# fraunhoferhhi/gaussian_gan_decoder

Hardware: AMD Instinct MI355X
Metric: forward raster frames/s, 1M Gaussians @ 1024x1024 (higher is better)
Workload: dtype f32; 1 GPU; 1000000 synthetic Gaussians ('cube' scene, seed 0, SH degree 0), 1024x1024, forward raster fp32, inputs resident in HBM; num_rendered=4152095, tiles=4096, parallelism=scene-parallel x1 (no collective)

## Files before the change

gaussian_gan_decoder_amd/_capi.py:

```python
from __future__ import annotations

import ctypes as C
import os
import threading

_PKG = os.path.dirname(os.path.abspath(__file__))
LIB_PATH = os.environ.get("GGD_LIB_PATH") or os.path.join(_PKG, "libggd_raster.so")

EXPORTS = [
    "ggd_geom_bytes", "ggd_binning_bytes", "ggd_img_bytes", "ggd_geom_layout", "ggd_binning_layout",
    "ggd_img_layout", "ggd_sort_bits", "ggd_create", "ggd_destroy", "ggd_last_error", "ggd_version",
    "ggd_forward_geometry", "ggd_forward_render", "ggd_forward", "ggd_forward_enqueue", "ggd_forward_collect", "ggd_forward_can_speculate", "ggd_backward",
    "ggd_forward_aux", "ggd_forward_render_aux", "ggd_backward_aux", "ggd_backward_abs", "ggd_mark_visible", "ggd_debug_unsorted",
    "ggd_triplane_forward", "ggd_triplane_backward", "ggd_trigrid_forward", "ggd_trigrid_backward", "ggd_planes_gather", "ggd_planes_scatter", "ggd_surface_tmp_bytes", "ggd_surface_sample", "ggd_attrs_split", "ggd_attrs_merge", "ggd_decoder_packed_bytes", "ggd_decoder_pack", "ggd_decoder_forward", "ggd_decoder_zbuf_bytes", "ggd_decoder_packed_t_bytes",
    "ggd_decoder_forward_train", "ggd_decoder_backward", "ggd_decoder_wgrad_floats", "ggd_decoder_wgrad", "ggd_decoder_backward_wgrad", "ggd_decoder_packed_hl_bytes", "ggd_decoder_packed_t_hl_bytes", "ggd_decoder_dzbuf_hl_bytes", "ggd_decoder_pack_hl", "ggd_decoder_forward_hl", "ggd_decoder_backward_wgrad_hl",
    "ggd_decoder_pack_chain", "ggd_decoder_forward_chain", "ggd_decoder_forward_train_chain", "ggd_decoder_backward_chain", "ggd_decoder_wgrad_chain",
    "ggd_decoder_backward_wgrad_chain", "ggd_decoder_pack_hl_chain", "ggd_decoder_forward_hl_chain", "ggd_decoder_backward_wgrad_hl_chain",
    "ggd_image_loss_tmp_bytes", "ggd_image_loss", "ggd_image_loss_masked", "ggd_mask_composite", "ggd_geometry_loss_tmp_bytes", "ggd_geometry_loss", "ggd_set_option", "ggd_get_option", "ggd_blend_stats", "ggd_blend_backward_stats", "ggd_blend_timeline", "ggd_set_profiling", "ggd_stage_count", "ggd_stage_name", "ggd_stage_times",
    "ggd_knn_tmp_bytes", "ggd_knn_leaf_size", "ggd_knn_max_points", "ggd_knn3", "ggd_knn3_stage",
    "ggd_densify_tmp_bytes", "ggd_densify_stats", "ggd_densify_plan", "ggd_prune_plan", "ggd_densify_emit", "ggd_densify_gather",
    "ggd_density_points", "ggd_density_grid", "ggd_density_lattice", "ggd_teacher_render",
]


class Params(C.Structure):
    _fields_ = [("P", C.c_int32), ("M", C.c_int32), ("sh_degree", C.c_int32), ("width", C.c_int32),
                ("height", C.c_int32), ("tanfovx", C.c_float), ("tanfovy", C.c_float),
                ("scale_modifier", C.c_float), ("prefiltered", C.c_int32), ("debug", C.c_int32),
                ("viewmatrix", C.c_void_p), ("projmatrix", C.c_void_p), ("campos", C.c_void_p),
                ("bg", C.c_void_p), ("raw_attributes", C.c_int32), ("antialiasing", C.c_int32)]


class GeomView(C.Structure):
    _fields_ = [(n, C.c_size_t) for n in ("splat", "tiles_touched", "point_offsets", "clamped", "depth_keys", "rect", "header", "total")]


class BinningView(C.Structure):
    _fields_ = [(n, C.c_size_t) for n in ("keys", "list", "keys_alt", "list_alt", "total")]


class ImgView(C.Structure):
    _fields_ = [(n, C.c_size_t) for n in ("ranges", "final_T", "n_contrib", "total")]


OPT_EXP_MODE, OPT_BLEND_CULL, OPT_BINNING, OPT_BLEND_SPLIT, OPT_FOLD, OPT_MSD_SORT, OPT_PREPROCESS_WGS = 0, 1, 2, 3, 4, 5, 6
STAT_FLAT_STREAK, STAT_SORT_RERUNS, STAT_MSD_FRAMES, STAT_SCAN_IN_SCATTER_FRAMES = 100, 101, 102, 103
SPLAT_BYTES = 48
SPLAT_FIELDS = ("x", "y", "hA", "nB", "hC", "thr", "opacity", "r", "g", "b", "ex", "ey")

_lib = None
_lock = threading.Lock()


def load():
    global _lib
    with _lock:
        if _lib is not None:
            return _lib
        if not os.path.exists(LIB_PATH):
            raise ImportError(
                f"{LIB_PATH} is missing: build it with `python -m gaussian_gan_decoder_amd.build` "
                "(hipcc --offload-arch=gfx950). There is no CPU fallback for the rasterizer.")
        import torch
        lib = C.CDLL(LIB_PATH, mode=C.RTLD_GLOBAL)
        vp, i32, i64, sz = C.c_void_p, C.c_int32, C.c_int64, C.c_size_t
        lib.ggd_geom_bytes.restype = sz; lib.ggd_geom_bytes.argtypes = [i32]
        lib.ggd_binning_bytes.restype = sz; lib.ggd_binning_bytes.argtypes = [i64]
        lib.ggd_img_bytes.restype = sz; lib.ggd_img_bytes.argtypes = [i32, i32]
        lib.ggd_geom_layout.argtypes = [i32, C.POINTER(GeomView)]
        lib.ggd_binning_layout.argtypes = [i64, C.POINTER(BinningView)]
        lib.ggd_img_layout.argtypes = [i32, i32, C.POINTER(ImgView)]
        lib.ggd_sort_bits.argtypes = [i32, i32]
        lib.ggd_create.restype = vp; lib.ggd_create.argtypes = [C.c_int]
        lib.ggd_destroy.restype = None; lib.ggd_destroy.argtypes = [vp]
        lib.ggd_last_error.restype = C.c_char_p; lib.ggd_last_error.argtypes = [vp]
        lib.ggd_version.restype = C.c_char_p
        lib.ggd_forward_geometry.argtypes = [vp, vp, C.POINTER(Params)] + [vp] * 7 + [vp, vp, C.POINTER(i64)]
        lib.ggd_forward_render.argtypes = [vp, vp, C.POINTER(Params), vp, i64, vp, vp, vp]
        lib.ggd_forward.argtypes = [vp, vp, C.POINTER(Params)] + [vp] * 7 + [vp, vp, vp, i64, vp, vp, C.POINTER(i64)]
        lib.ggd_forward_enqueue.argtypes = [vp, vp, C.POINTER(Params)] + [vp] * 7 + [vp, vp, vp, i64, vp, vp]
        lib.ggd_forward_collect.argtypes = [vp, vp, C.POINTER(i64)]
        lib.ggd_forward_can_speculate.argtypes = [vp, C.POINTER(Params), i64]
        lib.ggd_backward.argtypes = [vp, vp, C.POINTER(Params)] + [vp] * 7 + [vp, vp, vp, vp, i64, vp] + [vp] * 8
        lib.ggd_forward_aux.argtypes = [vp, vp, C.POINTER(Params)] + [vp] * 7 + [vp, vp, vp, i64, vp, vp, vp, vp, C.POINTER(i64)]
        lib.ggd_forward_render_aux.argtypes = [vp, vp, C.POINTER(Params), vp, i64, vp, vp, vp, vp, vp]
        lib.ggd_backward_aux.argtypes = [vp, vp, C.POINTER(Params)] + [vp] * 7 + [vp, vp, vp, vp, i64, vp, vp, vp] + [vp] * 8
        lib.ggd_backward_abs.argtypes = [vp, vp, C.POINTER(Params)] + [vp] * 7 + [vp, vp, vp, vp, i64, vp, vp, vp] + [vp] * 9
        lib.ggd_mark_visible.argtypes = [vp, vp, i32, vp, vp, vp, vp]
        lib.ggd_debug_unsorted.argtypes = [vp, vp, vp, vp, i64]
        lib.ggd_triplane_forward.argtypes = [vp, vp, vp, i32, i32, i32, vp, i32, C.c_float, vp]
        lib.ggd_triplane_backward.argtypes = [vp, vp, i32, i32, i32, vp, i32, C.c_float, vp, vp]
        lib.ggd_trigrid_forward.argtypes = [vp, vp, vp, i32, i32, i32, i32, i32, vp, i32, C.c_float, vp]
        lib.ggd_trigrid_backward.argtypes = [vp, vp, i32, i32, i32, i32, i32, vp, i32, C.c_float, vp, vp]
        lib.ggd_planes_gather.argtypes = [vp, vp, vp, i32, i32, i32, i32, i32, vp, vp, i32, C.c_float, vp]
        lib.ggd_planes_scatter.argtypes = [vp, vp, i32, i32, i32, i32, i32, vp, vp, i32, C.c_float, vp, vp, i32]
        lib.ggd_surface_tmp_bytes.restype = sz; lib.ggd_surface_tmp_bytes.argtypes = [i32]
        lib.ggd_surface_sample.argtypes = [vp, vp, vp, i32, C.c_float, i32, C.c_float, C.c_uint64, vp, vp, vp, sz]
        lib.ggd_attrs_split.argtypes = [vp, vp, vp, i64, vp, vp, vp, vp, vp]
        lib.ggd_attrs_merge.argtypes = [vp, vp, i64, vp, vp, vp, vp, vp, vp]
        lib.ggd_decoder_packed_bytes.restype = sz
        lib.ggd_decoder_pack.argtypes = [vp, vp, C.POINTER(C.c_void_p), vp, vp]
        lib.ggd_decoder_forward.argtypes = [vp, vp, vp, vp, i32, vp, vp]
        lib.ggd_decoder_zbuf_bytes.restype = sz; lib.ggd_decoder_zbuf_bytes.argtypes = [i32]
        lib.ggd_decoder_packed_t_bytes.restype = sz
        lib.ggd_decoder_forward_train.argtypes = [vp, vp, vp, vp, i32, vp, vp, vp]
        lib.ggd_decoder_backward.argtypes = [vp, vp, i32, vp, vp, vp, vp, vp, vp, vp, vp]
        lib.ggd_decoder_wgrad_floats.restype = sz
        lib.ggd_decoder_wgrad.argtypes = [vp, vp, i32, vp, vp, vp, vp, vp, vp, vp]
        lib.ggd_decoder_backward_wgrad.argtypes = [vp, vp, i32, i32, vp, vp, vp, vp, vp, vp, vp, vp, vp, vp, vp]
        lib.ggd_decoder_packed_hl_bytes.restype = sz
        lib.ggd_decoder_packed_t_hl_bytes.restype = sz
        lib.ggd_decoder_dzbuf_hl_bytes.restype = sz; lib.ggd_decoder_dzbuf_hl_bytes.argtypes = [i32]
        lib.ggd_decoder_pack_hl.argtypes = [vp, vp, C.POINTER(C.c_void_p), vp, vp]
        lib.ggd_decoder_forward_hl.argtypes = [vp, vp, vp, vp, i32, vp, vp, vp]
        lib.ggd_decoder_backward_wgrad_hl.argtypes = [vp, vp, i32, i32, vp, vp, vp, vp, vp, vp, vp, vp, vp, vp, vp]
        for name in ("pack", "forward", "forward_train", "backward", "wgrad", "backward_wgrad", "pack_hl", "forward_hl",
                     "backward_wgrad_hl"):
            base = getattr(lib, "ggd_decoder_" + name).argtypes
            getattr(lib, "ggd_decoder_" + name + "_chain").argtypes = list(base[:2]) + [i32] + list(base[2:])
        lib.ggd_image_loss_tmp_bytes.restype = sz; lib.ggd_image_loss_tmp_bytes.argtypes = [i32, i32]
        lib.ggd_image_loss.argtypes = [vp, vp, i32, i32, vp, vp, vp, vp, vp, vp, sz]
        lib.ggd_image_loss_masked.argtypes = [vp, vp, i32, i32, vp, vp, vp, i32, i32, vp, vp, vp, vp, sz]
        lib.ggd_mask_composite.argtypes = [vp, vp, i32, i32, i32, vp, vp, i32, i32, i32, vp]
        lib.ggd_geometry_loss_tmp_bytes.restype = sz; lib.ggd_geometry_loss_tmp_bytes.argtypes = [i32, i32]
        lib.ggd_geometry_loss.argtypes = [vp, vp, i32, i32, vp, vp, vp, vp, i32, i32, C.c_float, C.c_float, i32, vp, vp, vp, vp, vp, sz]
        lib.ggd_set_option.argtypes = [vp, C.c_int, C.c_int]
        lib.ggd_get_option.argtypes = [vp, C.c_int]
        lib.ggd_blend_stats.argtypes = [vp, C.c_int, C.POINTER(C.c_ulonglong)]
        lib.ggd_blend_backward_stats.argtypes = [vp, C.POINTER(C.c_ulonglong)]
        lib.ggd_blend_timeline.argtypes = [vp, C.POINTER(C.c_ulonglong), C.c_int]
        lib.ggd_set_profiling.argtypes = [vp, C.c_int]
        lib.ggd_stage_name.restype = C.c_char_p; lib.ggd_stage_name.argtypes = [C.c_int]
        lib.ggd_stage_times.argtypes = [vp, C.POINTER(C.c_float)]
        lib.ggd_knn_tmp_bytes.restype = sz; lib.ggd_knn_tmp_bytes.argtypes = [i32]
        lib.ggd_knn_leaf_size.restype = i32; lib.ggd_knn_leaf_size.argtypes = []
        lib.ggd_knn_max_points.restype = i32; lib.ggd_knn_max_points.argtypes = []
        lib.ggd_knn3.argtypes = [vp, vp, vp, i32, vp, vp, vp, vp, vp, sz]
        lib.ggd_knn3_stage.argtypes = [vp, vp, vp, i32, vp, vp, vp, vp, vp, sz, i32]
        f32 = C.c_float
        lib.ggd_densify_tmp_bytes.restype = sz; lib.ggd_densify_tmp_bytes.argtypes = [i32]
        lib.ggd_densify_stats.argtypes = [vp, vp, i32, vp, vp, vp, vp, vp, vp]
        lib.ggd_densify_plan.argtypes = [vp, vp, i32, vp, vp, vp, vp, f32, f32, f32, i32, f32, vp, sz, C.POINTER(i64)]
        lib.ggd_prune_plan.argtypes = [vp, vp, i32, vp, vp, sz, C.POINTER(i64)]
        lib.ggd_densify_emit.argtypes = [vp, vp, i32, i32, i32, C.POINTER(C.c_void_p), C.POINTER(C.c_void_p), vp, vp, sz]
        lib.ggd_densify_gather.argtypes = [vp, vp, i32, i32, i32, vp, vp, vp, sz]
        lib.ggd_density_points.argtypes = [vp, vp, vp, i32, i32, i32, i32, i32, f32, vp, vp, vp, vp, i32, vp, i32, vp, vp]
        lib.ggd_density_grid.argtypes = [vp, vp, vp, i32, i32, i32, i32, i32, f32, vp, vp, vp, vp, i32, i32, C.c_double, i32, vp, vp]
        lib.ggd_density_lattice.argtypes = [vp, vp, i32, C.c_double, i32, vp]
        lib.ggd_teacher_render.argtypes = [vp, vp, vp, i32, i32, i32, i32, i32, f32, vp, vp, vp, vp, i32, vp, vp, i32, C.c_double, C.c_double,
                                           vp, i32, i32, vp, vp, i32, C.c_double, i32, vp, vp, vp, vp]
        _lib = lib
        return lib


class RasterError(RuntimeError):
    pass


class Context:
    capacity_hint: dict
    capacity_retries: int

    def __init__(self, device_index: int):
        self.capacity_hint = {}
        self.capacity_retries = 0
        self.poison_outputs = False
        self.lib = load()
        self.device_index = int(device_index)
        self.handle = self.lib.ggd_create(self.device_index)
        if not self.handle:
            raise RasterError("ggd_create failed: " + self.lib.ggd_last_error(None).decode())

    def check(self, rc: int):
        if rc != 0:
            raise RasterError(f"ggd error {rc}: " + self.lib.ggd_last_error(self.handle).decode())

    def set_option(self, option: int, value: int):
        self.check(self.lib.ggd_set_option(self.handle, int(option), int(value)))

    def get_option(self, option: int) -> int:
        return int(self.lib.ggd_get_option(self.handle, int(option)))

    def blend_stats(self, enable):
        out = (C.c_ulonglong * 6)()
        self.check(self.lib.ggd_blend_stats(self.handle, int(enable), out))
        return dict(zip(("visited", "culled", "lanes", "pixels", "listed", "culled_in_loop"), [int(v) for v in out]))

    def blend_backward_stats(self):
        out = (C.c_ulonglong * 8)()
        self.check(self.lib.ggd_blend_backward_stats(self.handle, out))
        return dict(zip(("walked", "staged", "needed", "blended", "live_lanes", "atomic_spans", "rounds", "waves"), [int(v) for v in out]))

    def blend_timeline(self, waves: int):
        import numpy as np
        out = (C.c_ulonglong * (3 * waves))()
        self.check(self.lib.ggd_blend_timeline(self.handle, out, int(waves)))
        a = np.frombuffer(out, dtype=np.uint64).reshape(waves, 3)
        return np.stack([a[:, 0], a[:, 1], a[:, 2] >> np.uint64(32), a[:, 2] & np.uint64(0xFFFFFFFF)], 1).astype(np.int64)

    def set_profiling(self, on: bool):
        self.check(self.lib.ggd_set_profiling(self.handle, int(bool(on))))

    def stage_times(self) -> dict:
        n = self.lib.ggd_stage_count()
        arr = (C.c_float * n)()
        self.check(self.lib.ggd_stage_times(self.handle, arr))
        return {self.lib.ggd_stage_name(i).decode(): float(arr[i]) for i in range(n) if arr[i] >= 0}

    def close(self):
        if getattr(self, "handle", None):
            self.lib.ggd_destroy(self.handle)
            self.handle = None

    def __del__(self):
        try:
            self.close()
        except Exception:
            pass


_contexts: dict = {}


def context_for(device) -> Context:
    import torch
    idx = device.index if device.index is not None else torch.cuda.current_device()
    key = (idx, int(torch.cuda.current_stream(idx).cuda_stream))
    ctx = _contexts.get(key)
    if ctx is None:
        ctx = _contexts[key] = Context(idx)
    return ctx


def context_and_stream(device):
    import torch
    idx = device.index if device.index is not None else torch.cuda.current_device()
    handle = int(torch.cuda.current_stream(idx).cuda_stream)
    key = (idx, handle)
    ctx = _contexts.get(key)
    if ctx is None:
        ctx = _contexts[key] = Context(idx)
    return ctx, handle


def geom_view(P: int) -> GeomView:
    v = GeomView(); load().ggd_geom_layout(P, C.byref(v)); return v


def binning_view(R: int) -> BinningView:
    v = BinningView(); load().ggd_binning_layout(R, C.byref(v)); return v


def img_view(W: int, H: int) -> ImgView:
    v = ImgView(); load().ggd_img_layout(W, H, C.byref(v)); return v
```

gaussian_gan_decoder_amd/csrc/ggd_binning.hip:

```cpp
#include "ggd_common.h"

namespace {

#include "ggd_scan.inc"
#include "ggd_lookback.inc"

__global__ __launch_bounds__(SCAN_THREADS) void scan_reduce_kernel(const uint32_t* __restrict__ in, int64_t n,
                                                                   uint32_t* __restrict__ block_sums) {
  __shared__ uint32_t lds4[4];
  scan_reduce_block(in, n, block_sums, (int)blockIdx.x, lds4);
}

__global__ __launch_bounds__(SCAN_THREADS) void scan_blocksums_kernel(uint32_t* __restrict__ block_sums, int nb,
                                                                      uint32_t* __restrict__ d_total,
                                                                      uint32_t* h_total = nullptr) {
  __shared__ uint32_t lds4[4];
  scan_blocksums_block(block_sums, nb, d_total, h_total, lds4);
}

__global__ __launch_bounds__(SCAN_THREADS) void scan_apply_kernel(const uint32_t* __restrict__ in,
                                                                  uint32_t* __restrict__ out, int64_t n,
                                                                  const uint32_t* __restrict__ block_prefix) {
  __shared__ uint32_t lds4[4];
  scan_apply_block(in, out, n, block_prefix, (int)blockIdx.x, lds4);
}

__global__ __launch_bounds__(256) void duplicate_kernel(int P, int W, int H, const uint2* __restrict__ rect,
                                                        const uint32_t* __restrict__ depth_keys,
                                                        const uint32_t* __restrict__ tiles_touched,
                                                        const uint32_t* __restrict__ offsets,
                                                        uint64_t* __restrict__ keys, uint32_t* __restrict__ vals) {
  __shared__ uint32_t s_excl[257];
  __shared__ uint32_t s_origin[256];
  __shared__ uint32_t s_width[256];
  __shared__ uint32_t s_depth[256];
  __shared__ uint32_t s_base;
  const int tid = threadIdx.x;
  const int first = blockIdx.x * 256;
  const int i = first + tid;
  uint32_t nt = 0, inc = 0;
  if (i < P) { nt = tiles_touched[i]; inc = offsets[i]; }
  const uint32_t excl = inc - nt;
  if (tid == 0) s_base = excl;
  const int gx = (W + 15) / 16;
  uint32_t origin = 0, width = 1, dbits = 0;
  if (nt > 0) {
    const uint2 rc = rect[i];
    origin = (rc.x & 0xffffu) | ((rc.y & 0xffffu) << 16);
    width = (rc.x >> 16) - (rc.x & 0xffffu);
    dbits = depth_keys[i];
  }
  __syncthreads();
  const uint32_t base = s_base;
  s_excl[tid] = excl - base;
  s_origin[tid] = origin; s_width[tid] = width; s_depth[tid] = dbits;
  const int last = min(P, first + 256) - 1 - first;
  if (tid == last) s_excl[256] = inc - base;
  __syncthreads();
  const uint32_t total = s_excl[256];
  if (tid > last) s_excl[tid] = total;
  __syncthreads();
  for (uint32_t j = tid; j < total; j += 256) {
    int lo = 0;
#pragma unroll
    for (int step = 128; step >= 1; step >>= 1) {
      const int probe = lo + step;
      if (probe < 256 && s_excl[probe] <= j) lo = probe;
    }
    const uint32_t k = j - s_excl[lo];
    const uint32_t w = s_width[lo];
    const uint32_t ry = k / w, rx = k - ry * w;
    const uint32_t org = s_origin[lo];
    const uint32_t tile = ((org >> 16) + ry) * (uint32_t)gx + (org & 0xffffu) + rx;
    const size_t dst = (size_t)base + j;
    keys[dst] = ((uint64_t)tile << 32) | (uint64_t)s_depth[lo];
    vals[dst] = (uint32_t)(first + lo);
  }
}

template <typename KeyT, int ITEMS, bool SKIP = false>
__global__ __launch_bounds__(RS_THREADS) void sort_global_hist_kernel(const KeyT* __restrict__ keys, int64_t n,
                                                                      int passes, uint32_t* __restrict__ ghist,
                                                                      uint32_t* __restrict__ n_valid = nullptr,
                                                                      uint32_t* __restrict__ zero_ptr = nullptr,
                                                                      size_t zero_words = 0, int main_blocks = 0x7fffffff,
                                                                      ggd_scan_piggy pg = ggd_scan_piggy{}) {
  __shared__ uint32_t s_hist[RS_MAX_PASSES * RS_BINS];
  if ((int)blockIdx.x >= main_blocks) {
    scan_reduce_block(pg.in, pg.n, pg.block_sums, (int)blockIdx.x - main_blocks, s_hist);
    return;
  }
  const size_t nmain = (size_t)min((int)gridDim.x, main_blocks);
  for (size_t i = (size_t)blockIdx.x * RS_THREADS + threadIdx.x; i < zero_words; i += nmain * RS_THREADS)
    zero_ptr[i] = 0u;
  uint32_t my_valid = 0;
  for (int b = threadIdx.x; b < passes * RS_BINS; b += RS_THREADS) s_hist[b] = 0;
  __syncthreads();
  const int64_t base = (int64_t)blockIdx.x * (RS_THREADS * ITEMS);
  const int lane = threadIdx.x & 63;
  KeyT kreg[ITEMS];
#pragma unroll
  for (int k = 0; k < ITEMS; ++k) {
    const int64_t idx = base + (int64_t)k * RS_THREADS + threadIdx.x;
    kreg[k] = idx < n ? keys[idx] : (KeyT)0;
  }
#pragma unroll
  for (int k = 0; k < ITEMS; ++k) {
    const int64_t idx = base + (int64_t)k * RS_THREADS + threadIdx.x;
    const KeyT key = kreg[k];
    const bool ok = idx < n && !(SKIP && key == (KeyT)~(KeyT)0);
    const uint64_t act = __ballot(ok);
    if (act == 0ull) continue;
    if (SKIP && (threadIdx.x & 63) == 0) my_valid += (uint32_t)__popcll(act);
    const int leader = __builtin_ctzll(act);
    for (int p = 0; p < passes; ++p) {
      const uint32_t d = (uint32_t)(key >> (8 * p)) & 0xffu;
      if (p < 2) {
        if (ok) atomicAdd(&s_hist[p * RS_BINS + d], 1u);
        continue;
      }
      const uint32_t d0 = (uint32_t)__builtin_amdgcn_readlane((int)d, leader);
      if (__ballot(ok && d != d0) == 0ull) {
        if (lane == leader) atomicAdd(&s_hist[p * RS_BINS + d0], (uint32_t)__popcll(act));
      } else if (ok) {
        atomicAdd(&s_hist[p * RS_BINS + d], 1u);
      }
    }
  }
  __syncthreads();
  for (int b = threadIdx.x; b < passes * RS_BINS; b += RS_THREADS) {
    const uint32_t c = s_hist[b];
    if (c) atomicAdd(&ghist[b], c);
  }
  if (SKIP && n_valid && my_valid) atomicAdd(n_valid, my_valid);
}

__device__ __forceinline__ void fold_publish_range(const ggd_scan_piggy& pg, uint32_t flags, uint32_t nmin, uint32_t kmax) {
  if (threadIdx.x != 0) return;
  if (pg.d_total) { pg.d_total[3] = ~nmin; pg.d_total[4] = kmax; pg.d_total[5] = flags; }
  if (pg.h_total) { pg.h_total[4] = ~nmin; pg.h_total[5] = kmax; pg.h_total[6] = flags; }
}

enum ggd_passenger_role : int {
  GGD_PASSENGER_SCAN_SUMS = 2,
  GGD_PASSENGER_SCAN_APPLY = 3,
};

template <typename KeyT, bool IOTA, int ITEMS, bool COMPACT = false, bool STAGE = false>
__global__ __launch_bounds__(RS_THREADS) void sort_onesweep_kernel(
    const KeyT* __restrict__ keys_in, const uint32_t* __restrict__ vals_in, KeyT* __restrict__ keys_out,
    uint32_t* __restrict__ vals_out, int64_t n_host, int shift, const uint32_t* __restrict__ ghist ,
    uint32_t* status , int ntiles, int gshift, uint32_t* ticket,
    const uint32_t* __restrict__ n_dev = nullptr, int piggy_role = 0, ggd_scan_piggy pg = ggd_scan_piggy{},
    uint32_t* __restrict__ flat_flag = nullptr, int hist_reps = 1) {
  __shared__ uint32_t s_cnt[4][RS_BINS];
  if ((int)blockIdx.x >= ntiles) {
    if (piggy_role == GGD_PASSENGER_SCAN_SUMS && pg.wg_info) {
      const uint4 tv = scan_info_block(pg.wg_info, pg.n_info, pg.block_sums, pg.n_valid, pg.d_total, pg.h_total, &s_cnt[0][0]);
      int flat = 0;
      if (pg.fold_hist) {
        uint32_t acc[3] = {0u, 0u, 0u};
#pragma unroll 8
        for (int r = 1; r < GGD_FOLD_REPS; ++r) {
#pragma unroll
          for (int p = 1; p < 4; ++p) acc[p - 1] += pg.fold_hist[r * GGD_FOLD_REP_STRIDE + p * RS_BINS + threadIdx.x];
        }
#pragma unroll
        for (int p = 1; p < 4; ++p) {
          acc[p - 1] += pg.fold_hist[p * RS_BINS + threadIdx.x];
          pg.fold_hist[p * RS_BINS + threadIdx.x] = acc[p - 1];
        }
        flat = __syncthreads_or(acc[2] == tv.y);
        fold_publish_range(pg, flat ? 1u : 0u, tv.z, tv.w);
      }
      if (threadIdx.x == 0) {
        if (pg.spec_flat && pg.flat_flag) *pg.flat_flag = 1u;
        if (pg.d_total) pg.d_total[2] = (uint32_t)flat;
        if (pg.h_tagged)
          __hip_atomic_store(pg.h_tagged, ((unsigned long long)flat << 63) | ((unsigned long long)(pg.tag & 0x3fffffffu) << 32) | tv.x,
                             __ATOMIC_RELEASE, __HIP_MEMORY_SCOPE_SYSTEM);
      }
    }
    else if (piggy_role == GGD_PASSENGER_SCAN_SUMS)
      scan_blocksums_block(pg.block_sums, pg.nb, pg.d_total, pg.h_total, &s_cnt[0][0], pg.h_tagged, pg.tag);
    else
      scan_apply_block(pg.in, pg.out, pg.n, pg.block_sums, (int)blockIdx.x - ntiles, &s_cnt[0][0], pg.sum_stride);
    return;
  }
  __shared__ uint32_t s_scan[4];
  __shared__ uint32_t s_tile;
  __shared__ uint32_t s_flat;
  __shared__ KeyT s_keys[STAGE ? RS_THREADS * ITEMS : 1];
  __shared__ uint32_t s_vals[STAGE ? RS_THREADS * ITEMS : 1];
  __shared__ uint32_t s_gdst[STAGE ? RS_BINS : 1];
  __shared__ uint32_t s_ntile;
  const int lane = threadIdx.x & 63, wv = threadIdx.x >> 6;
  const bool use_ticket = ntiles > RS_RESIDENT;
  if (use_ticket && threadIdx.x == 0) s_tile = atomicAdd(ticket, 1u);
  const uint32_t n_dev_v = (COMPACT && !IOTA) ? *n_dev : 0u;
  uint32_t my_bin = ghist[threadIdx.x];
  if (hist_reps > 1) {
    uint32_t rep[GGD_FOLD_REPS - 1];
#pragma unroll
    for (int r = 1; r < GGD_FOLD_REPS; ++r) rep[r - 1] = ghist[r * GGD_FOLD_REP_STRIDE + threadIdx.x];
#pragma unroll
    for (int r = 1; r < GGD_FOLD_REPS; ++r) my_bin += rep[r - 1];
  }
  for (int b = threadIdx.x; b < 4 * RS_BINS; b += RS_THREADS) (&s_cnt[0][0])[b] = 0;
  if (threadIdx.x == 0) s_flat = 0u;
  uint32_t tile = blockIdx.x;
  if (use_ticket) { __syncthreads(); tile = s_tile; }

  const int64_t wbase = (int64_t)tile * (RS_THREADS * ITEMS) + (int64_t)wv * (64 * ITEMS);
  KeyT key[ITEMS];
  uint32_t val[ITEMS];
  uint32_t rank[ITEMS];
#pragma unroll
  for (int r = 0; r < ITEMS; ++r) {
    const int64_t idx = wbase + r * 64 + lane;
    const bool ok = idx < n_host;
    key[r] = ok ? keys_in[idx] : (KeyT)~(KeyT)0;
    val[r] = IOTA ? (uint32_t)idx : (ok ? vals_in[idx] : 0u);
  }
  const int64_t n = (COMPACT && !IOTA) ? (int64_t)n_dev_v : n_host;
  if (COMPACT && (int64_t)tile * (RS_THREADS * ITEMS) >= n) return;
  if (!use_ticket) __syncthreads();
  if (COMPACT && !IOTA) {
    if ((int64_t)my_bin == n) s_flat = 1u;
    __syncthreads();
    if (s_flat != 0u) {
      if (flat_flag) {
        if (tile == 0u && threadIdx.x == 0) *flat_flag = 1u;
        return;
      }
#pragma unroll
      for (int r = 0; r < ITEMS; ++r) {
        const int64_t idx = wbase + r * 64 + lane;
        if (idx < n) { keys_out[idx] = key[r]; vals_out[idx] = val[r]; }
      }
      return;
    }
  }
  const uint64_t lt_mask = (1ull << lane) - 1ull;
#pragma unroll
  for (int r = 0; r < ITEMS; ++r) {
    const int64_t idx = wbase + r * 64 + lane;
    const bool ok = idx < n && !(COMPACT && IOTA && key[r] == (KeyT)~(KeyT)0);
    const uint32_t d = (uint32_t)(key[r] >> shift) & 0xffu;
    uint64_t peers = __ballot(ok);
#pragma unroll
    for (int b = 0; b < 8; ++b) {
      const uint64_t m = __ballot((d >> b) & 1u);
      peers &= ((d >> b) & 1u) ? m : ~m;
    }
    const uint32_t before = s_cnt[wv][d];
    const uint32_t below = (uint32_t)__popcll(peers & lt_mask);
    rank[r] = before + below;
    __builtin_amdgcn_wave_barrier();
    if (ok && below == 0) s_cnt[wv][d] = before + (uint32_t)__popcll(peers);
    __builtin_amdgcn_wave_barrier();
  }
  __syncthreads();
  {
    const int d = threadIdx.x;
    const uint32_t c0 = s_cnt[0][d], c1 = s_cnt[1][d], c2 = s_cnt[2][d], c3 = s_cnt[3][d];
    const uint32_t local = c0 + c1 + c2 + c3;
    const int64_t live_tiles = (n + RS_THREADS * ITEMS - 1) / (RS_THREADS * ITEMS);
    gshift = min(gshift, ggd_group_shift(live_tiles));
    const uint32_t excl = lookback_two_level<RS_BINS>(status, d, ntiles, tile, gshift, local, 0u);
    uint32_t tot;
    const uint32_t gbase = block_exclusive_scan_256(my_bin, &tot, s_scan);
    const uint32_t base = gbase + excl;
    if constexpr (STAGE) {
      uint32_t ltot;
      const uint32_t lexcl = block_exclusive_scan_256(local, &ltot, s_scan);
      s_cnt[0][d] = lexcl; s_cnt[1][d] = lexcl + c0; s_cnt[2][d] = lexcl + c0 + c1; s_cnt[3][d] = lexcl + c0 + c1 + c2;
      s_gdst[d] = base - lexcl;
      if (d == 0) s_ntile = ltot;
    } else {
      s_cnt[0][d] = base; s_cnt[1][d] = base + c0; s_cnt[2][d] = base + c0 + c1; s_cnt[3][d] = base + c0 + c1 + c2;
    }
  }
  __syncthreads();
  if constexpr (STAGE) {
#pragma unroll
    for (int r = 0; r < ITEMS; ++r) {
      const int64_t idx = wbase + r * 64 + lane;
      if (idx < n && !(COMPACT && IOTA && key[r] == (KeyT)~(KeyT)0)) {
        const uint32_t d = (uint32_t)(key[r] >> shift) & 0xffu;
        const uint32_t p = s_cnt[wv][d] + rank[r];
        s_keys[p] = key[r];
        s_vals[p] = val[r];
      }
    }
    __syncthreads();
    const uint32_t nt = s_ntile;
    for (uint32_t p = threadIdx.x; p < nt; p += RS_THREADS) {
      const KeyT k = s_keys[p];
      const uint32_t d = (uint32_t)(k >> shift) & 0xffu;
      const size_t dst = (size_t)(uint32_t)(s_gdst[d] + p);
      keys_out[dst] = k;
      vals_out[dst] = s_vals[p];
    }
    return;
  }
#pragma unroll
  for (int r = 0; r < ITEMS; ++r) {
    const int64_t idx = wbase + r * 64 + lane;
    if (idx < n && !(COMPACT && IOTA && key[r] == (KeyT)~(KeyT)0)) {
      const uint32_t d = (uint32_t)(key[r] >> shift) & 0xffu;
      const size_t dst = (size_t)s_cnt[wv][d] + rank[r];
      keys_out[dst] = key[r];
      vals_out[dst] = val[r];
    }
  }
}


#include "ggd_msd_finish.inc"
constexpr int MSD_DIGIT_BITS = 10;
static_assert((1 << MSD_DIGIT_BITS) == GGD_MSD_BINS && GGD_MSD_BINS % (4 * RS_THREADS) == 0, "1024 buckets");

__device__ __forceinline__ void msd_piggy_block(const ggd_scan_piggy& pg, uint32_t* lds) {
  constexpr int NS = GGD_FOLD_REP_STRIDE / 256;
  uint32_t rep[GGD_FOLD_REPS][NS];
#pragma unroll
  for (int r = 0; r < GGD_FOLD_REPS; ++r)
#pragma unroll
    for (int q = 0; q < NS; ++q) rep[r][q] = pg.fold_hist[r * GGD_FOLD_REP_STRIDE + q * 256 + threadIdx.x];
  const uint32_t outside = pg.fold_hist[GGD_FOLD_OUTSIDE];
  const uint4 tv = scan_info_block(pg.wg_info, pg.n_info, pg.block_sums, pg.n_valid, pg.d_total, pg.h_total, lds);
  uint32_t acc[NS];
#pragma unroll
  for (int q = 0; q < NS; ++q) acc[q] = 0u;
#pragma unroll
  for (int r = 0; r < GGD_FOLD_REPS; ++r) {
#pragma unroll
    for (int q = 0; q < NS; ++q) acc[q] += rep[r][q];
  }
  bool over = false;
#pragma unroll
  for (int q = 0; q < NS; ++q) {
    pg.fold_hist[q * 256 + threadIdx.x] = acc[q];
    if (q < NS - 1) over = over || acc[q] > (uint32_t)GGD_MSD_CAP;
  }
  const int flat = __syncthreads_or(acc[NS - 1] == tv.y);
  const int big = __syncthreads_or(over);
  const bool inside = outside == 0u;
  const unsigned long long ok = (inside && !big) ? 1ull : 0ull;
  fold_publish_range(pg, (flat ? 1u : 0u) | (inside ? 2u : 0u) | (big ? 0u : 4u), tv.z, tv.w);
  if (threadIdx.x == 0) {
    if (pg.d_total) pg.d_total[2] = (uint32_t)(flat ? 1u : 0u) | ((uint32_t)ok << 1);
    if (pg.h_tagged)
      __hip_atomic_store(pg.h_tagged, ((unsigned long long)(flat ? 1 : 0) << 63) | (ok << 62) |
                                      ((unsigned long long)(pg.tag & 0x3fffffffu) << 32) | tv.x,
                         __ATOMIC_RELEASE, __HIP_MEMORY_SCOPE_SYSTEM);
  }
}

__global__ __launch_bounds__(RS_THREADS) void sort_msd_partition_kernel(const uint32_t* __restrict__ keys_in,
                                                                        uint32_t* __restrict__ keys_out,
                                                                        uint32_t* __restrict__ vals_out, int64_t n,
                                                                        uint32_t* __restrict__ table, int ntiles,
                                                                        uint32_t lo, int shift, ggd_scan_piggy pg) {
  __shared__ uint32_t s_cnt[4][GGD_MSD_BINS];
  __shared__ uint32_t s_keys[MSD_TILE];
  __shared__ uint32_t s_vals[MSD_TILE];
  __shared__ uint32_t s_scan[4];
  if ((int)blockIdx.x >= ntiles) { msd_piggy_block(pg, &s_cnt[0][0]); return; }
  const int lane = threadIdx.x & 63, wv = threadIdx.x >> 6;
  const uint32_t tile = blockIdx.x;
  const int64_t wbase = (int64_t)tile * MSD_TILE + (int64_t)wv * (64 * MSD_ITEMS);
  uint32_t key[MSD_ITEMS], rank[MSD_ITEMS];
#pragma unroll
  for (int r = 0; r < MSD_ITEMS; ++r) {
    const int64_t idx = wbase + r * 64 + lane;
    key[r] = idx < n ? keys_in[idx] : 0xffffffffu;
  }
  uint32_t dig[MSD_ITEMS];
#pragma unroll
  for (int r = 0; r < MSD_ITEMS; ++r) {
    const bool ok = key[r] != 0xffffffffu;
    const uint32_t rel = key[r] - lo;
    dig[r] = min(rel >> shift, (uint32_t)(GGD_MSD_BINS - 1));
    key[r] = ok ? rel : 0xffffffffu;
    if (!ok) dig[r] = 0xffffffffu;
  }
  for (int b = threadIdx.x; b < 4 * GGD_MSD_BINS; b += RS_THREADS) (&s_cnt[0][0])[b] = 0;
  __syncthreads();
  const uint64_t lt_mask = (1ull << lane) - 1ull;
#pragma unroll
  for (int r = 0; r < MSD_ITEMS; ++r) {
    const bool ok = dig[r] != 0xffffffffu;
    const uint32_t d = dig[r] & (GGD_MSD_BINS - 1);
    uint64_t peers = __ballot(ok);
#pragma unroll
    for (int b = 0; b < MSD_DIGIT_BITS; ++b) {
      const uint64_t m = __ballot((d >> b) & 1u);
      peers &= ((d >> b) & 1u) ? m : ~m;
    }
    const uint32_t before = s_cnt[wv][d];
    const uint32_t below = (uint32_t)__popcll(peers & lt_mask);
    rank[r] = before + below;
    __builtin_amdgcn_wave_barrier();
    if (ok && below == 0) s_cnt[wv][d] = before + (uint32_t)__popcll(peers);
    __builtin_amdgcn_wave_barrier();
  }
  __syncthreads();
  uint32_t ltot;
  {
    constexpr int DPT = GGD_MSD_BINS / RS_THREADS, G = DPT / 4;
    uint4 c[G][4];
    uint32_t mine = 0;
#pragma unroll
    for (int g = 0; g < G; ++g)
#pragma unroll
      for (int w = 0; w < 4; ++w) {
        c[g][w] = *reinterpret_cast<const uint4*>(&s_cnt[w][DPT * threadIdx.x + 4 * g]);
        mine += c[g][w].x + c[g][w].y + c[g][w].z + c[g][w].w;
      }
    uint32_t e = block_exclusive_scan_256(mine, &ltot, s_scan);
#pragma unroll
    for (int g = 0; g < G; ++g) {
      const uint32_t l0 = c[g][0].x + c[g][1].x + c[g][2].x + c[g][3].x, l1 = c[g][0].y + c[g][1].y + c[g][2].y + c[g][3].y;
      const uint32_t l2 = c[g][0].z + c[g][1].z + c[g][2].z + c[g][3].z, l3 = c[g][0].w + c[g][1].w + c[g][2].w + c[g][3].w;
      const uint32_t e0 = e, e1 = e0 + l0, e2 = e1 + l1, e3 = e2 + l2;
      e = e3 + l3;
      uint4 run = make_uint4(e0, e1, e2, e3);
#pragma unroll
      for (int w = 0; w < 4; ++w) {
        *reinterpret_cast<uint4*>(&s_cnt[w][DPT * threadIdx.x + 4 * g]) = run;
        run.x += c[g][w].x; run.y += c[g][w].y; run.z += c[g][w].z; run.w += c[g][w].w;
      }
      *reinterpret_cast<uint4*>(table + (size_t)tile * GGD_MSD_BINS + DPT * threadIdx.x + 4 * g) =
          make_uint4((e0 << 16) | l0, (e1 << 16) | l1, (e2 << 16) | l2, (e3 << 16) | l3);
    }
  }
  __syncthreads();
#pragma unroll
  for (int r = 0; r < MSD_ITEMS; ++r) {
    if (dig[r] != 0xffffffffu) {
      const uint32_t d = dig[r];
      const uint32_t p = s_cnt[wv][d] + rank[r];
      s_keys[p] = key[r];
      s_vals[p] = (uint32_t)(wbase + r * 64 + lane);
    }
  }
  __syncthreads();
  for (uint32_t p = threadIdx.x; p < ltot; p += RS_THREADS) {
    keys_out[(size_t)tile * MSD_TILE + p] = s_keys[p];
    vals_out[(size_t)tile * MSD_TILE + p] = s_vals[p];
  }
}

__global__ __launch_bounds__(MSDF_THREADS, 8) void sort_msd_finish_kernel(const uint32_t* __restrict__ keys_in,
                                                                       const uint32_t* __restrict__ vals_in,
                                                                       uint32_t* __restrict__ keys_out,
                                                                       uint32_t* __restrict__ vals_out,
                                                                       const uint32_t* __restrict__ hist ,
                                                                       const uint32_t* __restrict__ table, int ntiles, int kshift) {
  __shared__ msd_lds L;
  const int tid = threadIdx.x;
  const uint32_t b = blockIdx.x;
  const uint32_t nb = hist[b];
  constexpr int HPT = GGD_MSD_BINS / MSDF_THREADS;
  uint32_t below = 0;
#pragma unroll
  for (int q = 0; q < HPT; ++q) { const uint32_t i = (uint32_t)(HPT * tid + q); const uint32_t h = hist[i]; if (i < b) below += h; }
  const uint32_t e0 = tid < ntiles ? table[(size_t)tid * GGD_MSD_BINS + b] : 0u;
  if (nb == 0u) return;
  uint32_t base;
  block_exclusive_scan_1024(below, &base, L.part);
  const bool oversized = nb > (uint32_t)GGD_MSD_CAP;
  msd_bucket_pieces(L, table, ntiles, b, e0, oversized);
  if (oversized) {
    for (uint32_t p = tid; p < nb; p += MSDF_THREADS) {
      const size_t src = msd_piece_src_big(L, table, b, ntiles, p);
      vals_out[(size_t)base + p] = vals_in[src];
    }
    return;
  }
  if (nb > (uint32_t)MSD_XCAP) {
    msd_bucket_sort<true, MSDF_ITEMS>(L, keys_in, vals_in, ntiles, nb, kshift, keys_out + base, vals_out + base);
    return;
  }
  msd_bucket_sort<false, MSDX_ITEMS>(L, keys_in, vals_in, ntiles, nb, kshift, nullptr, nullptr);
  for (uint32_t p = tid; p < nb; p += MSDF_THREADS) vals_out[(size_t)base + p] = L.kv[MSD_XCAP + p];
}

__global__ __launch_bounds__(256) void ranges_kernel(const uint64_t* __restrict__ keys, int64_t n,
                                                     uint32_t* __restrict__ ranges) {
  const int64_t i = (int64_t)blockIdx.x * 256 + threadIdx.x;
  if (i >= n) return;
  const uint32_t tile = (uint32_t)(keys[i] >> 32);
  if (i == 0) {
    ranges[2 * tile] = 0;
  } else {
    const uint32_t prev = (uint32_t)(keys[i - 1] >> 32);
    if (prev != tile) {
      ranges[2 * prev + 1] = (uint32_t)i;
      ranges[2 * tile] = (uint32_t)i;
    }
  }
  if (i == n - 1) ranges[2 * tile + 1] = (uint32_t)n;
}

}

size_t ggd_scan_tmp_bytes(int64_t n) {
  const int64_t nb = (n + SCAN_TILE - 1) / SCAN_TILE;
  return ggd_align((size_t)(nb > 0 ? nb : 1) * sizeof(uint32_t));
}

int ggd_launch_inclusive_scan(ggd_ctx* ctx, hipStream_t s, const uint32_t* in, uint32_t* out, int64_t n,
                              uint32_t* d_total, void* tmp, size_t tmp_bytes, uint32_t* h_total) {
  if (n <= 0) {
    if (d_total) GGD_HIP(hipMemsetAsync(d_total, 0, sizeof(uint32_t), s));
    if (h_total) *h_total = 0u;
    return GGD_OK;
  }
  const int nb = (int)((n + SCAN_TILE - 1) / SCAN_TILE);
  if (tmp_bytes < (size_t)nb * sizeof(uint32_t)) return ggd_fail(ctx, GGD_E_INVALID, "scan tmp too small");
  uint32_t* block_sums = static_cast<uint32_t*>(tmp);
  hipLaunchKernelGGL(scan_reduce_kernel, dim3(nb), dim3(SCAN_THREADS), 0, s, in, n, block_sums);
  hipLaunchKernelGGL(scan_blocksums_kernel, dim3(1), dim3(SCAN_THREADS), 0, s, block_sums, nb, d_total, h_total);
  hipLaunchKernelGGL(scan_apply_kernel, dim3(nb), dim3(SCAN_THREADS), 0, s, in, out, n, block_sums);
  GGD_HIP(hipGetLastError());
  return GGD_OK;
}
int ggd_scan_blocks(int64_t n) { return n > 0 ? (int)((n + SCAN_TILE - 1) / SCAN_TILE) : 0; }

int ggd_launch_duplicate(ggd_ctx* ctx, hipStream_t s, const ggd_params& prm, const uint2* rect, const uint32_t* depth_keys,
                         const uint32_t* tiles_touched, const uint32_t* offsets, uint64_t* keys, uint32_t* vals) {
  if (prm.P == 0) return GGD_OK;
  hipLaunchKernelGGL(duplicate_kernel, dim3((prm.P + 255) / 256), dim3(256), 0, s, prm.P, prm.width, prm.height,
                     rect, depth_keys, tiles_touched, offsets, keys, vals);
  GGD_HIP(hipGetLastError());
  return GGD_OK;
}

static inline int sort_passes(int nbits) { return (nbits + 7) / 8; }
int ggd_sort_input_is_alt(int nbits) { return sort_passes(nbits) & 1; }

template <typename KeyT>
static int launch_sort_t(ggd_ctx* ctx, hipStream_t s, KeyT* keys_a, uint32_t* vals_a, KeyT* keys_b, uint32_t* vals_b,
                         int64_t n, int nbits, void* tmp, size_t tmp_bytes) {
  if (n <= 0) return GGD_OK;
  const int passes = sort_passes(nbits);
  if (passes > RS_MAX_PASSES) return ggd_fail(ctx, GGD_E_INVALID, "sort: too many key bits");
  if (tmp_bytes < ggd_sort_tmp_bytes(n)) return ggd_fail(ctx, GGD_E_INVALID, "sort tmp too small");
  const int ntiles = (int)((n + RS_TILE - 1) / RS_TILE);
  const ggd_sort_ctl ctl = ggd_sort_ctl::in_tmp(tmp);
  const int gshift = ggd_group_shift((int64_t)ntiles);
  GGD_HIP(hipMemsetAsync(tmp, 0, ggd_sort_clear_bytes(passes, ntiles), s));
  KeyT* kin = (passes & 1) ? keys_b : keys_a;
  uint32_t* vin = (passes & 1) ? vals_b : vals_a;
  KeyT* kout = (passes & 1) ? keys_a : keys_b;
  uint32_t* vout = (passes & 1) ? vals_a : vals_b;
  hipLaunchKernelGGL((sort_global_hist_kernel<KeyT, RS_ITEMS>), dim3(ntiles), dim3(RS_THREADS), 0, s, kin, n, passes,
                     ctl.ghist);
  for (int p = 0; p < passes; ++p) {
    hipLaunchKernelGGL((sort_onesweep_kernel<KeyT, false, RS_ITEMS>), dim3(ntiles), dim3(RS_THREADS), 0, s, kin, vin, kout, vout, n,
                       8 * p, ctl.pass_hist(p), ctl.pass_status(p, ntiles), ntiles, gshift, ctl.pass_ticket(p));
    KeyT* tk = kin; kin = kout; kout = tk;
    uint32_t* tv = vin; vin = vout; vout = tv;
  }
  GGD_HIP(hipGetLastError());
  return GGD_OK;
}

int ggd_launch_sort32_iota(ggd_ctx* ctx, hipStream_t s, const uint32_t* keys_src, uint32_t* keys_a, uint32_t* vals_a,
                           uint32_t* keys_b, uint32_t* vals_b, int64_t n, int nbits, void* tmp, size_t tmp_bytes,
                           const ggd_sort32_opts& o) {
  if (n <= 0) return GGD_OK;
  const ggd_fold* fold = o.fold;
  const int passes = sort_passes(nbits);
  if (passes > RS_MAX_PASSES || (passes & 1)) return ggd_fail(ctx, GGD_E_INVALID, "sort32: need an even pass count");
  if (fold && (passes != 4 || !o.piggy || !o.piggy->wg_info)) return ggd_fail(ctx, GGD_E_INVALID, "sort32: folded front end needs 4 passes and the workgroup sums");
  if (!fold && tmp_bytes < ggd_sort32_tmp_bytes(n)) return ggd_fail(ctx, GGD_E_INVALID, "sort tmp too small");
  if (o.skip_last && !(fold && o.flag_flat_last)) return ggd_fail(ctx, GGD_E_INVALID, "sort32: skip_last needs the folded front end");
  const int ntiles = (int)((n + RS32_TILE - 1) / RS32_TILE);
  const ggd_sort_ctl ctl = ggd_sort_ctl::select(tmp, o.clean_ctl, fold ? fold->ctl : nullptr);
  const bool own_ctl = !o.clean_ctl && !fold;
  const int gshift = ggd_group_shift((int64_t)ntiles);
  if (own_ctl) GGD_HIP(hipMemsetAsync(tmp, 0, ggd_sort_clear_bytes(passes, ntiles), s));
  ggd_scan_piggy pg = o.piggy ? *o.piggy : ggd_scan_piggy{};
  const int pnb = o.piggy ? pg.nb : 0;
  if (fold) { pg.n_valid = ctl.n_valid; pg.fold_hist = ctl.ghist; pg.flat_flag = ctl.flat; pg.spec_flat = o.skip_last ? 1 : 0; }
  if (!fold) {
    const int htiles = ntiles;
    hipLaunchKernelGGL((sort_global_hist_kernel<uint32_t, RS32_ITEMS, true>), dim3(htiles + pnb), dim3(RS_THREADS), 0, s,
                       keys_src, n, passes, ctl.ghist, ctl.n_valid, o.clean_ctl ? ctl.status : nullptr,
                       o.clean_ctl ? ggd_sort_status_words(passes, ntiles) : (size_t)0, htiles, pg);
  }
  const uint32_t* kin = keys_src;
  const uint32_t* vin = nullptr;
  for (int p = 0; p < passes - (o.skip_last ? 1 : 0); ++p) {
    uint32_t* kout = (p & 1) ? keys_a : keys_b;
    uint32_t* vout = (p & 1) ? vals_a : vals_b;
    if (p == 0)
      hipLaunchKernelGGL((sort_onesweep_kernel<uint32_t, true, RS32_ITEMS, true, true>), dim3(ntiles + (pnb ? 1 : 0)),
                         dim3(RS_THREADS), 0, s, kin, vin, kout, vout, n, 0, ctl.pass_hist(0), ctl.pass_status(0, ntiles), ntiles,
                         gshift, ctl.pass_ticket(0), ctl.n_valid, GGD_PASSENGER_SCAN_SUMS, pg, (uint32_t*)nullptr, ctl.reps);
    if (p != 0)
      hipLaunchKernelGGL((sort_onesweep_kernel<uint32_t, false, RS32_ITEMS, true, true>), dim3(ntiles + ((p == 1 && o.apply_here) ? pnb : 0)),
                         dim3(RS_THREADS), 0, s, kin, vin, kout, vout, n, 8 * p, ctl.pass_hist(p), ctl.pass_status(p, ntiles),
                         ntiles, gshift, ctl.pass_ticket(p), ctl.n_valid, GGD_PASSENGER_SCAN_APPLY, pg,
                         (o.flag_flat_last && p == passes - 1) ? ctl.flat : nullptr, 1);
    kin = kout; vin = vout;
  }
  GGD_HIP(hipGetLastError());
  return GGD_OK;
}

bool ggd_sort32_msd_supported(int64_t n) { return n > 0 && (n + MSD_TILE - 1) / MSD_TILE <= GGD_MSD_MAX_TILES; }

int ggd_launch_sort32_msd(ggd_ctx* ctx, hipStream_t s, const uint32_t* keys_src, uint32_t* keys_a, uint32_t* vals_a,
                          uint32_t* keys_b, uint32_t* vals_b, int64_t n, uint32_t* table, const ggd_scan_piggy* piggy,
                          const ggd_fold* fold) {
  if (n <= 0) return GGD_OK;
  if (!fold || !fold->msd || !piggy || !piggy->wg_info || !ggd_sort32_msd_supported(n))
    return ggd_fail(ctx, GGD_E_INVALID, "sort32 (two launches): needs the folded front end in its msd form");
  if (fold->msd_shift < 0 || fold->msd_shift > GGD_MSD_MAX_SHIFT) return ggd_fail(ctx, GGD_E_INVALID, "sort32 (two launches): bucket shift out of range");
  const int ntiles = (int)((n + MSD_TILE - 1) / MSD_TILE);
  const ggd_sort_ctl ctl = ggd_sort_ctl::in_fold(fold->ctl);
  ggd_scan_piggy pg = *piggy;
  pg.n_valid = ctl.n_valid; pg.fold_hist = ctl.ghist;
  hipLaunchKernelGGL(sort_msd_partition_kernel, dim3(ntiles + 1), dim3(RS_THREADS), 0, s, keys_src, keys_b, vals_b, n, table,
                     ntiles, fold->msd_lo, fold->msd_shift, pg);
  hipLaunchKernelGGL(sort_msd_finish_kernel, dim3(GGD_MSD_BINS), dim3(MSDF_THREADS), 0, s, keys_b, vals_b, keys_a, vals_a,
                     ctl.ghist, table, ntiles, fold->msd_shift);
  GGD_HIP(hipGetLastError());
  return GGD_OK;
}

int ggd_launch_sort(ggd_ctx* ctx, hipStream_t s, uint64_t* keys_a, uint32_t* vals_a, uint64_t* keys_b,
                    uint32_t* vals_b, int64_t n, int nbits, void* tmp, size_t tmp_bytes) {
  return launch_sort_t<uint64_t>(ctx, s, keys_a, vals_a, keys_b, vals_b, n, nbits, tmp, tmp_bytes);
}

int ggd_launch_ranges(ggd_ctx* ctx, hipStream_t s, const uint64_t* keys, int64_t n, uint32_t* ranges, int T) {
  GGD_HIP(hipMemsetAsync(ranges, 0, (size_t)T * 2 * sizeof(uint32_t), s));
  if (n <= 0) return GGD_OK;
  hipLaunchKernelGGL(ranges_kernel, dim3((unsigned)((n + 255) / 256)), dim3(256), 0, s, keys, n, ranges);
  GGD_HIP(hipGetLastError());
  return GGD_OK;
}
```

gaussian_gan_decoder_amd/csrc/ggd_binning_layout.h:

```cpp
#pragma once

#include <stdint.h>
#include <stddef.h>

#if defined(__HIPCC__)
#define GGD_HOST_DEVICE __host__ __device__
#else
#define GGD_HOST_DEVICE
#endif

static inline size_t ggd_align(size_t v, size_t a = 256) { return (v + a - 1) / a * a; }

constexpr int RS_THREADS = 256;
constexpr int RS_ITEMS = 16;
constexpr int RS_TILE = RS_THREADS * RS_ITEMS;
constexpr int RS_BINS = 256;
constexpr int RS_MAX_PASSES = 8;
constexpr int RS32_ITEMS = 16;
constexpr int RS32_TILE = RS_THREADS * RS32_ITEMS;
constexpr int RS_HWORDS = RS_MAX_PASSES * RS_BINS;
constexpr int RS_RESIDENT = 1024;

template <typename T>
GGD_HOST_DEVICE inline int ggd_group_shift(T n) { int g = 2; while (((T)1 << (2 * g)) < n) ++g; return g; }

static inline int64_t rs_status_words(int64_t ntiles) {
  return (ntiles + ((int64_t)1 << ggd_group_shift(ntiles)) + 1) * RS_BINS;
}
static inline int64_t ggd_tiles(int64_t n, int tile) { const int64_t t = (n + tile - 1) / tile; return t > 0 ? t : 1; }

static inline size_t ggd_sort_ctrl_bytes() { return ggd_align((size_t)(RS_HWORDS + 64) * sizeof(uint32_t)); }
static inline size_t ggd_sort_ctrl_words() { return ggd_sort_ctrl_bytes() / sizeof(uint32_t); }
static inline size_t ggd_sort_tmp_bytes(int64_t n) {
  return ggd_sort_ctrl_bytes() + ggd_align((size_t)RS_MAX_PASSES * (size_t)rs_status_words(ggd_tiles(n, RS_TILE)) * sizeof(uint32_t));
}
static inline size_t ggd_sort32_tmp_bytes(int64_t n) {
  return ggd_sort_ctrl_bytes() + ggd_align((size_t)4 * (size_t)rs_status_words(ggd_tiles(n, RS32_TILE)) * sizeof(uint32_t));
}
static inline size_t ggd_sort_status_words(int passes, int64_t ntiles) { return (size_t)passes * (size_t)rs_status_words(ntiles); }
static inline size_t ggd_sort_clear_bytes(int passes, int64_t ntiles) {
  return ggd_sort_ctrl_bytes() + ggd_sort_status_words(passes, ntiles) * sizeof(uint32_t);
}

constexpr int GGD_MSD_BINS = 1024, GGD_MSD_CAP = 12288, GGD_MSD_MAX_TILES = 2048;
constexpr int MSD_ITEMS = 16;
constexpr int MSD_TILE = 256 * MSD_ITEMS;
static inline size_t ggd_sort32_msd_table_bytes(int64_t n) {
  return ggd_align((size_t)ggd_tiles(n, MSD_TILE) * GGD_MSD_BINS * sizeof(uint32_t));
}

constexpr int GGD_FOLD_REPS = 16;
constexpr int GGD_FOLD_REP_STRIDE = GGD_MSD_BINS + 256;
constexpr int GGD_FOLD_OUTSIDE = GGD_FOLD_REPS * GGD_FOLD_REP_STRIDE + 16;
constexpr int GGD_FOLD_ROWTOT = GGD_FOLD_REPS * GGD_FOLD_REP_STRIDE + 64;
constexpr int GGD_FOLD_HEAD = GGD_FOLD_ROWTOT + GGD_FOLD_REPS * 64;
static inline size_t ggd_fold_l1_offset(int64_t P) {
  return (size_t)GGD_FOLD_HEAD + (size_t)4 * (size_t)rs_status_words(ggd_tiles(P, RS32_TILE));
}
static inline size_t ggd_fold_ctl_words(int64_t P) {
  const int64_t chunks = (P + 1023) / 1024;
  return ggd_fold_l1_offset(P) + (size_t)(chunks + ((int64_t)1 << ggd_group_shift(chunks > 0 ? chunks : 1)) + 2) * 64;
}
static inline size_t ggd_fold_rowinst_offset(int64_t P) { return ggd_fold_ctl_words(P); }
static inline size_t ggd_fold_block_words(int64_t P) { return ggd_fold_rowinst_offset(P) + (size_t)GGD_FOLD_REPS * 64; }
static inline uint32_t* ggd_fold_rowtot(uint32_t* fold_ctl) { return fold_ctl + GGD_FOLD_ROWTOT; }
static inline uint32_t* ggd_fold_rowinst(uint32_t* fold_ctl, int64_t P) { return fold_ctl + ggd_fold_rowinst_offset(P); }
static inline uint32_t* ggd_fold_l1_status(uint32_t* fold_ctl, int64_t P) { return fold_ctl + ggd_fold_l1_offset(P); }

struct ggd_sort_ctl {
  uint32_t* ghist = nullptr;
  uint32_t* tickets = nullptr;
  uint32_t* n_valid = nullptr;
  uint32_t* flat = nullptr;
  uint32_t* status = nullptr;
  int reps = 1;

  static ggd_sort_ctl in_tmp(void* tmp) {
    return make(static_cast<uint32_t*>(tmp), RS_HWORDS, tmp_status(tmp), 1);
  }
  static ggd_sort_ctl in_clean(uint32_t* clean_ctl, void* tmp) { return make(clean_ctl, RS_HWORDS, tmp_status(tmp), 1); }
  static ggd_sort_ctl in_fold(uint32_t* fold_ctl) {
    return make(fold_ctl, GGD_FOLD_REPS * GGD_FOLD_REP_STRIDE, fold_ctl + GGD_FOLD_HEAD, GGD_FOLD_REPS);
  }
  static ggd_sort_ctl select(void* tmp, uint32_t* clean_ctl, uint32_t* fold_ctl) {
    return fold_ctl ? in_fold(fold_ctl) : (clean_ctl ? in_clean(clean_ctl, tmp) : in_tmp(tmp));
  }

  uint32_t* pass_hist(int p) const { return ghist + p * RS_BINS; }
  uint32_t* pass_ticket(int p) const { return tickets + p; }
  uint32_t* pass_status(int p, int64_t ntiles) const { return status + ggd_sort_status_words(p, ntiles); }

 private:
  static uint32_t* tmp_status(void* tmp) { return reinterpret_cast<uint32_t*>(static_cast<char*>(tmp) + ggd_sort_ctrl_bytes()); }
  static ggd_sort_ctl make(uint32_t* head, int hist_words, uint32_t* status, int reps) {
    ggd_sort_ctl c;
    c.ghist = head; c.tickets = head + hist_words; c.n_valid = c.tickets + RS_MAX_PASSES; c.flat = c.n_valid + 1;
    c.status = status; c.reps = reps;
    return c;
  }
};

constexpr int RB_THREADS = 256;
constexpr int RB_IPL = 4;
constexpr int RB_CHUNK = RB_THREADS * RB_IPL;
constexpr int RB_TAB_ROWSTART = 0, RB_TAB_ROWBLK = 65, RB_TAB_TILESTART = 130, RB_TAB_ROWINST = 130 + 64 * 64,
              RB_TAB_FLAG = RB_TAB_ROWINST + 64, RB_TAB_WORDS = RB_TAB_FLAG + 64;
constexpr int RBW_NG = 4;
constexpr int RBW_BINS = 64 * RBW_NG;
constexpr int RBW_TAB_ROWSTART = 0, RBW_TAB_ROWBLK = RBW_BINS + 1, RBW_TAB_ROWINST = 2 * (RBW_BINS + 1),
              RBW_TAB_FLAG = RBW_TAB_ROWINST + RBW_BINS, RBW_TAB_TILESTART = RBW_TAB_FLAG + RBW_BINS,
              RBW_TAB_WORDS = RBW_TAB_TILESTART + RBW_BINS * RBW_BINS;

static inline bool rb_is_wide(int W, int H) { return (W + 15) / 16 > 64 || (H + 15) / 16 > 64; }
static inline int rb_blocks1(int P) { return (P + RB_CHUNK - 1) / RB_CHUNK; }
constexpr uint32_t RB_SCAN_IN_SCATTER_MAX_BLOCKS = (1u << 24) / RB_CHUNK + 128;
static inline uint32_t rb_blocks2(uint32_t cap, bool wide) {
  return (cap + RB_CHUNK - 1) / RB_CHUNK + (wide ? (uint32_t)RBW_BINS : 64u);
}

struct ggd_rowbin_tmp {
  size_t packed, counts1, tab, ent, counts2, total;
};
static inline ggd_rowbin_tmp ggd_rowbin_layout(int P, uint32_t capacity, int W, int H) {
  const bool wide = rb_is_wide(W, H);
  const int nby = 64 * (((H + 15) / 16 + 63) / 64), nbx = 64 * (((W + 15) / 16 + 63) / 64);
  ggd_rowbin_tmp t;
  t.packed = 0;
  t.counts1 = t.packed + ggd_align((size_t)P * 8);
  t.tab = t.counts1 + ggd_align((size_t)rb_blocks1(P) * (wide ? nby : 64) * 4);
  t.ent = t.tab + ggd_align((size_t)(wide ? RBW_TAB_WORDS : RB_TAB_WORDS) * 4);
  t.counts2 = t.ent + ggd_align((size_t)capacity * 8);
  t.total = t.counts2 + ggd_align((size_t)rb_blocks2(capacity, wide) * (wide ? nbx : 64) * 4);
  return t;
}
```

gaussian_gan_decoder_amd/csrc/ggd_capi.hip:

```cpp
#include <stdlib.h>
#include <string.h>

#include <initializer_list>
#include <new>

#include "ggd_common.h"

static std::string g_create_error;

static const char* const kStageNames[ST_COUNT] = {"preprocess", "scan", "readback", "duplicate", "sort",
                                                  "ranges", "blend", "blend_bwd", "preprocess_bwd"};

int ggd_fail(ggd_ctx* ctx, int code, const std::string& msg) {
  if (ctx) ctx->err = msg; else g_create_error = msg;
  return code;
}

int ggd_reserve_scratch(ggd_ctx* ctx, size_t bytes, hipStream_t stream) {
  if (bytes <= ctx->scratch_bytes) return GGD_OK;
  size_t want = bytes + bytes / 4 + (1u << 20);
  if (ctx->scratch) {
    GGD_HIP(hipStreamSynchronize(stream));
    GGD_HIP(hipFree(ctx->scratch));
    ctx->scratch = nullptr; ctx->scratch_bytes = 0;
  }
  hipError_t e = hipMalloc(&ctx->scratch, want);
  if (e != hipSuccess) return ggd_fail(ctx, GGD_E_NOMEM, std::string("hipMalloc scratch: ") + hipGetErrorString(e));
  ctx->scratch_bytes = want;
  return GGD_OK;
}

extern "C" int ggd_geom_layout(int32_t P, ggd_geom_view* v) {
  if (!v || P < 0) return GGD_E_INVALID;
  size_t off = 0;
  v->splat = off; off += ggd_align((size_t)P * sizeof(ggd_splat));
  v->tiles_touched = off; off += ggd_align((size_t)P * sizeof(uint32_t));
  v->point_offsets = off; off += ggd_align((size_t)P * sizeof(uint32_t));
  v->clamped = off; off += ggd_align((size_t)P);
  v->depth_keys = off; off += ggd_align((size_t)P * sizeof(uint32_t));
  v->rect = off; off += ggd_align((size_t)P * 2 * sizeof(uint32_t));
  v->header = off; off += (P > 0 ? 256 : 0);
  v->total = off;
  return GGD_OK;
}
extern "C" int ggd_binning_layout(int64_t R, ggd_binning_view* v) {
  if (!v || R < 0) return GGD_E_INVALID;
  size_t off = 0;
  v->list = off; off += ggd_align((size_t)R * sizeof(uint32_t));
  v->list_alt = off; off += ggd_align((size_t)R * sizeof(uint32_t));
  v->keys = off; off += ggd_align((size_t)R * sizeof(uint64_t));
  v->keys_alt = off; off += ggd_align((size_t)R * sizeof(uint64_t));
  v->total = off;
  return GGD_OK;
}
extern "C" int ggd_img_layout(int32_t W, int32_t H, ggd_img_view* v) {
  if (!v || W < 0 || H < 0) return GGD_E_INVALID;
  const size_t T = (size_t)((W + 15) / 16) * ((H + 15) / 16);
  size_t off = 0;
  v->ranges = off; off += ggd_align(T * 2 * sizeof(uint32_t));
  v->final_T = off; off += ggd_align((size_t)W * H * sizeof(float));
  v->n_contrib = off; off += ggd_align((size_t)W * H * sizeof(uint32_t));
  v->total = off;
  return GGD_OK;
}
extern "C" size_t ggd_geom_bytes(int32_t P) { ggd_geom_view v; return ggd_geom_layout(P, &v) == GGD_OK ? v.total : 0; }
extern "C" size_t ggd_binning_bytes(int64_t R) { ggd_binning_view v; return ggd_binning_layout(R, &v) == GGD_OK ? v.total : 0; }
extern "C" size_t ggd_img_bytes(int32_t W, int32_t H) { ggd_img_view v; return ggd_img_layout(W, H, &v) == GGD_OK ? v.total : 0; }

static uint32_t higher_msb(uint32_t n) {
  uint32_t msb = 16, step = 16;
  while (step > 1) {
    step /= 2;
    if (n >> msb) msb += step; else msb -= step;
  }
  if (n >> msb) msb++;
  return msb;
}
extern "C" int ggd_sort_bits(int32_t W, int32_t H) {
  const uint32_t T = (uint32_t)((W + 15) / 16) * (uint32_t)((H + 15) / 16);
  return 32 + (int)higher_msb(T);
}

static bool use_tile_binning(const ggd_ctx* ctx, const ggd_params* prm, int64_t R) {
  const int mode = ctx->opt[GGD_OPT_BINNING];
  return !prm->debug && ggd_rowbin_supported(prm->width, prm->height) && (mode >= 2 || (mode == 1 && R > 0));
}

struct ggd_buf { void** ptr; size_t elem; };
static int grow_buffers(ggd_ctx* ctx, std::initializer_list<ggd_buf> bufs, size_t* cap, size_t need, size_t want,
                        const hipStream_t* sync = nullptr) {
  if (*cap >= need) return GGD_OK;
  if (sync) GGD_HIP(hipStreamSynchronize(*sync));
  for (const ggd_buf& b : bufs) { if (*b.ptr) (void)hipFree(*b.ptr); *b.ptr = nullptr; }
  *cap = 0;
  for (const ggd_buf& b : bufs) GGD_HIP(hipMalloc(b.ptr, want * b.elem));
  *cap = want;
  return GGD_OK;
}

template <class T> static T* ggd_at(const void* base, size_t off) {
  return reinterpret_cast<T*>(static_cast<char*>(const_cast<void*>(base)) + off);
}
struct geom_ptrs { ggd_splat* splat; uint32_t *tiles, *offsets; uint8_t* clamped; uint32_t* depth_keys; uint2* rect; };
struct binning_ptrs { uint32_t *list, *list_alt; uint64_t *keys, *keys_alt; };
struct img_ptrs { uint32_t* ranges; float* final_T; uint32_t* n_contrib; };
static geom_ptrs geom_view(const ggd_params* prm, const void* buf) {
  ggd_geom_view v; ggd_geom_layout(prm->P, &v);
  return {ggd_at<ggd_splat>(buf, v.splat), ggd_at<uint32_t>(buf, v.tiles_touched), ggd_at<uint32_t>(buf, v.point_offsets),
          ggd_at<uint8_t>(buf, v.clamped), ggd_at<uint32_t>(buf, v.depth_keys), ggd_at<uint2>(buf, v.rect)};
}
static binning_ptrs binning_view(int64_t layout_R, const void* buf) {
  ggd_binning_view v; ggd_binning_layout(layout_R, &v);
  return {ggd_at<uint32_t>(buf, v.list), ggd_at<uint32_t>(buf, v.list_alt), ggd_at<uint64_t>(buf, v.keys), ggd_at<uint64_t>(buf, v.keys_alt)};
}
static img_ptrs img_view(int32_t W, int32_t H, const void* buf) {
  ggd_img_view v; ggd_img_layout(W, H, &v);
  return {ggd_at<uint32_t>(buf, v.ranges), ggd_at<float>(buf, v.final_T), ggd_at<uint32_t>(buf, v.n_contrib)};
}

extern "C" const char* ggd_version(void) { return "ggd-raster 0.1 (gfx950)"; }
extern "C" int ggd_stage_count(void) { return ST_COUNT; }
extern "C" const char* ggd_stage_name(int s) { return (s >= 0 && s < ST_COUNT) ? kStageNames[s] : ""; }

extern "C" ggd_ctx* ggd_create(int device) {
  int ndev = 0;
  if (hipGetDeviceCount(&ndev) != hipSuccess || ndev <= 0 || device < 0 || device >= ndev) {
    ggd_fail(nullptr, GGD_E_NODEVICE, "no HIP device " + std::to_string(device) + " visible");
    return nullptr;
  }
  ggd_ctx* ctx = new (std::nothrow) ggd_ctx();
  if (!ctx) { ggd_fail(nullptr, GGD_E_NOMEM, "out of host memory"); return nullptr; }
  ctx->device = device;
  if (const char* e = getenv("GGD_EXP_MODE")) { const int v = atoi(e); if (v >= 0 && v <= 3) ctx->opt[GGD_OPT_EXP_MODE] = v; }
  if (const char* e = getenv("GGD_BINNING")) { const int v = atoi(e); if (v >= 0 && v <= 3) ctx->opt[GGD_OPT_BINNING] = v; }
  if (const char* e = getenv("GGD_BLEND_SPLIT")) { const int v = atoi(e); if (v >= 0 && v <= 4) ctx->opt[GGD_OPT_BLEND_SPLIT] = v; }
  if (const char* e = getenv("GGD_BLEND_CULL")) ctx->opt[GGD_OPT_BLEND_CULL] = atoi(e) != 0;
  if (const char* e = getenv("GGD_FOLD")) ctx->opt[GGD_OPT_FOLD] = atoi(e) != 0;
  if (const char* e = getenv("GGD_MSD_SORT")) ctx->opt[GGD_OPT_MSD_SORT] = atoi(e) != 0;
  if (const char* e = getenv("GGD_PREPROCESS_WGS")) { const int v = atoi(e); if (v >= 0 && v <= GGD_PREPROCESS_WGS_MAX) ctx->opt[GGD_OPT_PREPROCESS_WGS] = v; }
  if (const char* e = getenv("GGD_MSD_BUCKETS")) { const int v = atoi(e); if (v >= 16 && v <= GGD_MSD_BINS) ctx->spec.msd_buckets = v; }
  int prev = 0;
  (void)hipGetDevice(&prev);
  bool ok = hipSetDevice(device) == hipSuccess &&
            hipMalloc((void**)&ctx->d_words, 256) == hipSuccess &&
            hipHostMalloc((void**)&ctx->h_words, 64, hipHostMallocCoherent | hipHostMallocMapped) == hipSuccess &&
            hipMemset(ctx->d_words, 0, 256) == hipSuccess &&
            hipDeviceGetAttribute(&ctx->cus, hipDeviceAttributeMultiprocessorCount, device) == hipSuccess && ctx->cus > 0;
  if (ok) memset(ctx->h_words, 0, 64);
  for (int i = 0; ok && i < 2 * ST_COUNT; ++i) ok = hipEventCreate(&ctx->ev[i]) == hipSuccess;
  if (ok && hipHostGetDevicePointer((void**)&ctx->h_words_dev, ctx->h_words, 0) != hipSuccess) {
    ctx->h_words_dev = nullptr;
    (void)hipGetLastError();
  }
  if (ok && (hipMalloc((void**)&ctx->sortctl, ggd_sort_ctrl_words() * sizeof(uint32_t)) != hipSuccess ||
             hipMemset(ctx->sortctl, 0, ggd_sort_ctrl_words() * sizeof(uint32_t)) != hipSuccess)) {
    ctx->sortctl = nullptr;
    (void)hipGetLastError();
  }
  (void)hipSetDevice(prev);
  if (!ok) {
    ggd_fail(nullptr, GGD_E_HIP, std::string("ggd_create: ") + hipGetErrorString(hipGetLastError()));
    ggd_destroy(ctx);
    return nullptr;
  }
  return ctx;
}

extern "C" void ggd_destroy(ggd_ctx* ctx) {
  if (!ctx) return;
  void* const device_buffers[] = {ctx->scratch, ctx->d_words, ctx->sortctl, ctx->foldctl[0], ctx->foldctl[1], ctx->gelu_tables,
                                  ctx->scan_sums, ctx->stats_buf, ctx->dbg_keys, ctx->dbg_vals};
  for (void* p : device_buffers) if (p) (void)hipFree(p);
  if (ctx->h_words) (void)hipHostFree(ctx->h_words);
  for (int i = 0; i < 2 * ST_COUNT; ++i)
    if (ctx->ev[i]) (void)hipEventDestroy(ctx->ev[i]);
  delete ctx;
}

extern "C" const char* ggd_last_error(ggd_ctx* ctx) { return ctx ? ctx->err.c_str() : g_create_error.c_str(); }

extern "C" int ggd_set_option(ggd_ctx* ctx, int option, int value) {
  if (!ctx) return GGD_E_INVALID;
  static const int kMax[GGD_OPT_COUNT] = {3, 1, 3, 4, 1, 1, GGD_PREPROCESS_WGS_MAX};
  if (option < 0 || option >= GGD_OPT_COUNT || value < 0 || value > kMax[option])
    return ggd_fail(ctx, GGD_E_INVALID, "ggd_set_option: unknown option or value");
  ctx->opt[option] = value;
  if (option == GGD_OPT_MSD_SORT || option == GGD_OPT_FOLD) {
    ctx->spec.reset();
  }
  return GGD_OK;
}
extern "C" int ggd_blend_stats(ggd_ctx* ctx, int enable, unsigned long long* out) {
  if (!ctx) return GGD_E_INVALID;
  GGD_HIP(hipDeviceSynchronize());
  if (out && ctx->blend_stats) GGD_HIP(hipMemcpy(out, ctx->stats_buf, 6 * sizeof(unsigned long long), hipMemcpyDeviceToHost));
  if (enable) {
    const size_t bytes = (GGD_STATS_HEAD + 3ull * GGD_STATS_MAX_WAVES) * sizeof(unsigned long long);
    if (!ctx->stats_buf) GGD_HIP(hipMalloc((void**)&ctx->stats_buf, bytes));
    GGD_HIP(hipMemset(ctx->stats_buf, 0, bytes));
    if (enable == 2) {
      const unsigned long long one = 1ull;
      GGD_HIP(hipMemcpy(ctx->stats_buf + GGD_STATS_MODE, &one, sizeof(one), hipMemcpyHostToDevice));
    }
    ctx->blend_stats = ctx->stats_buf;
  } else {
    ctx->blend_stats = nullptr;
  }
  return GGD_OK;
}
extern "C" int ggd_blend_backward_stats(ggd_ctx* ctx, unsigned long long* out) {
  if (!ctx || !out) return GGD_E_INVALID;
  if (!ctx->stats_buf) return ggd_fail(ctx, GGD_E_INVALID, "ggd_blend_backward_stats: statistics were never enabled (ggd_blend_stats)");
  GGD_HIP(hipDeviceSynchronize());
  GGD_HIP(hipMemcpy(out, ctx->stats_buf + GGD_STATS_BWD, 8 * sizeof(unsigned long long), hipMemcpyDeviceToHost));
  return GGD_OK;
}
extern "C" int ggd_blend_timeline(ggd_ctx* ctx, unsigned long long* out, int waves) {
  if (!ctx || !out || waves < 0 || waves > GGD_STATS_MAX_WAVES) return GGD_E_INVALID;
  if (!ctx->stats_buf) return ggd_fail(ctx, GGD_E_INVALID, "ggd_blend_timeline: statistics were never enabled");
  GGD_HIP(hipDeviceSynchronize());
  GGD_HIP(hipMemcpy(out, ctx->stats_buf + GGD_STATS_HEAD, 3ull * waves * sizeof(unsigned long long), hipMemcpyDeviceToHost));
  return GGD_OK;
}

extern "C" int ggd_get_option(ggd_ctx* ctx, int option) {
  if (ctx && option == GGD_STAT_FLAT_STREAK) return ctx->spec.flat_streak;
  if (ctx && option == GGD_STAT_SORT_RERUNS) return (int)(ctx->spec.reruns & 0x7fffffffull);
  if (ctx && option == GGD_STAT_MSD_FRAMES) return (int)(ctx->spec.msd_frames & 0x7fffffffull);
  if (ctx && option == GGD_STAT_SCAN_IN_SCATTER_FRAMES) return (int)(ctx->scan_in_scatter_frames & 0x7fffffffull);
  if (!ctx || option < 0 || option >= GGD_OPT_COUNT) return GGD_E_INVALID;
  return ctx->opt[option];
}

extern "C" int ggd_set_profiling(ggd_ctx* ctx, int enabled) {
  if (!ctx) return GGD_E_INVALID;
  ctx->profiling = enabled != 0;
  for (int i = 0; i < ST_COUNT; ++i) ctx->ev_used[i] = false;
  return GGD_OK;
}

extern "C" int ggd_stage_times(ggd_ctx* ctx, float* ms_out) {
  if (!ctx || !ms_out) return GGD_E_INVALID;
  for (int i = 0; i < ST_COUNT; ++i) {
    ms_out[i] = -1.0f;
    if (ctx->ev_used[i]) {
      GGD_HIP(hipEventSynchronize(ctx->ev[2 * i + 1]));
      float ms = 0.0f;
      GGD_HIP(hipEventElapsedTime(&ms, ctx->ev[2 * i], ctx->ev[2 * i + 1]));
      ms_out[i] = ms;
    }
  }
  return GGD_OK;
}

static int check_params(ggd_ctx* ctx, const ggd_params* prm) {
  if (!ctx) return GGD_E_INVALID;
  if (!prm) return ggd_fail(ctx, GGD_E_INVALID, "params is NULL");
  if (prm->P < 0 || prm->width <= 0 || prm->height <= 0)
    return ggd_fail(ctx, GGD_E_INVALID, "bad P / image size");
  if (!prm->viewmatrix || !prm->projmatrix || !prm->campos || !prm->bg)
    return ggd_fail(ctx, GGD_E_INVALID, "viewmatrix / projmatrix / campos / bg must be device pointers");
  if (prm->sh_degree < 0 || prm->sh_degree > 3) return ggd_fail(ctx, GGD_E_INVALID, "sh_degree must be 0..3");
  if (prm->tanfovx == 0.0f || prm->tanfovy == 0.0f) return ggd_fail(ctx, GGD_E_INVALID, "tanfov must be non-zero");
  return GGD_OK;
}

static int check_inputs(ggd_ctx* ctx, const ggd_params* prm, const float* means3D, const float* shs,
                        const float* colors_precomp, const float* scales, const float* rotations,
                        const float* cov3D_precomp) {
  if (prm->P == 0) return GGD_OK;
  if (!means3D) return ggd_fail(ctx, GGD_E_INVALID, "means3D is NULL");
  if ((shs == nullptr) == (colors_precomp == nullptr))
    return ggd_fail(ctx, GGD_E_INVALID, "Please provide excatly one of either SHs or precomputed colors!");
  if (((scales == nullptr) || (rotations == nullptr)) == (cov3D_precomp == nullptr) ||
      ((scales == nullptr) != (rotations == nullptr)))
    return ggd_fail(ctx, GGD_E_INVALID,
                    "Please provide exactly one of either scale/rotation pair or precomputed 3D covariance!");
  if (shs && (prm->sh_degree + 1) * (prm->sh_degree + 1) > prm->M)
    return ggd_fail(ctx, GGD_E_INVALID, "shs holds fewer coefficients than sh_degree needs");
  return GGD_OK;
}

static const char* const kPendingMsg = "a frame enqueued with ggd_forward_enqueue is pending on this context: call ggd_forward_collect first";

static ggd_frame frame_renew(ggd_ctx* ctx) {
  const ggd_frame old = ctx->frame;
  ctx->frame = ggd_frame();
  ctx->frame.r_tag = old.r_tag;
  return old;
}

static int fold_prepare(ggd_ctx* ctx, hipStream_t s, const ggd_params* prm, ggd_fold* fold) {
  const int nwg = (prm->P + 255) / 256;
  int rc = grow_buffers(ctx, {{(void**)&ctx->scan_sums, sizeof(uint32_t)}}, &ctx->scan_sums_cap, 5 * (size_t)nwg + 64,
                        5 * (size_t)(nwg + nwg / 2) + 64);
  if (rc != GGD_OK) return rc;
  const size_t need = ggd_fold_block_words(prm->P);
  const bool fresh = ctx->foldctl_cap < need;
  rc = grow_buffers(ctx, {{(void**)&ctx->foldctl[0], sizeof(uint32_t)}, {(void**)&ctx->foldctl[1], sizeof(uint32_t)}},
                    &ctx->foldctl_cap, need, need + need / 2, &s);
  if (rc != GGD_OK) return rc;
  if (fresh) ctx->fold_cur = 0;
  if (fresh || ctx->fold_poisoned) {
    for (int b = 0; b < 2; ++b) {
      GGD_HIP(hipMemsetAsync(ctx->foldctl[b], 0, ctx->foldctl_cap * sizeof(uint32_t), s));
      ctx->foldctl_dirty[b] = 0;
    }
    ctx->fold_poisoned = false;
  }
  const int cur = ctx->fold_cur, oth = cur ^ 1;
  fold->ctl = ctx->foldctl[cur];
  fold->clear = ctx->foldctl[oth];
  fold->clear_words = (uint32_t)ctx->foldctl_dirty[oth];
  fold->wg_info = reinterpret_cast<uint4*>(ctx->scan_sums + (((size_t)nwg + 3) & ~(size_t)3));
  fold->rows = ((prm->width + 15) / 16 <= 64 && (prm->height + 15) / 16 <= 64) ? 1 : 0;
  fold->rowinst = ggd_fold_rowinst(fold->ctl, prm->P);
  const ggd_spec_plan plan = ctx->spec.plan(ctx->opt[GGD_OPT_FOLD], ctx->opt[GGD_OPT_MSD_SORT], ggd_sort32_msd_supported(prm->P));
  fold->msd = plan.msd ? 1 : 0;
  fold->msd_lo = plan.lo; fold->msd_shift = plan.shift;
  ctx->foldctl_dirty[oth] = 0;
  ctx->foldctl_dirty[cur] = need;
  ctx->fold_cur = oth;
  ctx->frame.plan = plan;
  ctx->frame.geom.folded = true;
  return GGD_OK;
}

static int geometry_enqueue(ggd_ctx* ctx, void* stream, const ggd_params* prm, const float* means3D,
                            const float* shs, const float* colors_precomp, const float* opacities,
                            const float* scales, const float* rotations, const float* cov3D_precomp,
                            void* geom_buf, int32_t* radii, int64_t* num_rendered, bool defer_scan = false) {
  (void)hipGetLastError();
  int rc = check_params(ctx, prm);
  if (rc != GGD_OK) return rc;
  rc = check_inputs(ctx, prm, means3D, shs, colors_precomp, scales, rotations, cov3D_precomp);
  if (rc != GGD_OK) return rc;
  if (!num_rendered) return ggd_fail(ctx, GGD_E_INVALID, "num_rendered is NULL");
  *num_rendered = 0;
  frame_renew(ctx);
  ggd_frame& fr = ctx->frame;
  if (prm->P == 0) return GGD_OK;
  if (!geom_buf || !radii || !opacities) return ggd_fail(ctx, GGD_E_INVALID, "geom_buf / radii / opacities is NULL");
  if (prm->raw_attributes && cov3D_precomp)
    return ggd_fail(ctx, GGD_E_INVALID, "raw_attributes needs scales/rotations (no cov3D_precomp)");
  hipStream_t s = static_cast<hipStream_t>(stream);
  const geom_ptrs g = geom_view(prm, geom_buf);

  rc = ggd_reserve_scratch(ctx, ggd_scan_tmp_bytes(prm->P), s);
  if (rc != GGD_OK) return rc;
  if (prm->prefiltered) GGD_HIP(hipMemsetAsync(ctx->d_words + 1, 0, sizeof(uint32_t), s));
  const bool ride = defer_scan && ctx->h_words_dev;
  ggd_fold fold;
  if (ride && ctx->opt[GGD_OPT_FOLD] != 0) {
    rc = fold_prepare(ctx, s, prm, &fold);
    if (rc != GGD_OK) return rc;
  }
  {
    StageTimer t(ctx, ST_PREPROCESS, s);
    const bool old_ctl = !fr.geom.folded && ctx->sortctl;
    rc = ggd_launch_preprocess(ctx, s, *prm, means3D, shs, colors_precomp, opacities, scales, rotations,
                               cov3D_precomp, g.splat, g.tiles, shs ? g.clamped : nullptr, radii, g.depth_keys, g.rect,
                               ctx->d_words + 1, old_ctl ? ctx->sortctl : nullptr, old_ctl ? (int)ggd_sort_ctrl_words() : 0,
                               fr.geom.folded ? &fold : nullptr);
    if (rc != GGD_OK) { ctx->fold_poisoned = fr.geom.folded; return rc; }
    fr.geom.sortctl_clean = old_ctl;
  }
  if (ride) {
    const size_t nb = (size_t)ggd_scan_blocks(prm->P);
    if (!fr.geom.folded) {
      rc = grow_buffers(ctx, {{(void**)&ctx->scan_sums, sizeof(uint32_t)}}, &ctx->scan_sums_cap, nb, nb + nb / 2 + 64);
      if (rc != GGD_OK) return rc;
    }
    if (prm->prefiltered)
      GGD_HIP(hipMemcpyAsync(ctx->h_words + 1, ctx->d_words + 1, sizeof(uint32_t), hipMemcpyDeviceToHost, s));
    fr.geom.ride = true;
    return GGD_OK;
  }
  {
    StageTimer t(ctx, ST_SCAN, s);
    rc = ggd_launch_inclusive_scan(ctx, s, g.tiles, g.offsets, prm->P, ctx->d_words, ctx->scratch, ctx->scratch_bytes,
                                   ctx->h_words_dev);
    if (rc != GGD_OK) return rc;
  }
  {
    StageTimer t(ctx, ST_READBACK, s);
    if (!ctx->h_words_dev)
      GGD_HIP(hipMemcpyAsync(ctx->h_words, ctx->d_words, 2 * sizeof(uint32_t), hipMemcpyDeviceToHost, s));
    else if (prm->prefiltered)
      GGD_HIP(hipMemcpyAsync(ctx->h_words + 1, ctx->d_words + 1, sizeof(uint32_t), hipMemcpyDeviceToHost, s));
  }
  return GGD_OK;
}

static int geometry_finish(ggd_ctx* ctx, void* stream, const ggd_params* prm, int64_t* num_rendered) {
  ggd_frame& fr = ctx->frame;
  if (fr.r_pending) {
    volatile unsigned long long* slot = reinterpret_cast<volatile unsigned long long*>(ctx->h_words + 2);
    const unsigned long long want = fr.r_tag;
    unsigned long long v = *slot;
    for (unsigned spins = 0; ((v >> 32) & 0x3fffffffull) != want; ++spins) {
      __builtin_ia32_pause();
      if ((spins & 0xfff) == 0xfff) {
        const hipError_t q = hipStreamQuery(static_cast<hipStream_t>(stream));
        if (q == hipSuccess) {
          v = *slot;
          if (((v >> 32) & 0x3fffffffull) != want) {
            uint32_t w6[6] = {0u, 0u, 0u, 0u, 0u, 0u};
            GGD_HIP(hipMemcpy(w6, ctx->d_words, sizeof(w6), hipMemcpyDeviceToHost));
            v = ((unsigned long long)(w6[2] & 1u) << 63) | ((unsigned long long)((w6[2] >> 1) & 1u) << 62) | (want << 32) | w6[0];
            ctx->h_words[4] = w6[3]; ctx->h_words[5] = w6[4]; ctx->h_words[6] = w6[5];
          }
          break;
        }
        if (q != hipErrorNotReady)
          return ggd_fail(ctx, GGD_E_HIP, std::string("hipStreamQuery: ") + hipGetErrorString(q));
      }
      v = *slot;
    }
    ctx->h_words[0] = (uint32_t)v;
    fr.report.flat = (v >> 63) != 0ull;
    fr.report.msd_ok = ((v >> 62) & 1ull) != 0ull;
    if (fr.report.folded) {
      volatile uint32_t* hw = ctx->h_words;
      fr.report.kmin = hw[4]; fr.report.kmax = hw[5]; fr.report.msd_flags = hw[6];
    }
  } else {
    GGD_HIP(hipStreamSynchronize(static_cast<hipStream_t>(stream)));
  }
  if (prm->prefiltered && ctx->h_words[1] != 0)
    return ggd_fail(ctx, GGD_E_PREFILTER, "Point is filtered although prefiltered is set. This shouldn't happen!");
  *num_rendered = (int64_t)ctx->h_words[0];
  return GGD_OK;
}

extern "C" int ggd_forward_geometry(ggd_ctx* ctx, void* stream, const ggd_params* prm, const float* means3D,
                                    const float* shs, const float* colors_precomp, const float* opacities,
                                    const float* scales, const float* rotations, const float* cov3D_precomp,
                                    void* geom_buf, int32_t* radii, int64_t* num_rendered) {
  if (ctx && ctx->pending.valid) return ggd_fail(ctx, GGD_E_INVALID, kPendingMsg);
  const int rc = geometry_enqueue(ctx, stream, prm, means3D, shs, colors_precomp, opacities, scales, rotations,
                                  cov3D_precomp, geom_buf, radii, num_rendered);
  if (rc != GGD_OK || prm->P == 0) return rc;
  return geometry_finish(ctx, stream, prm, num_rendered);
}

static int sort_depth_and_bin_tiles(ggd_ctx* ctx, hipStream_t s, const ggd_params* prm, const geom_ptrs& g, uint32_t* list,
                                    uint32_t* ranges, uint32_t capacity, bool speculative) {
  ggd_frame& fr = ctx->frame;
  const bool riding = fr.geom.ride;
  const bool folded = riding && fr.geom.folded;
  const bool msd = folded && fr.plan.msd;
  uint32_t* clean_ctl = fr.geom.sortctl_clean ? ctx->sortctl : nullptr;
  fr.geom = {};
  const size_t pairs = ggd_align((size_t)prm->P * sizeof(uint32_t));
  const size_t sort_tmp = ggd_sort32_tmp_bytes(prm->P);
  const size_t bin_tmp = ggd_rowbin_tmp_bytes(prm->P, capacity, prm->width, prm->height);
  const size_t msd_tab = msd ? ggd_sort32_msd_table_bytes(prm->P) : 0;
  int rc = ggd_reserve_scratch(ctx, 4 * pairs + sort_tmp + bin_tmp + msd_tab, s);
  if (rc != GGD_OK) return rc;
  char* sc = static_cast<char*>(ctx->scratch);
  uint32_t* ka = reinterpret_cast<uint32_t*>(sc);
  uint32_t* va = reinterpret_cast<uint32_t*>(sc + pairs);
  uint32_t* kb = reinterpret_cast<uint32_t*>(sc + 2 * pairs);
  uint32_t* vb = reinterpret_cast<uint32_t*>(sc + 3 * pairs);
  void* tmp = sc + 4 * pairs;
  void* bin_tmp_ptr = sc + 4 * pairs + sort_tmp;
  ggd_scan_piggy pg;
  ggd_fold fold;
  const uint32_t *n_vis_ptr = nullptr, *flat_ptr = nullptr;
  {
    StageTimer t(ctx, ST_SORT, s);
    if (riding) {
      pg.in = g.tiles; pg.out = g.offsets;
      pg.n = prm->P; pg.nb = ggd_scan_blocks(prm->P); pg.block_sums = ctx->scan_sums;
      pg.d_total = ctx->d_words; pg.h_total = ctx->h_words_dev;
      pg.h_tagged = reinterpret_cast<unsigned long long*>(ctx->h_words_dev + 2);
      pg.tag = fr.r_tag = fr.r_tag % 0x3fffffffu + 1u;
      if (folded) {
        const int nwg = (prm->P + 255) / 256;
        fold.ctl = ctx->foldctl[ctx->fold_cur ^ 1];
        pg.wg_info = reinterpret_cast<const uint4*>(ctx->scan_sums + (((size_t)nwg + 3) & ~(size_t)3));
        pg.n_info = nwg;
        pg.sum_stride = 8;
      }
    }
    if (msd && !speculative) return ggd_fail(ctx, GGD_E_INVALID, "internal: two-launch sort outside the speculative tile-binning path");
    fr.three_passes = ctx->spec.three_passes(fr.plan, folded, speculative, ctx->opt[GGD_OPT_FOLD]);
    fr.report.folded = folded;
    fold.msd = msd ? 1 : 0;
    fold.msd_lo = fr.plan.lo; fold.msd_shift = fr.plan.shift;
    if (msd)
      rc = ggd_launch_sort32_msd(ctx, s, g.depth_keys, ka, va, kb, vb, prm->P,
                                 reinterpret_cast<uint32_t*>(sc + 4 * pairs + sort_tmp + bin_tmp), &pg, &fold);
    else {
      ggd_sort32_opts so;
      so.clean_ctl = folded ? nullptr : clean_ctl;
      so.piggy = riding ? &pg : nullptr;
      so.fold = folded ? &fold : nullptr;
      so.flag_flat_last = true;
      so.apply_here = false;
      so.skip_last = fr.three_passes;
      rc = ggd_launch_sort32_iota(ctx, s, g.depth_keys, ka, va, kb, vb, prm->P, 32, tmp, sort_tmp, so);
    }
    if (rc != GGD_OK) return rc;
    fr.r_pending = riding;
    const ggd_sort_ctl sc = ggd_sort_ctl::select(tmp, clean_ctl, folded ? fold.ctl : nullptr);
    n_vis_ptr = sc.n_valid; flat_ptr = sc.flat;
  }
  StageTimer t(ctx, ST_DUPLICATE, s);
  const bool l1 = folded && (prm->width + 15) / 16 <= 64 && (prm->height + 15) / 16 <= 64;
  bool scan_in_scatter = false;
  rc = ggd_launch_rowbin(ctx, s, *prm, g.rect, va, n_vis_ptr, list, ranges, capacity, bin_tmp_ptr, bin_tmp, vb,
                         flat_ptr, riding ? &pg : nullptr, l1 ? ggd_fold_rowtot(fold.ctl) : nullptr,
                         l1 ? ggd_fold_l1_status(fold.ctl, prm->P) : nullptr, l1 ? ggd_fold_rowinst(fold.ctl, prm->P) : nullptr,
                         &scan_in_scatter);
  if (scan_in_scatter) ++ctx->scan_in_scatter_frames;
  return rc;
}

static int duplicate_sort_ranges(ggd_ctx* ctx, hipStream_t s, const ggd_params* prm, const geom_ptrs& g, const binning_ptrs& b,
                                 uint32_t* ranges, int64_t R) {
  const int T = ((prm->width + 15) / 16) * ((prm->height + 15) / 16);
  int rc = GGD_OK;
  if (R > 0) {
    const int nbits = ggd_sort_bits(prm->width, prm->height);
    const size_t sort_tmp = ggd_sort_tmp_bytes(R);
    rc = ggd_reserve_scratch(ctx, sort_tmp, s);
    if (rc != GGD_OK) return rc;
    const bool to_alt = ggd_sort_input_is_alt(nbits) != 0;
    uint64_t* k0 = to_alt ? b.keys_alt : b.keys;
    uint32_t* v0 = to_alt ? b.list_alt : b.list;
    {
      StageTimer t(ctx, ST_DUPLICATE, s);
      rc = ggd_launch_duplicate(ctx, s, *prm, g.rect, g.depth_keys, g.tiles, g.offsets, k0, v0);
      if (rc != GGD_OK) return rc;
    }
    if (prm->debug) {
      rc = grow_buffers(ctx, {{&ctx->dbg_keys, sizeof(uint64_t)}, {&ctx->dbg_vals, sizeof(uint32_t)}}, &ctx->dbg_cap, (size_t)R, (size_t)R);
      if (rc != GGD_OK) return rc;
      GGD_HIP(hipMemcpyAsync(ctx->dbg_keys, k0, (size_t)R * sizeof(uint64_t), hipMemcpyDeviceToDevice, s));
      GGD_HIP(hipMemcpyAsync(ctx->dbg_vals, v0, (size_t)R * sizeof(uint32_t), hipMemcpyDeviceToDevice, s));
    }
    StageTimer t(ctx, ST_SORT, s);
    rc = ggd_launch_sort(ctx, s, b.keys, b.list, b.keys_alt, b.list_alt, R, nbits, ctx->scratch, ctx->scratch_bytes);
    if (rc != GGD_OK) return rc;
  }
  StageTimer t(ctx, ST_RANGES, s);
  return ggd_launch_ranges(ctx, s, b.keys, R, ranges, T);
}

static int render_enqueue(ggd_ctx* ctx, void* stream, const ggd_params* prm, const void* geom_buf, int64_t layout_R,
                          int64_t R, void* binning_buf, void* img_buf, float* out_color, bool speculative,
                          float* out_depth = nullptr, float* out_alpha = nullptr) {
  (void)hipGetLastError();
  int rc = check_params(ctx, prm);
  if (rc != GGD_OK) return rc;
  if (R < 0) return ggd_fail(ctx, GGD_E_INVALID, "num_rendered < 0");
  if (!img_buf || !out_color) return ggd_fail(ctx, GGD_E_INVALID, "img_buf / out_color is NULL");
  if (R > 0 && (!geom_buf || !binning_buf)) return ggd_fail(ctx, GGD_E_INVALID, "geom_buf / binning_buf is NULL");
  hipStream_t s = static_cast<hipStream_t>(stream);
  const geom_ptrs g = geom_view(prm, geom_buf);
  const binning_ptrs b = binning_view(layout_R, binning_buf);
  const img_ptrs im = img_view(prm->width, prm->height, img_buf);
  const bool tiles = use_tile_binning(ctx, prm, R);
  if (speculative && !tiles) return ggd_fail(ctx, GGD_E_INVALID, "speculative render needs the tile-binning path");
  const uint32_t capacity = R > 0xffffffffll ? 0xffffffffu : (uint32_t)R;
  rc = (R > 0 && tiles) ? sort_depth_and_bin_tiles(ctx, s, prm, g, b.list, im.ranges, capacity, speculative)
                        : duplicate_sort_ranges(ctx, s, prm, g, b, im.ranges, R);
  if (rc != GGD_OK) return rc;
  StageTimer t(ctx, ST_BLEND, s);
  return ggd_launch_blend(ctx, s, *prm, g.splat, b.list, im.ranges, capacity, out_color, im.final_T, im.n_contrib, g.depth_keys,
                          out_depth, out_alpha);
}

extern "C" int ggd_forward_render(ggd_ctx* ctx, void* stream, const ggd_params* prm, const void* geom_buf,
                                  int64_t R, void* binning_buf, void* img_buf, float* out_color) {
  if (ctx && ctx->pending.valid) return ggd_fail(ctx, GGD_E_INVALID, kPendingMsg);
  return render_enqueue(ctx, stream, prm, geom_buf, R, R, binning_buf, img_buf, out_color, false);
}

static int check_aux_planes(ggd_ctx* ctx, const float* out_depth, const float* out_alpha) {
  if (!ctx) return GGD_E_INVALID;
  if (!out_depth || !out_alpha) return ggd_fail(ctx, GGD_E_INVALID, "out_depth / out_alpha is NULL");
  return GGD_OK;
}

extern "C" int ggd_forward_render_aux(ggd_ctx* ctx, void* stream, const ggd_params* prm, const void* geom_buf,
                                      int64_t R, void* binning_buf, void* img_buf, float* out_color, float* out_depth,
                                      float* out_alpha) {
  const int rc = check_aux_planes(ctx, out_depth, out_alpha);
  if (rc != GGD_OK) return rc;
  if (ctx->pending.valid) return ggd_fail(ctx, GGD_E_INVALID, kPendingMsg);
  return render_enqueue(ctx, stream, prm, geom_buf, R, R, binning_buf, img_buf, out_color, false, out_depth, out_alpha);
}

extern "C" int ggd_forward_can_speculate(ggd_ctx* ctx, const ggd_params* prm, int64_t capacity) {
  return ctx && prm && prm->P > 0 && use_tile_binning(ctx, prm, capacity) ? 1 : 0;
}

static int forward_spec_enqueue(ggd_ctx* ctx, void* stream, const ggd_params* prm, const float* means3D, const float* shs,
                                const float* colors_precomp, const float* opacities, const float* scales,
                                const float* rotations, const float* cov3D_precomp, void* geom_buf, int32_t* radii,
                                void* binning_buf, int64_t capacity, void* img_buf, float* out_color, int64_t* num_rendered,
                                float* out_depth = nullptr, float* out_alpha = nullptr) {
  int rc = geometry_enqueue(ctx, stream, prm, means3D, shs, colors_precomp, opacities, scales, rotations,
                            cov3D_precomp, geom_buf, radii, num_rendered, true);
  if (rc != GGD_OK) return rc;
  return render_enqueue(ctx, stream, prm, geom_buf, capacity, capacity, binning_buf, img_buf, out_color, true, out_depth,
                        out_alpha);
}
static int forward_spec_collect(ggd_ctx* ctx, void* stream, const ggd_params* prm, const void* geom_buf, void* binning_buf,
                                int64_t capacity, void* img_buf, float* out_color, int64_t* num_rendered,
                                float* out_depth = nullptr, float* out_alpha = nullptr) {
  const int rc = geometry_finish(ctx, stream, prm, num_rendered);
  if (rc != GGD_OK) return rc;
  const ggd_frame done = frame_renew(ctx);
  const bool too_small = *num_rendered > capacity;
  const bool again = ctx->spec.observe(done.plan, done.three_passes, done.report, too_small);
  if (too_small)
    return ggd_fail(ctx, GGD_E_CAPACITY, "binning_buf capacity is below num_rendered: re-run with a larger buffer");
  if (!again) return GGD_OK;
  return render_enqueue(ctx, stream, prm, geom_buf, capacity, *num_rendered, binning_buf, img_buf, out_color, false, out_depth,
                        out_alpha);
}

static int forward_single_call(ggd_ctx* ctx, void* stream, const ggd_params* prm, const float* means3D, const float* shs,
                               const float* colors_precomp, const float* opacities, const float* scales,
                               const float* rotations, const float* cov3D_precomp, void* geom_buf, int32_t* radii,
                               void* binning_buf, int64_t capacity, void* img_buf, float* out_color,
                               int64_t* num_rendered, float* out_depth, float* out_alpha) {
  if (capacity < 0) return ggd_fail(ctx, GGD_E_INVALID, "capacity < 0");
  if (ctx && ctx->pending.valid) return ggd_fail(ctx, GGD_E_INVALID, kPendingMsg);
  if (prm && prm->P > 0 && capacity > 0 && ggd_forward_can_speculate(ctx, prm, capacity)) {
    const int rc = forward_spec_enqueue(ctx, stream, prm, means3D, shs, colors_precomp, opacities, scales, rotations,
                                        cov3D_precomp, geom_buf, radii, binning_buf, capacity, img_buf, out_color, num_rendered,
                                        out_depth, out_alpha);
    if (rc != GGD_OK) return rc;
    return forward_spec_collect(ctx, stream, prm, geom_buf, binning_buf, capacity, img_buf, out_color, num_rendered, out_depth,
                                out_alpha);
  }
  int rc = geometry_enqueue(ctx, stream, prm, means3D, shs, colors_precomp, opacities, scales, rotations,
                            cov3D_precomp, geom_buf, radii, num_rendered, false);
  if (rc != GGD_OK) return rc;
  if (prm->P == 0)
    return render_enqueue(ctx, stream, prm, geom_buf, capacity, 0, binning_buf, img_buf, out_color, false, out_depth, out_alpha);
  rc = geometry_finish(ctx, stream, prm, num_rendered);
  if (rc != GGD_OK) return rc;
  if (*num_rendered > capacity)
    return ggd_fail(ctx, GGD_E_CAPACITY, "binning_buf capacity is below num_rendered: re-run with a larger buffer");
  return render_enqueue(ctx, stream, prm, geom_buf, capacity, *num_rendered, binning_buf, img_buf, out_color, false, out_depth,
                        out_alpha);
}

extern "C" int ggd_forward(ggd_ctx* ctx, void* stream, const ggd_params* prm, const float* means3D, const float* shs,
                           const float* colors_precomp, const float* opacities, const float* scales,
                           const float* rotations, const float* cov3D_precomp, void* geom_buf, int32_t* radii,
                           void* binning_buf, int64_t capacity, void* img_buf, float* out_color,
                           int64_t* num_rendered) {
  return forward_single_call(ctx, stream, prm, means3D, shs, colors_precomp, opacities, scales, rotations, cov3D_precomp,
                             geom_buf, radii, binning_buf, capacity, img_buf, out_color, num_rendered, nullptr, nullptr);
}

extern "C" int ggd_forward_aux(ggd_ctx* ctx, void* stream, const ggd_params* prm, const float* means3D, const float* shs,
                               const float* colors_precomp, const float* opacities, const float* scales,
                               const float* rotations, const float* cov3D_precomp, void* geom_buf, int32_t* radii,
                               void* binning_buf, int64_t capacity, void* img_buf, float* out_color, float* out_depth,
                               float* out_alpha, int64_t* num_rendered) {
  const int rc = check_aux_planes(ctx, out_depth, out_alpha);
  if (rc != GGD_OK) return rc;
  return forward_single_call(ctx, stream, prm, means3D, shs, colors_precomp, opacities, scales, rotations, cov3D_precomp,
                             geom_buf, radii, binning_buf, capacity, img_buf, out_color, num_rendered, out_depth, out_alpha);
}

extern "C" int ggd_forward_enqueue(ggd_ctx* ctx, void* stream, const ggd_params* prm, const float* means3D, const float* shs,
                                   const float* colors_precomp, const float* opacities, const float* scales,
                                   const float* rotations, const float* cov3D_precomp, void* geom_buf, int32_t* radii,
                                   void* binning_buf, int64_t capacity, void* img_buf, float* out_color) {
  if (!ctx) return GGD_E_INVALID;
  if (ctx->pending.valid) return ggd_fail(ctx, GGD_E_INVALID, "ggd_forward_enqueue: the previous frame of this context has not been collected");
  if (!prm || prm->P <= 0 || capacity <= 0 || !ggd_forward_can_speculate(ctx, prm, capacity))
    return ggd_fail(ctx, GGD_E_INVALID, "ggd_forward_enqueue needs the tile-binning path, P > 0 and a capacity (ggd_forward_can_speculate)");
  int64_t dummy = 0;
  const int rc = forward_spec_enqueue(ctx, stream, prm, means3D, shs, colors_precomp, opacities, scales, rotations,
                                      cov3D_precomp, geom_buf, radii, binning_buf, capacity, img_buf, out_color, &dummy);
  if (rc != GGD_OK) return rc;
  ctx->pending = {true, *prm, geom_buf, binning_buf, capacity, img_buf, out_color};
  return GGD_OK;
}

extern "C" int ggd_forward_collect(ggd_ctx* ctx, void* stream, int64_t* num_rendered) {
  if (!ctx || !num_rendered) return GGD_E_INVALID;
  if (!ctx->pending.valid) return ggd_fail(ctx, GGD_E_INVALID, "ggd_forward_collect: no frame is pending on this context");
  ctx->pending.valid = false;
  return forward_spec_collect(ctx, stream, &ctx->pending.prm, ctx->pending.geom, ctx->pending.binning, ctx->pending.capacity,
                              ctx->pending.img, ctx->pending.out, num_rendered);
}

static int backward_impl(ggd_ctx* ctx, void* stream, const ggd_params* prm, const float* means3D,
                         const float* shs, const float* colors_precomp, const float* opacities, const float* scales,
                         const float* rotations, const float* cov3D_precomp, const int32_t* radii,
                         const void* geom_buf, const void* binning_buf, const void* img_buf, int64_t R,
                         const float* dL_dpix, float* dL_dmeans2D, float* dL_dcolors, float* dL_dopacity,
                         float* dL_dmeans3D, float* dL_dcov3D, float* dL_dsh, float* dL_dscales,
                         float* dL_drots, bool aux, const float* dL_ddepth, const float* dL_dalpha,
                         bool abs = false, float* dL_dmeans2D_abs = nullptr) {
  (void)hipGetLastError();
  int rc = check_params(ctx, prm);
  if (rc != GGD_OK) return rc;
  rc = check_inputs(ctx, prm, means3D, shs, colors_precomp, scales, rotations, cov3D_precomp);
  if (rc != GGD_OK) return rc;
  const int P = prm->P;
  if (P == 0) return GGD_OK;
  if (!radii || !geom_buf || !img_buf || !dL_dpix || !dL_dmeans2D || !dL_dcolors || !dL_dopacity ||
      !dL_dmeans3D || !dL_dcov3D || !dL_dscales || !dL_drots || (prm->M > 0 && !dL_dsh) || (R > 0 && !binning_buf))
    return ggd_fail(ctx, GGD_E_INVALID, "ggd_backward: NULL buffer");
  if (abs && !dL_dmeans2D_abs) return ggd_fail(ctx, GGD_E_INVALID, "ggd_backward_abs: NULL dL_dmeans2D_abs");
  if (prm->raw_attributes && (!opacities || cov3D_precomp))
    return ggd_fail(ctx, GGD_E_INVALID, "raw_attributes needs opacities and scales/rotations (no cov3D_precomp)");
  if (prm->antialiasing && !opacities)
    return ggd_fail(ctx, GGD_E_INVALID, "antialiasing needs the opacities in the backward");
  hipStream_t s = static_cast<hipStream_t>(stream);
  const geom_ptrs g = geom_view(prm, geom_buf);
  const binning_ptrs b = binning_view(R, binning_buf);
  const img_ptrs im = img_view(prm->width, prm->height, img_buf);

  const size_t acc_bytes = (size_t)P * GGD_ACC_FLOATS * sizeof(float);
  rc = ggd_reserve_scratch(ctx, ggd_align(acc_bytes), s);
  if (rc != GGD_OK) return rc;
  float* grad_acc = static_cast<float*>(ctx->scratch);
  GGD_HIP(hipMemsetAsync(grad_acc, 0, acc_bytes, s));
  if (cov3D_precomp) {
    GGD_HIP(hipMemsetAsync(dL_dscales, 0, (size_t)P * 3 * sizeof(float), s));
    GGD_HIP(hipMemsetAsync(dL_drots, 0, (size_t)P * 4 * sizeof(float), s));
  }
  if (colors_precomp && prm->M > 0 && dL_dsh) GGD_HIP(hipMemsetAsync(dL_dsh, 0, (size_t)P * prm->M * 3 * sizeof(float), s));

  if (R > 0) {
    StageTimer t(ctx, ST_BLEND_BWD, s);
    rc = ggd_launch_blend_backward(ctx, s, *prm, g.splat, b.list, im.ranges, im.final_T, im.n_contrib, dL_dpix, grad_acc, aux,
                                   g.depth_keys, dL_ddepth, dL_dalpha, abs);
    if (rc != GGD_OK) return rc;
  }
  {
    StageTimer t(ctx, ST_PREPROCESS_BWD, s);
    rc = ggd_launch_preprocess_backward(ctx, s, *prm, means3D, shs, colors_precomp, opacities, dL_dopacity, scales, rotations,
                                        cov3D_precomp, radii, shs ? g.clamped : nullptr, grad_acc, dL_dmeans2D,
                                        dL_dcolors, dL_dmeans3D, dL_dcov3D, dL_dsh, dL_dscales, dL_drots, aux,
                                        abs ? dL_dmeans2D_abs : nullptr);
    if (rc != GGD_OK) return rc;
  }
  return GGD_OK;
}

extern "C" int ggd_backward(ggd_ctx* ctx, void* stream, const ggd_params* prm, const float* means3D,
                            const float* shs, const float* colors_precomp, const float* opacities, const float* scales,
                            const float* rotations, const float* cov3D_precomp, const int32_t* radii,
                            const void* geom_buf, const void* binning_buf, const void* img_buf, int64_t R,
                            const float* dL_dpix, float* dL_dmeans2D, float* dL_dcolors, float* dL_dopacity,
                            float* dL_dmeans3D, float* dL_dcov3D, float* dL_dsh, float* dL_dscales,
                            float* dL_drots) {
  return backward_impl(ctx, stream, prm, means3D, shs, colors_precomp, opacities, scales, rotations, cov3D_precomp, radii,
                       geom_buf, binning_buf, img_buf, R, dL_dpix, dL_dmeans2D, dL_dcolors, dL_dopacity, dL_dmeans3D,
                       dL_dcov3D, dL_dsh, dL_dscales, dL_drots, false, nullptr, nullptr);
}

extern "C" int ggd_backward_aux(ggd_ctx* ctx, void* stream, const ggd_params* prm, const float* means3D,
                                const float* shs, const float* colors_precomp, const float* opacities, const float* scales,
                                const float* rotations, const float* cov3D_precomp, const int32_t* radii,
                                const void* geom_buf, const void* binning_buf, const void* img_buf, int64_t R,
                                const float* dL_dpix, const float* dL_ddepth, const float* dL_dalpha, float* dL_dmeans2D,
                                float* dL_dcolors, float* dL_dopacity, float* dL_dmeans3D, float* dL_dcov3D, float* dL_dsh,
                                float* dL_dscales, float* dL_drots) {
  return backward_impl(ctx, stream, prm, means3D, shs, colors_precomp, opacities, scales, rotations, cov3D_precomp, radii,
                       geom_buf, binning_buf, img_buf, R, dL_dpix, dL_dmeans2D, dL_dcolors, dL_dopacity, dL_dmeans3D,
                       dL_dcov3D, dL_dsh, dL_dscales, dL_drots, true, dL_ddepth, dL_dalpha);
}

extern "C" int ggd_backward_abs(ggd_ctx* ctx, void* stream, const ggd_params* prm, const float* means3D,
                                const float* shs, const float* colors_precomp, const float* opacities, const float* scales,
                                const float* rotations, const float* cov3D_precomp, const int32_t* radii,
                                const void* geom_buf, const void* binning_buf, const void* img_buf, int64_t R,
                                const float* dL_dpix, const float* dL_ddepth, const float* dL_dalpha, float* dL_dmeans2D,
                                float* dL_dcolors, float* dL_dopacity, float* dL_dmeans3D, float* dL_dcov3D, float* dL_dsh,
                                float* dL_dscales, float* dL_drots, float* dL_dmeans2D_abs) {
  return backward_impl(ctx, stream, prm, means3D, shs, colors_precomp, opacities, scales, rotations, cov3D_precomp, radii,
                       geom_buf, binning_buf, img_buf, R, dL_dpix, dL_dmeans2D, dL_dcolors, dL_dopacity, dL_dmeans3D,
                       dL_dcov3D, dL_dsh, dL_dscales, dL_drots, dL_ddepth || dL_dalpha, dL_ddepth, dL_dalpha, true,
                       dL_dmeans2D_abs);
}

extern "C" int ggd_mark_visible(ggd_ctx* ctx, void* stream, int32_t P, const float* means3D,
                                const float* viewmatrix, const float* projmatrix, uint8_t* present) {
  (void)projmatrix;
  if (!ctx) return GGD_E_INVALID;
  if (P < 0) return ggd_fail(ctx, GGD_E_INVALID, "P < 0");
  if (P == 0) return GGD_OK;
  if (!means3D || !viewmatrix || !present) return ggd_fail(ctx, GGD_E_INVALID, "ggd_mark_visible: NULL pointer");
  return ggd_launch_mark_visible(ctx, static_cast<hipStream_t>(stream), P, means3D, viewmatrix, present);
}

extern "C" int ggd_debug_unsorted(ggd_ctx* ctx, void* stream, uint64_t* keys, uint32_t* values, int64_t R) {
  if (!ctx) return GGD_E_INVALID;
  if (R < 0 || (size_t)R > ctx->dbg_cap) return ggd_fail(ctx, GGD_E_INVALID, "no debug copy of that size (debug=1?)");
  hipStream_t s = static_cast<hipStream_t>(stream);
  if (keys && R) GGD_HIP(hipMemcpyAsync(keys, ctx->dbg_keys, (size_t)R * sizeof(uint64_t), hipMemcpyDeviceToDevice, s));
  if (values && R) GGD_HIP(hipMemcpyAsync(values, ctx->dbg_vals, (size_t)R * sizeof(uint32_t), hipMemcpyDeviceToDevice, s));
  return GGD_OK;
}
```

gaussian_gan_decoder_amd/csrc/ggd_common.h:

```cpp
#pragma once

#include <hip/hip_runtime.h>
#include <stdint.h>
#include <string>
#include <type_traits>

#include "ggd_raster.h"
#include "ggd_spec.h"
#include "ggd_binning_layout.h"

#define GGD_WAVE 64

enum {
  ST_PREPROCESS = 0, ST_SCAN, ST_READBACK, ST_DUPLICATE, ST_SORT, ST_RANGES, ST_BLEND,
  ST_BLEND_BWD, ST_PREPROCESS_BWD, ST_COUNT
};

enum { GGD_ATTR_MLP_FWD = 1, GGD_ATTR_MLP_BWD = 2, GGD_ATTR_MLP_WGRAD = 4, GGD_ATTR_MLP_HL = 64 };

constexpr int GGD_STATS_MODE = 9;
constexpr int GGD_STATS_BWD = 16;
constexpr int GGD_STATS_HEAD = 32;
constexpr int GGD_STATS_MAX_WAVES = 1 << 17;


struct ggd_frame {
  struct {
    bool ride = false;
    bool folded = false;
    bool sortctl_clean = false;
  } geom;
  ggd_spec_plan plan;
  bool three_passes = false;
  bool r_pending = false;
  uint32_t r_tag = 0;
  ggd_spec_report report;
};

struct ggd_ctx {
  int device = 0;
  int cus = 0;
  void* scratch = nullptr;
  size_t scratch_bytes = 0;
  uint32_t attr_mask = 0;
  uint32_t* d_words = nullptr;
  uint32_t* h_words = nullptr;
  uint32_t* h_words_dev = nullptr;
  uint32_t* sortctl = nullptr;
  uint32_t* scan_sums = nullptr;
  size_t scan_sums_cap = 0;
  uint32_t* foldctl[2] = {nullptr, nullptr};
  size_t foldctl_cap = 0;
  size_t foldctl_dirty[2] = {0, 0};
  int fold_cur = 0;
  bool fold_poisoned = false;
  unsigned long long scan_in_scatter_frames = 0;
  ggd_spec spec;
  ggd_frame frame;
  struct { bool valid = false; ggd_params prm; const void* geom = nullptr; void* binning = nullptr; int64_t capacity = 0;
           void* img = nullptr; float* out = nullptr; } pending;
  void* gelu_tables = nullptr;
  void *dbg_keys = nullptr, *dbg_vals = nullptr;
  size_t dbg_cap = 0;
  int opt[GGD_OPT_COUNT] = {3, 1, 1, 1, 1, 1, 0};
  unsigned long long* blend_stats = nullptr;
  unsigned long long* stats_buf = nullptr;
  bool profiling = false;
  hipEvent_t ev[2 * ST_COUNT] = {};
  bool ev_used[ST_COUNT] = {};
  std::string err;
};

struct ggd_scan_piggy {
  const uint32_t* in = nullptr;
  uint32_t* out = nullptr;
  int64_t n = 0;
  int nb = 0;
  uint32_t* block_sums = nullptr;
  uint32_t* d_total = nullptr;
  uint32_t* h_total = nullptr;
  unsigned long long* h_tagged = nullptr;
  uint32_t tag = 0;
  const uint4* wg_info = nullptr;
  int n_info = 0;
  uint32_t* n_valid = nullptr;
  int sum_stride = 1;
  uint32_t* flat_flag = nullptr;
  int spec_flat = 0;
  uint32_t* fold_hist = nullptr;
  int msd = 0;
  uint32_t msd_lo = 0;
  int msd_shift = GGD_MSD_SHIFT;
};

struct ggd_fold {
  uint32_t* ctl = nullptr;
  uint32_t* clear = nullptr;
  uint32_t clear_words = 0;
  uint4* wg_info = nullptr;
  int rows = 0;
  uint32_t* rowinst = nullptr;
  int msd = 0;
  uint32_t msd_lo = 0;
  int msd_shift = GGD_MSD_SHIFT;
};

int ggd_fail(ggd_ctx* ctx, int code, const std::string& msg);
int ggd_reserve_scratch(ggd_ctx* ctx, size_t bytes, hipStream_t stream);

static inline const char* ggd_basename(const char* p) {
  const char* b = p;
  for (; *p; ++p) if (*p == '/') b = p + 1;
  return b;
}
#define GGD_HIP(call)                                                                                      \
  do {                                                                                                     \
    hipError_t e_ = (call);                                                                                \
    if (e_ != hipSuccess)                                                                                  \
      return ggd_fail(ctx, GGD_E_HIP, std::string(#call) + " (" + ggd_basename(__FILE__) + ":" +            \
                                          std::to_string(__LINE__) + "): " + hipGetErrorString(e_));         \
  } while (0)

struct StageTimer {
  ggd_ctx* c; int st; hipStream_t s;
  StageTimer(ggd_ctx* ctx, int stage, hipStream_t stream) : c(ctx), st(stage), s(stream) {
    if (c->profiling) { (void)hipEventRecord(c->ev[2 * st], s); }
  }
  ~StageTimer() {
    if (c->profiling) { (void)hipEventRecord(c->ev[2 * st + 1], s); c->ev_used[st] = true; }
  }
};

template <int N, int I = 0, typename F>
static inline void ggd_dispatch(int v, F&& f) {
  if constexpr (I == N - 1) f(std::integral_constant<int, I>{});
  else if (v == I) f(std::integral_constant<int, I>{});
  else ggd_dispatch<N, I + 1>(v, f);
}

int ggd_launch_preprocess(ggd_ctx* ctx, hipStream_t s, const ggd_params& prm, const float* means3D,
                          const float* shs, const float* colors_precomp, const float* opacities,
                          const float* scales, const float* rotations, const float* cov3D_precomp,
                          ggd_splat* splat, uint32_t* tiles_touched, uint8_t* clamped, int32_t* radii,
                          uint32_t* depth_keys, uint2* rect, uint32_t* trap_flag, uint32_t* zero_ptr = nullptr,
                          int zero_words = 0,
                          const ggd_fold* fold = nullptr);
int ggd_launch_mark_visible(ggd_ctx* ctx, hipStream_t s, int P, const float* means3D, const float* view,
                            uint8_t* present);
int ggd_launch_inclusive_scan(ggd_ctx* ctx, hipStream_t s, const uint32_t* in, uint32_t* out, int64_t n,
                              uint32_t* d_total, void* tmp, size_t tmp_bytes, uint32_t* h_total = nullptr);
size_t ggd_scan_tmp_bytes(int64_t n);
int ggd_scan_blocks(int64_t n);
int ggd_launch_duplicate(ggd_ctx* ctx, hipStream_t s, const ggd_params& prm, const uint2* rect,
                         const uint32_t* depth_keys, const uint32_t* tiles_touched, const uint32_t* offsets,
                         uint64_t* keys, uint32_t* vals);
int ggd_sort_input_is_alt(int nbits);
int ggd_launch_sort(ggd_ctx* ctx, hipStream_t s, uint64_t* keys_a, uint32_t* vals_a, uint64_t* keys_b,
                    uint32_t* vals_b, int64_t n, int nbits, void* tmp, size_t tmp_bytes);
struct ggd_sort32_opts {
  uint32_t* clean_ctl = nullptr;
  const ggd_scan_piggy* piggy = nullptr;
  const ggd_fold* fold = nullptr;
  bool flag_flat_last = false;
  bool apply_here = true;
  bool skip_last = false;
};
int ggd_launch_sort32_iota(ggd_ctx* ctx, hipStream_t s, const uint32_t* keys_src, uint32_t* keys_a, uint32_t* vals_a,
                           uint32_t* keys_b, uint32_t* vals_b, int64_t n, int nbits, void* tmp, size_t tmp_bytes,
                           const ggd_sort32_opts& opts = ggd_sort32_opts());
bool ggd_sort32_msd_supported(int64_t n);
int ggd_launch_sort32_msd(ggd_ctx* ctx, hipStream_t s, const uint32_t* keys_src, uint32_t* keys_a, uint32_t* vals_a,
                          uint32_t* keys_b, uint32_t* vals_b, int64_t n, uint32_t* table, const ggd_scan_piggy* piggy,
                          const ggd_fold* fold);
bool ggd_rowbin_supported(int W, int H);
static inline size_t ggd_rowbin_tmp_bytes(int P, uint32_t capacity, int W, int H) { return ggd_rowbin_layout(P, capacity, W, H).total; }
int ggd_launch_rowbin(ggd_ctx* ctx, hipStream_t s, const ggd_params& prm, const uint2* rect, const uint32_t* order,
                      const uint32_t* n_vis_ptr, uint32_t* list, uint32_t* ranges, uint32_t capacity, void* tmp,
                      size_t tmp_bytes, const uint32_t* order_alt = nullptr, const uint32_t* use_alt = nullptr,
                      const ggd_scan_piggy* apply = nullptr, const uint32_t* fold_rowtot = nullptr, uint32_t* fold_status1 = nullptr,
                      const uint32_t* fold_rowinst = nullptr, bool* scan_in_scatter = nullptr);
int ggd_launch_ranges(ggd_ctx* ctx, hipStream_t s, const uint64_t* keys, int64_t n, uint32_t* ranges, int T);
int ggd_launch_blend(ggd_ctx* ctx, hipStream_t s, const ggd_params& prm, const ggd_splat* splat,
                     const uint32_t* list, const uint32_t* ranges, uint32_t capacity, float* out_color, float* final_T,
                     uint32_t* n_contrib, const uint32_t* depth_keys = nullptr, float* out_depth = nullptr,
                     float* out_alpha = nullptr);
constexpr int GGD_ACC_FLOATS = 12;
constexpr int GGD_ACC_CONIC = 0, GGD_ACC_OPACITY = 3, GGD_ACC_MEAN2D = 4, GGD_ACC_COLOR = 6;
constexpr int GGD_ACC_DEPTH = 9;
constexpr int GGD_ACC_ABS = 10;
int ggd_launch_blend_backward(ggd_ctx* ctx, hipStream_t s, const ggd_params& prm, const ggd_splat* splat,
                              const uint32_t* list, const uint32_t* ranges, const float* final_T,
                              const uint32_t* n_contrib, const float* dL_dpix, float* grad_acc ,
                              bool aux = false, const uint32_t* depth_keys = nullptr, const float* dL_ddepth = nullptr,
                              const float* dL_dalpha = nullptr, bool abs = false);
int ggd_launch_preprocess_backward(ggd_ctx* ctx, hipStream_t s, const ggd_params& prm, const float* means3D,
                                   const float* shs, const float* colors_precomp, const float* opacities,
                                   float* dL_dopacity, const float* scales,
                                   const float* rotations, const float* cov3D_precomp, const int32_t* radii,
                                   const uint8_t* clamped, const float* grad_acc, float* dL_dmean2D,
                                   float* dL_dcolors, float* dL_dmeans3D, float* dL_dcov3D, float* dL_dsh,
                                   float* dL_dscales, float* dL_drots, bool aux = false,
                                   float* dL_dmean2D_abs = nullptr);

#ifdef __HIPCC__
__device__ __forceinline__ int ggd_tile_rect(float px, float py, int irad, int gx, int gy, int& minx, int& miny,
                                             int& maxx, int& maxy) {
  const float fr = (float)irad;
  minx = min(gx, max(0, (int)((px - fr) / 16.0f)));
  miny = min(gy, max(0, (int)((py - fr) / 16.0f)));
  maxx = min(gx, max(0, (int)((px + fr + 15.0f) / 16.0f)));
  maxy = min(gy, max(0, (int)((py + fr + 15.0f) / 16.0f)));
  return (maxx - minx) * (maxy - miny);
}
#endif
```

gaussian_gan_decoder_amd/csrc/ggd_msd_finish.inc:

```
constexpr int MSDF_THREADS = 1024, MSDF_ITEMS = GGD_MSD_CAP / MSDF_THREADS, MSDF_WAVES = MSDF_THREADS / 64;
static_assert(MSDF_ITEMS * MSDF_THREADS == GGD_MSD_CAP, "bucket capacity must be a multiple of the workgroup size");

__device__ __forceinline__ uint32_t block_exclusive_scan_1024(uint32_t v, uint32_t* total, uint32_t* lds16) {
  const int lane = threadIdx.x & 63, wv = threadIdx.x >> 6;
  const uint32_t inc = wave_inclusive_scan(v);
  if (lane == 63) lds16[wv] = inc;
  __syncthreads();
  uint32_t base = 0, tot = 0;
#pragma unroll
  for (int w = 0; w < MSDF_WAVES; ++w) {
    const uint32_t s = lds16[w];
    if (w < wv) base += s;
    tot += s;
  }
  __syncthreads();
  *total = tot;
  return base + inc - v;
}

constexpr int MSD_XCAP = 8000;
constexpr int MSDX_ITEMS = (MSD_XCAP + MSDF_THREADS - 1) / MSDF_THREADS;
struct msd_lds {
  uint32_t kv[2 * MSD_XCAP];
  uint16_t cnt[MSDF_WAVES][256];
  uint32_t pp[GGD_MSD_MAX_TILES];
  uint32_t part[MSDF_WAVES];
};
static_assert(2 * sizeof(msd_lds) <= 160 * 1024, "two finish workgroups per CU");
static_assert(GGD_MSD_MAX_SHIFT <= 16, "two 8-bit passes order the bits below the bucket digit");
static_assert(GGD_MSD_CAP < (1 << 20) && MSD_TILE <= (1 << 12), "packed piece word");

__device__ __forceinline__ size_t msd_piece_src(const msd_lds& L, int ntiles, uint32_t p) {
  int lo = 0;
#pragma unroll
  for (int step = GGD_MSD_MAX_TILES / 2; step >= 1; step >>= 1) {
    const int probe = lo + step;
    if (probe < ntiles && (L.pp[probe] >> 12) <= p) lo = probe;
  }
  const uint32_t e = L.pp[lo];
  return (size_t)lo * MSD_TILE + (e & 0xfffu) + (p - (e >> 12));
}
__device__ __forceinline__ size_t msd_piece_src_big(const msd_lds& L, const uint32_t* __restrict__ table, uint32_t b, int ntiles, uint32_t p) {
  int lo = 0;
#pragma unroll
  for (int step = GGD_MSD_MAX_TILES / 2; step >= 1; step >>= 1) {
    const int probe = lo + step;
    if (probe < ntiles && L.pp[probe] <= p) lo = probe;
  }
  return (size_t)lo * MSD_TILE + (table[(size_t)lo * GGD_MSD_BINS + b] >> 16) + (p - L.pp[lo]);
}

__device__ __forceinline__ void msd_bucket_pieces(msd_lds& L, const uint32_t* __restrict__ table, int ntiles, uint32_t b, uint32_t e0,
                                                  bool oversized) {
  const int tid = threadIdx.x;
  uint32_t carry = 0;
  for (int t0 = 0; t0 < ntiles; t0 += MSDF_THREADS) {
    const int t = t0 + tid;
    const uint32_t e = t0 == 0 ? e0 : (t < ntiles ? table[(size_t)t * GGD_MSD_BINS + b] : 0u);
    uint32_t tot;
    const uint32_t ex = block_exclusive_scan_1024(e & 0xffffu, &tot, L.part);
    if (t < ntiles) L.pp[t] = oversized ? carry + ex : ((carry + ex) << 12) | ((e >> 16) & 0xfffu);
    carry += tot;
  }
  __syncthreads();
}

template <bool GLOBAL_X, int ITEMS>
__device__ __forceinline__ void msd_bucket_sort(msd_lds& L, const uint32_t* __restrict__ keys_in, const uint32_t* __restrict__ vals_in,
                                                int ntiles, uint32_t nb, int kshift, uint32_t* xk_g, uint32_t* xv_g) {
  const int tid = threadIdx.x, lane = tid & 63, wv = tid >> 6;
  uint32_t key[ITEMS], val[ITEMS], rank[ITEMS];
  const int rounds = (int)((nb + MSDF_THREADS - 1) / MSDF_THREADS);
  const uint32_t pbase = (uint32_t)wv * (64u * (uint32_t)rounds) + (uint32_t)lane;
#pragma unroll
  for (int r = 0; r < ITEMS; ++r) {
    if (r >= rounds) break;
    const uint32_t p = pbase + r * 64;
    key[r] = 0u; val[r] = 0u;
    if (p < nb) {
      const size_t src = msd_piece_src(L, ntiles, p);
      key[r] = keys_in[src];
      val[r] = vals_in[src];
    }
  }
  const uint64_t lt_mask = (1ull << lane) - 1ull;
#pragma unroll
  for (int pass = 0; pass < 2; ++pass) {
    const int shift = 8 * pass;
    const int nbits = pass == 0 ? min(8, kshift) : kshift - 8;
    if (pass == 1 && nbits <= 0) break;
    if (pass == 1) {
#pragma unroll
      for (int r = 0; r < ITEMS; ++r) {
        if (r >= rounds) break;
        const uint32_t p = pbase + r * 64;
        if (p < nb) {
          if (GLOBAL_X) { key[r] = xk_g[p]; val[r] = xv_g[p]; }
          else { key[r] = L.kv[p]; val[r] = L.kv[MSD_XCAP + p]; }
        }
      }
    }
    for (int z = tid; z < MSDF_WAVES * 128; z += MSDF_THREADS) reinterpret_cast<uint32_t*>(&L.cnt[0][0])[z] = 0u;
    __syncthreads();
#pragma unroll
    for (int r = 0; r < ITEMS; ++r) {
      if (r >= rounds) break;
      const bool ok = pbase + r * 64 < nb;
      const uint32_t d = (key[r] >> shift) & ((1u << nbits) - 1u);
      uint64_t peers = __ballot(ok);
#pragma unroll
      for (int bit = 0; bit < 8; ++bit) {
        if (bit >= nbits) break;
        const uint64_t m = __ballot((d >> bit) & 1u);
        peers &= ((d >> bit) & 1u) ? m : ~m;
      }
      const uint32_t before = L.cnt[wv][d];
      const uint32_t below = (uint32_t)__popcll(peers & lt_mask);
      rank[r] = before + below;
      __builtin_amdgcn_wave_barrier();
      if (ok && below == 0) L.cnt[wv][d] = (uint16_t)(before + (uint32_t)__popcll(peers));
      __builtin_amdgcn_wave_barrier();
    }
    __syncthreads();
    {
      uint32_t local = 0;
      if (tid < 256) {
#pragma unroll
        for (int w = 0; w < MSDF_WAVES; ++w) local += L.cnt[w][tid];
      }
      uint32_t tot;
      uint32_t run = block_exclusive_scan_1024(tid < 256 ? local : 0u, &tot, L.part);
      if (tid < 256) {
#pragma unroll
        for (int w = 0; w < MSDF_WAVES; ++w) { const uint32_t c = L.cnt[w][tid]; L.cnt[w][tid] = (uint16_t)run; run += c; }
      }
    }
    __syncthreads();
#pragma unroll
    for (int r = 0; r < ITEMS; ++r) {
      if (r >= rounds) break;
      if (pbase + r * 64 < nb) {
        const uint32_t d = (key[r] >> shift) & ((1u << nbits) - 1u);
        const uint32_t p = (uint32_t)L.cnt[wv][d] + rank[r];
        if (GLOBAL_X) { xk_g[p] = key[r]; xv_g[p] = val[r]; }
        else { L.kv[p] = key[r]; L.kv[MSD_XCAP + p] = val[r]; }
      }
    }
    __syncthreads();
  }
}
```

gaussian_gan_decoder_amd/csrc/ggd_rowbin.hip:

```cpp
#include "ggd_common.h"

namespace {

#include "ggd_scan.inc"
#include "ggd_lookback.inc"

constexpr int RB_WAVES = RB_THREADS / 64;
constexpr int RB_STAGE = 4096;
constexpr int RB_STAGE1 = 4096;
constexpr int RB_WCHUNK = 64 * RB_IPL;

__device__ __forceinline__ void rb_write_row_tables(uint32_t* tab, int lane, uint32_t tot, uint32_t inc, uint32_t ent_cap) {
  const uint32_t rs = inc - tot;
  tab[RB_TAB_ROWSTART + lane] = rs;
  if (lane == 63) tab[RB_TAB_ROWSTART + 64] = inc;
  const uint32_t have = rs < ent_cap ? min(tot, ent_cap - rs) : 0u;
  const uint32_t nblk = (have + RB_CHUNK - 1) / RB_CHUNK;
  const uint32_t binc = wave_inclusive_scan(nblk);
  tab[RB_TAB_ROWBLK + lane] = binc - nblk;
  if (lane == 63) tab[RB_TAB_ROWBLK + 64] = binc;
  tab[RB_TAB_FLAG + lane] = 0u;
}

__global__ __launch_bounds__(RB_THREADS) void rb_count1_kernel(int W, int H, const uint2* __restrict__ rect,
                                                               const uint32_t* __restrict__ order,
                                                               const uint32_t* __restrict__ n_vis_ptr, int P,
                                                               uint2* __restrict__ packed, uint32_t* __restrict__ counts1,
                                                               const uint32_t* __restrict__ order_alt,
                                                               const uint32_t* __restrict__ use_alt) {
  __shared__ int diff[65];
  if (use_alt && *use_alt != 0u) order = order_alt;
  const uint32_t n_vis = min((uint32_t)P, *n_vis_ptr);
  const uint32_t base = (uint32_t)blockIdx.x * RB_CHUNK;
  if (base >= n_vis) return;
  const int tid = threadIdx.x;
  if (tid < 65) diff[tid] = 0;
  __syncthreads();
#pragma unroll
  for (int q = 0; q < RB_IPL; ++q) {
    const uint32_t rnk = base + (uint32_t)q * RB_THREADS + tid;
    if (rnk < n_vis) {
      const uint32_t id = order[rnk];
      const uint2 rc = rect[id];
      int x0 = (int)(rc.x & 0xffffu), x1 = (int)(rc.x >> 16), y0 = (int)(rc.y & 0xffffu), y1 = (int)(rc.y >> 16);
      const int n = (x1 - x0) * (y1 - y0);
      if (n <= 0) { x0 = x1 = y0 = y1 = 0; }
      packed[rnk] = make_uint2(id, (uint32_t)x0 | ((uint32_t)x1 << 8) | ((uint32_t)y0 << 16) | ((uint32_t)y1 << 24));
      if (n > 0) { atomicAdd(&diff[y0], 1); atomicAdd(&diff[y1], -1); }
    }
  }
  __syncthreads();
  if (tid < 64) counts1[(size_t)blockIdx.x * 64 + tid] = (uint32_t)wave_inclusive_scan(diff[tid]);
}

__global__ __launch_bounds__(1024) void rb_scan1_kernel(uint32_t* __restrict__ counts1,
                                                        const uint32_t* __restrict__ n_vis_ptr, int P,
                                                        uint32_t* __restrict__ tab, uint32_t ent_cap) {
  __shared__ uint32_t part[16][64];
  const int lane = threadIdx.x & 63, wv = threadIdx.x >> 6;
  const uint32_t n_vis = min((uint32_t)P, *n_vis_ptr);
  const int nb = (int)((n_vis + RB_CHUNK - 1) / RB_CHUNK);
  const int per = (nb + 15) / 16;
  const int r0 = min(nb, wv * per), r1 = min(nb, r0 + per);
  uint32_t s = 0;
#pragma unroll 8
  for (int r = r0; r < r1; ++r) s += counts1[(size_t)r * 64 + lane];
  part[wv][lane] = s;
  __syncthreads();
  uint32_t run = 0, tot = 0;
#pragma unroll
  for (int w = 0; w < 16; ++w) { const uint32_t p = part[w][lane]; if (w < wv) run += p; tot += p; }
#pragma unroll 8
  for (int r = r0; r < r1; ++r) {
    const size_t idx = (size_t)r * 64 + lane;
    const uint32_t c = counts1[idx];
    counts1[idx] = run;
    run += c;
  }
  if (wv == 0) rb_write_row_tables(tab, lane, tot, wave_inclusive_scan(tot), ent_cap);
}

template <int D, uint32_t M>
__device__ __forceinline__ void tr_stage(uint32_t& lo, uint32_t& hi, uint32_t lane) {
  const bool up = (lane & (uint32_t)D) != 0;
  const uint32_t keep = up ? ~M : M;
  const uint32_t slo = up ? ((lo & M) << D) : ((lo & ~M) >> D);
  const uint32_t shi = up ? ((hi & M) << D) : ((hi & ~M) >> D);
  lo = (lo & keep) | (uint32_t)__shfl_xor((int)slo, D, 64);
  hi = (hi & keep) | (uint32_t)__shfl_xor((int)shi, D, 64);
}

__device__ __forceinline__ uint64_t wave_transpose64(uint64_t row) {
  const uint32_t lane = threadIdx.x & 63;
  uint32_t lo = (uint32_t)row, hi = (uint32_t)(row >> 32);
  {
    const bool up = (lane & 32u) != 0;
    const uint32_t recv = (uint32_t)__shfl_xor((int)(up ? lo : hi), 32, 64);
    if (up) lo = recv; else hi = recv;
  }
  tr_stage<16, 0x0000FFFFu>(lo, hi, lane);
  tr_stage<8, 0x00FF00FFu>(lo, hi, lane);
  tr_stage<4, 0x0F0F0F0Fu>(lo, hi, lane);
  tr_stage<2, 0x33333333u>(lo, hi, lane);
  tr_stage<1, 0x55555555u>(lo, hi, lane);
  return (uint64_t)lo | ((uint64_t)hi << 32);
}

__device__ __forceinline__ uint32_t wave_cols(const uint32_t (&iv)[RB_IPL], int n_items, uint64_t (&cols)[RB_IPL]) {
  uint32_t cnt = 0;
#pragma unroll
  for (int q = 0; q < RB_IPL; ++q) {
    cols[q] = 0ull;
    if (q * 64 >= n_items) continue;
    const uint32_t l = iv[q] & 0xffu, h = iv[q] >> 8;
    const uint64_t below_h = h >= 64u ? ~0ull : ((1ull << h) - 1ull);
    const uint64_t row = h > l ? (below_h & ~((1ull << l) - 1ull)) : 0ull;
    cols[q] = wave_transpose64(row);
    cnt += (uint32_t)__popcll(cols[q]);
  }
  return cnt;
}

__device__ __forceinline__ bool rb_walk_items(uint32_t width, uint32_t fill) {
  const int wi = __ballot(width > 16u) ? 3 : (__ballot(width > 8u) ? 2 : (__ballot(width > 4u) ? 1 : 0));
  const int wf = __ballot(fill > 16u) ? 3 : (__ballot(fill > 8u) ? 2 : (__ballot(fill > 4u) ? 1 : 0));
  return wi <= wf + 1;
}

template <bool TWO, typename Emit>
__device__ __forceinline__ void wave_emit(const uint32_t (&iv)[RB_IPL], const uint32_t (&pa)[RB_IPL],
                                          const uint32_t (&pb)[RB_IPL], const uint64_t (&cols)[RB_IPL], int n_items,
                                          uint32_t& dst, uint4* slab , Emit&& emit) {
  const int lane = threadIdx.x & 63;
  const uint64_t lt_mask = (1ull << lane) - 1ull;
#pragma unroll
  for (int q = 0; q < RB_IPL; ++q) {
    if (q * 64 >= n_items) continue;
    __builtin_amdgcn_wave_barrier();
    slab[lane] = make_uint4((uint32_t)cols[q], (uint32_t)(cols[q] >> 32), dst, 0u);
    __builtin_amdgcn_wave_barrier();
    const uint32_t l = iv[q] & 0xffu, h = iv[q] >> 8;
    if (rb_walk_items(h > l ? h - l : 0u, (uint32_t)__popcll(cols[q]))) {
      for (uint32_t b = l; __ballot(b < h) != 0ull; ++b) {
        const bool act = b < h;
        const uint4 e = slab[act ? b : 0u];
        const uint64_t m = (uint64_t)e.x | ((uint64_t)e.y << 32);
        if (act) emit(e.z + (uint32_t)__popcll(m & lt_mask), pa[q], TWO ? pb[q] : 0u);
      }
      dst += (uint32_t)__popcll(cols[q]);
    } else {
      uint64_t col = cols[q];
      while (__ballot(col != 0ull) != 0ull) {
        const bool act = col != 0ull;
        const int k = act ? (__ffsll((unsigned long long)col) - 1) : 0;
        col &= col - 1ull;
        const uint32_t a = (uint32_t)__shfl((int)pa[q], k, 64);
        const uint32_t bb = TWO ? (uint32_t)__shfl((int)pb[q], k, 64) : 0u;
        if (act) { emit(dst, a, bb); dst += 1; }
      }
    }
  }
}

__global__ __launch_bounds__(RB_THREADS) void rb_scatter1_kernel(const uint2* __restrict__ packed,
                                                                 const uint32_t* __restrict__ n_vis_ptr, int P,
                                                                 const uint32_t* __restrict__ prefix1,
                                                                 const uint32_t* __restrict__ tab,
                                                                 uint2* __restrict__ ent, uint32_t ent_cap) {
  __shared__ uint4 slab[RB_WAVES][64];
  __shared__ uint32_t wcnt[RB_WAVES][64];
  const uint32_t n_vis = min((uint32_t)P, *n_vis_ptr);
  const uint32_t base = (uint32_t)blockIdx.x * RB_CHUNK;
  if (base >= n_vis) return;
  const int tid = threadIdx.x, lane = tid & 63, wv = tid >> 6;
  const uint32_t wbeg = base + (uint32_t)wv * RB_WCHUNK;
  const int n_items = (int)min((uint32_t)RB_WCHUNK, n_vis > wbeg ? n_vis - wbeg : 0u);
  uint32_t iv[RB_IPL], pa[RB_IPL], pb[RB_IPL];
#pragma unroll
  for (int q = 0; q < RB_IPL; ++q) {
    const int i = q * 64 + lane;
    uint2 it = make_uint2(0, 0);
    if (i < n_items) it = packed[wbeg + i];
    pa[q] = it.x; pb[q] = it.y & 0xffffu;
    iv[q] = it.y >> 16;
  }
  uint64_t cols[RB_IPL];
  const uint32_t mine = wave_cols(iv, n_items, cols);
  wcnt[wv][lane] = mine;
  __syncthreads();
  uint32_t dst = tab[RB_TAB_ROWSTART + lane] + prefix1[(size_t)blockIdx.x * 64 + lane];
#pragma unroll
  for (int w = 0; w < RB_WAVES; ++w) if (w < wv) dst += wcnt[w][lane];
  wave_emit<true>(iv, pa, pb, cols, n_items, dst, slab[wv], [&](uint32_t d, uint32_t id, uint32_t xx) {
    if (d < ent_cap) ent[d] = make_uint2(id, xx);
  });
}

__global__ __launch_bounds__(RB_THREADS) void rb_level1_kernel(const uint2* __restrict__ rect, const uint32_t* __restrict__ order,
                                                               const uint32_t* __restrict__ n_vis_ptr, int P,
                                                               const uint32_t* __restrict__ rowtot, uint32_t* status,
                                                               int chunks_max, int gshift_max, uint32_t* __restrict__ tab,
                                                               uint2* __restrict__ ent, uint32_t ent_cap,
                                                               const uint32_t* __restrict__ order_alt,
                                                               const uint32_t* __restrict__ use_alt,
                                                               const uint32_t* __restrict__ rowinst) {
  __shared__ uint4 slab[RB_WAVES][64];
  __shared__ uint32_t wcnt[RB_WAVES][64];
  __shared__ uint32_t s_base[64];
  __shared__ uint2 stage[RB_STAGE1];
  if (use_alt && *use_alt != 0u) order = order_alt;
  const uint32_t n_vis = min((uint32_t)P, *n_vis_ptr);
  const int tid = threadIdx.x, lane = tid & 63, wv = tid >> 6;
  uint32_t rowstart = 0;
  if (wv == 0) {
    uint32_t tot = 0;
#pragma unroll
    for (int r = 0; r < GGD_FOLD_REPS; ++r) tot += rowtot[r * 64 + lane];
    const uint32_t inc = wave_inclusive_scan(tot);
    rowstart = inc - tot;
    if (blockIdx.x == 0) {
      rb_write_row_tables(tab, lane, tot, inc, ent_cap);
      if (rowinst) {
        uint32_t inst = 0;
#pragma unroll
        for (int r = 0; r < GGD_FOLD_REPS; ++r) inst += rowinst[r * 64 + lane];
        tab[RB_TAB_ROWINST + lane] = inst;
      }
    }
  }
  const uint32_t base = (uint32_t)blockIdx.x * RB_CHUNK;
  if (base >= n_vis) return;
  const uint32_t wbeg = base + (uint32_t)wv * RB_WCHUNK;
  const int n_items = (int)min((uint32_t)RB_WCHUNK, n_vis > wbeg ? n_vis - wbeg : 0u);
  uint32_t iv[RB_IPL], pa[RB_IPL], pb[RB_IPL];
#pragma unroll
  for (int q = 0; q < RB_IPL; ++q) {
    const int i = q * 64 + lane;
    pa[q] = 0; pb[q] = 0; iv[q] = 0;
    if (i < n_items) {
      const uint32_t id = order[wbeg + i];
      const uint2 rc = rect[id];
      const uint32_t x0 = rc.x & 0xffffu, x1 = rc.x >> 16, y0 = rc.y & 0xffffu, y1 = rc.y >> 16;
      pa[q] = id;
      if ((int)(x1 - x0) * (int)(y1 - y0) > 0) { pb[q] = x0 | (x1 << 8); iv[q] = y0 | (y1 << 8); }
    }
  }
  uint64_t cols[RB_IPL];
  const uint32_t mine = wave_cols(iv, n_items, cols);
  wcnt[wv][lane] = mine;
  __syncthreads();
  if (wv == 0) {
    const uint32_t local = wcnt[0][lane] + wcnt[1][lane] + wcnt[2][lane] + wcnt[3][lane];
    const int chunk = (int)blockIdx.x;
    const int live = (int)((n_vis + RB_CHUNK - 1) / RB_CHUNK);
    const int gs = min(ggd_group_shift(live), gshift_max);
    s_base[lane] = lookback_two_level<64>(status, lane, chunks_max, chunk, gs, local, rowstart);
  }
  __syncthreads();
  uint32_t before = 0, rowtot_c = 0;
#pragma unroll
  for (int w = 0; w < RB_WAVES; ++w) { const uint32_t c = wcnt[w][lane]; if (w < wv) before += c; rowtot_c += c; }
  const uint32_t rowend = wave_inclusive_scan(rowtot_c);
  const uint32_t total = (uint32_t)__shfl((int)rowend, 63, 64);
  const uint32_t rowbeg = rowend - rowtot_c;
  const uint32_t gbase = s_base[lane];
  if (total <= (uint32_t)RB_STAGE1) {
    uint32_t ldst = rowbeg + before;
    wave_emit<true>(iv, pa, pb, cols, n_items, ldst, slab[wv], [&](uint32_t d, uint32_t id, uint32_t xx) { stage[d] = make_uint2(id, xx); });
    __syncthreads();
#pragma unroll 4
    for (int c = wv; c < 64; c += RB_WAVES) {
      const uint32_t n = (uint32_t)__shfl((int)rowtot_c, c, 64);
      if (n == 0) continue;
      const uint32_t b0 = (uint32_t)__shfl((int)rowbeg, c, 64), g = (uint32_t)__shfl((int)gbase, c, 64);
      for (uint32_t k = lane; k < n; k += 64) {
        const uint32_t d = g + k;
        if (d < ent_cap) ent[d] = stage[b0 + k];
      }
    }
    return;
  }
  uint32_t dst = gbase + before;
  wave_emit<true>(iv, pa, pb, cols, n_items, dst, slab[wv], [&](uint32_t d, uint32_t id, uint32_t xx) {
    if (d < ent_cap) ent[d] = make_uint2(id, xx);
  });
}

__device__ __forceinline__ bool rb_block_row_range(const uint32_t* __restrict__ tab, uint32_t blk, uint32_t ent_cap, int& row,
                                                   uint32_t& chunk, uint32_t& rbeg, uint32_t& rend) {
  const int lane = threadIdx.x & 63;
  const uint32_t first = tab[RB_TAB_ROWBLK + lane];
  const uint32_t total = tab[RB_TAB_ROWBLK + 64];
  const uint32_t start = tab[RB_TAB_ROWSTART + lane];
  const uint32_t all = tab[RB_TAB_ROWSTART + 64];
  if (blk >= total) return false;
  const int r = __popcll(__ballot(first <= blk)) - 1;
  row = r; chunk = blk - (uint32_t)__shfl((int)first, r, 64);
  rbeg = (uint32_t)__shfl((int)start, r, 64);
  rend = min(r == 63 ? all : (uint32_t)__shfl((int)start, (r + 1) & 63, 64), ent_cap);
  return true;
}

__global__ __launch_bounds__(RB_THREADS) void rb_count2_kernel(const uint2* __restrict__ ent, uint32_t ent_cap,
                                                               const uint32_t* __restrict__ tab,
                                                               uint32_t* __restrict__ counts2) {
  __shared__ int diff[65];
  int row; uint32_t chunk, rbeg, rend;
  if (!rb_block_row_range(tab, blockIdx.x, ent_cap, row, chunk, rbeg, rend)) return;
  const int tid = threadIdx.x;
  const uint32_t base = rbeg + chunk * RB_CHUNK;
  uint32_t xs[RB_IPL];
#pragma unroll
  for (int q = 0; q < RB_IPL; ++q) {
    const uint32_t i = base + (uint32_t)q * RB_THREADS + tid;
    xs[q] = i < rend ? ent[i].y : 0u;
  }
  if (tid < 65) diff[tid] = 0;
  __syncthreads();
#pragma unroll
  for (int q = 0; q < RB_IPL; ++q) {
    const uint32_t x0 = xs[q] & 0xffu, x1 = (xs[q] >> 8) & 0xffu;
    if (x1 > x0) { atomicAdd(&diff[x0], 1); atomicAdd(&diff[x1], -1); }
  }
  __syncthreads();
  if (tid < 64) counts2[(size_t)blockIdx.x * 64 + tid] = (uint32_t)wave_inclusive_scan(diff[tid]);
}

__global__ __launch_bounds__(1024) void rb_scan2_kernel(uint32_t* __restrict__ counts2, uint32_t* tab, int gx, int gy,
                                                        uint32_t* __restrict__ ranges) {
  __shared__ uint32_t part[16][64];
  const int lane = threadIdx.x & 63, wv = threadIdx.x >> 6;
  const int r = blockIdx.x;
  const uint32_t b0 = tab[RB_TAB_ROWBLK + r], b1 = tab[RB_TAB_ROWBLK + r + 1];
  const uint32_t nb = b1 - b0, per = (nb + 15u) / 16u;
  const uint32_t c0 = b0 + min(nb, (uint32_t)wv * per), c1 = min(b1, c0 + per);
  uint32_t s = 0;
#pragma unroll 4
  for (uint32_t b = c0; b < c1; ++b) s += counts2[(size_t)b * 64 + lane];
  part[wv][lane] = s;
  __syncthreads();
  uint32_t run = 0, tot = 0;
#pragma unroll
  for (int w = 0; w < 16; ++w) { const uint32_t p = part[w][lane]; if (w < wv) run += p; tot += p; }
#pragma unroll 4
  for (uint32_t b = c0; b < c1; ++b) {
    const size_t idx = (size_t)b * 64 + lane;
    const uint32_t c = counts2[idx];
    counts2[idx] = run;
    run += c;
  }
  if (wv == 0) {
    const uint32_t inc = wave_inclusive_scan(tot);
    if (lane == 63) {
      tab[RB_TAB_ROWINST + r] = inc;
      __builtin_amdgcn_fence(__ATOMIC_RELEASE, "agent");
      __hip_atomic_store(&tab[RB_TAB_FLAG + r], 1u, __ATOMIC_RELAXED, __HIP_MEMORY_SCOPE_AGENT);
    }
    uint32_t below = 0;
    if (lane < r) {
      while (__hip_atomic_load(&tab[RB_TAB_FLAG + lane], __ATOMIC_RELAXED, __HIP_MEMORY_SCOPE_AGENT) == 0u) {}
    }
    __builtin_amdgcn_fence(__ATOMIC_ACQUIRE, "agent");
    if (lane < r) below = __hip_atomic_load(&tab[RB_TAB_ROWINST + lane], __ATOMIC_RELAXED, __HIP_MEMORY_SCOPE_AGENT);
    const uint32_t binc = wave_inclusive_scan(below);
    const uint32_t rowbase = (uint32_t)__builtin_amdgcn_readlane((int)binc, 63);
    if (lane < gx) {
      const uint32_t start = rowbase + inc - tot;
      tab[RB_TAB_TILESTART + r * 64 + lane] = start;
      const int t = r * gx + lane;
      ranges[2 * t] = tot ? start : 0u;
      ranges[2 * t + 1] = tot ? start + tot : 0u;
    }
  }
}

template <bool SCAN>
__global__ __launch_bounds__(RB_THREADS) void rb_scatter2_kernel(const uint2* __restrict__ ent, uint32_t ent_cap,
                                                                 const uint32_t* __restrict__ tab,
                                                                 const uint32_t* __restrict__ prefix2,
                                                                 uint32_t* __restrict__ list, uint32_t capacity,
                                                                 uint32_t main_blocks, ggd_scan_piggy pg, int gx, int gy,
                                                                 uint32_t* __restrict__ ranges) {
  __shared__ uint4 slab[RB_WAVES][64];
  __shared__ uint32_t wcnt[RB_WAVES][64];
  __shared__ __attribute__((aligned(16))) uint32_t wsum[SCAN ? 2 * RB_WAVES : 1][64];
  __shared__ uint32_t stage[RB_STAGE];
  if (blockIdx.x >= main_blocks) {
    scan_apply_block(pg.in, pg.out, pg.n, pg.block_sums, (int)(blockIdx.x - main_blocks), stage, pg.sum_stride);
    return;
  }
  const int tid = threadIdx.x, lane = tid & 63, wv = tid >> 6;
  uint32_t rowinst = 0, rowblks = 0;
  if constexpr (SCAN) {
    rowinst = tab[RB_TAB_ROWINST + lane];
    rowblks = tab[RB_TAB_ROWBLK + lane + 1] - tab[RB_TAB_ROWBLK + lane];
    if ((int)blockIdx.x < gy && wv == 0) {
      const uint32_t nb_z = (uint32_t)__shfl((int)rowblks, (int)blockIdx.x, 64);
      if (nb_z == 0u && lane < gx) {
        const int t = (int)blockIdx.x * gx + lane;
        ranges[2 * t] = 0u;
        ranges[2 * t + 1] = 0u;
      }
    }
  }
  int row; uint32_t chunk, rbeg, rend;
  if (!rb_block_row_range(tab, blockIdx.x, ent_cap, row, chunk, rbeg, rend)) return;
  const uint32_t wbeg = rbeg + chunk * RB_CHUNK + (uint32_t)wv * RB_WCHUNK;
  const int n_items = (int)min((uint32_t)RB_WCHUNK, rend > wbeg ? rend - wbeg : 0u);
  uint32_t iv[RB_IPL], pa[RB_IPL], pb[RB_IPL];
  const uint32_t blkbeg = rbeg + chunk * RB_CHUNK;
  uint2 raw[RB_IPL];
#pragma unroll
  for (int q = 0; q < RB_IPL; ++q) {
    const int i = q * 64 + lane;
    raw[q] = ent[i < n_items ? wbeg + (uint32_t)i : blkbeg];
  }
  uint32_t gbase = 0;
  if constexpr (SCAN) {
    const uint32_t blk0 = blockIdx.x - chunk;
    const uint32_t nblk_row = (uint32_t)__shfl((int)rowblks, row, 64);
    constexpr int BATCH = 8;
    const uint32_t sub = (uint32_t)lane >> 4, c4 = ((uint32_t)lane & 15u) * 4u;
    uint4 bef4 = make_uint4(0, 0, 0, 0), tot4 = make_uint4(0, 0, 0, 0);
    for (uint32_t k0 = (uint32_t)wv * 4u; k0 < nblk_row; k0 += 4u * RB_WAVES * BATCH) {
      uint4 v[BATCH];
#pragma unroll
      for (int j = 0; j < BATCH; ++j) {
        const uint32_t k = k0 + sub + (uint32_t)(4 * RB_WAVES * j);
        v[j] = make_uint4(0, 0, 0, 0);
        if (k < nblk_row) v[j] = *reinterpret_cast<const uint4*>(prefix2 + (size_t)(blk0 + k) * 64 + c4);
      }
#pragma unroll
      for (int j = 0; j < BATCH; ++j) {
        const uint32_t k = k0 + sub + (uint32_t)(4 * RB_WAVES * j);
        tot4.x += v[j].x; tot4.y += v[j].y; tot4.z += v[j].z; tot4.w += v[j].w;
        const uint32_t m = k < chunk ? 0xffffffffu : 0u;
        bef4.x += v[j].x & m; bef4.y += v[j].y & m; bef4.z += v[j].z & m; bef4.w += v[j].w & m;
      }
    }
#pragma unroll
    for (int d = 16; d <= 32; d <<= 1) {
      tot4.x += (uint32_t)__shfl_xor((int)tot4.x, d, 64); tot4.y += (uint32_t)__shfl_xor((int)tot4.y, d, 64);
      tot4.z += (uint32_t)__shfl_xor((int)tot4.z, d, 64); tot4.w += (uint32_t)__shfl_xor((int)tot4.w, d, 64);
      bef4.x += (uint32_t)__shfl_xor((int)bef4.x, d, 64); bef4.y += (uint32_t)__shfl_xor((int)bef4.y, d, 64);
      bef4.z += (uint32_t)__shfl_xor((int)bef4.z, d, 64); bef4.w += (uint32_t)__shfl_xor((int)bef4.w, d, 64);
    }
    if (lane < 16) {
      *reinterpret_cast<uint4*>(&wsum[wv][c4]) = bef4;
      *reinterpret_cast<uint4*>(&wsum[RB_WAVES + wv][c4]) = tot4;
    }
  } else {
    gbase = tab[RB_TAB_TILESTART + row * 64 + lane] + prefix2[(size_t)blockIdx.x * 64 + lane];
  }
#pragma unroll
  for (int q = 0; q < RB_IPL; ++q) {
    const bool have = q * 64 + lane < n_items;
    pa[q] = have ? raw[q].x : 0u; pb[q] = 0;
    iv[q] = have ? raw[q].y & 0xffffu : 0u;
  }
  uint64_t cols[RB_IPL];
  const uint32_t mine = wave_cols(iv, n_items, cols);
  wcnt[wv][lane] = mine;
  __syncthreads();
  if constexpr (SCAN) {
    uint32_t bef = 0, tot = 0;
#pragma unroll
    for (int w = 0; w < RB_WAVES; ++w) { bef += wsum[w][lane]; tot += wsum[RB_WAVES + w][lane]; }
    const uint32_t rinc = wave_inclusive_scan(rowinst);
    const uint32_t rowbase = (uint32_t)__shfl((int)(rinc - rowinst), row, 64);
    const uint32_t start = rowbase + wave_inclusive_scan(tot) - tot;
    gbase = start + bef;
    if (chunk == 0u && wv == 0 && lane < gx) {
      const int t = row * gx + lane;
      ranges[2 * t] = tot ? start : 0u;
      ranges[2 * t + 1] = tot ? start + tot : 0u;
    }
  }
  uint32_t before = 0, coltot = 0;
#pragma unroll
  for (int w = 0; w < RB_WAVES; ++w) { const uint32_t c = wcnt[w][lane]; if (w < wv) before += c; coltot += c; }
  const uint32_t colend = wave_inclusive_scan(coltot);
  const uint32_t total = (uint32_t)__shfl((int)colend, 63, 64);
  const uint32_t colbeg = colend - coltot;
  if (total <= (uint32_t)RB_STAGE) {
    uint32_t ldst = colbeg + before;
    wave_emit<false>(iv, pa, pb, cols, n_items, ldst, slab[wv], [&](uint32_t d, uint32_t id, uint32_t) { stage[d] = id; });
    __syncthreads();
#pragma unroll 4
    for (int c = wv; c < 64; c += RB_WAVES) {
      const uint32_t n = (uint32_t)__shfl((int)coltot, c, 64);
      if (n == 0) continue;
      const uint32_t b0 = (uint32_t)__shfl((int)colbeg, c, 64), g = (uint32_t)__shfl((int)gbase, c, 64);
      for (uint32_t k = lane; k < n; k += 64) {
        const uint32_t d = g + k;
        if (d < capacity) list[d] = stage[b0 + k];
      }
    }
    return;
  }
  uint32_t dst = gbase + before;
  wave_emit<false>(iv, pa, pb, cols, n_items, dst, slab[wv], [&](uint32_t d, uint32_t id, uint32_t) {
    if (d < capacity) list[d] = id;
  });
}

#include "ggd_rowbin_wide.inc"

}

bool ggd_rowbin_supported(int W, int H) { return W > 0 && H > 0 && (W + 15) / 16 <= 255 && (H + 15) / 16 <= 255; }

int ggd_launch_rowbin(ggd_ctx* ctx, hipStream_t s, const ggd_params& prm, const uint2* rect, const uint32_t* order,
                      const uint32_t* n_vis_ptr, uint32_t* list, uint32_t* ranges, uint32_t capacity, void* tmp,
                      size_t tmp_bytes, const uint32_t* order_alt, const uint32_t* use_alt, const ggd_scan_piggy* apply,
                      const uint32_t* fold_rowtot, uint32_t* fold_status1, const uint32_t* fold_rowinst, bool* scan_in_scatter) {
  if (scan_in_scatter) *scan_in_scatter = false;
  if (!ggd_rowbin_supported(prm.width, prm.height)) return ggd_fail(ctx, GGD_E_INVALID, "tile grid too large for row binning");
  const ggd_rowbin_tmp lay = ggd_rowbin_layout(prm.P, capacity, prm.width, prm.height);
  if (tmp_bytes < lay.total) return ggd_fail(ctx, GGD_E_INVALID, "rowbin tmp too small");
  const int gx = (prm.width + 15) / 16, gy = (prm.height + 15) / 16;
  const bool wide = rb_is_wide(prm.width, prm.height);
  char* p = static_cast<char*>(tmp);
  uint2* packed = reinterpret_cast<uint2*>(p + lay.packed);
  uint32_t* counts1 = reinterpret_cast<uint32_t*>(p + lay.counts1);
  uint32_t* tab = reinterpret_cast<uint32_t*>(p + lay.tab);
  uint2* ent = reinterpret_cast<uint2*>(p + lay.ent);
  uint32_t* counts2 = reinterpret_cast<uint32_t*>(p + lay.counts2);
  const int nb1 = rb_blocks1(prm.P);
  const uint32_t nb2 = rb_blocks2(capacity, wide);
  const uint32_t nb_apply = apply ? (uint32_t)apply->nb : 0u;
  const ggd_scan_piggy pg = apply ? *apply : ggd_scan_piggy{};
  static_assert(RB_THREADS == SCAN_THREADS, "the appended scan workgroups share the launch's block size");
  if (wide) {
    const int ngy = (gy + 63) / 64, ngx = (gx + 63) / 64, nby = 64 * ngy, nbx = 64 * ngx;
    hipLaunchKernelGGL(rbw_count1_kernel, dim3(nb1), dim3(RB_THREADS), 0, s, rect, order, n_vis_ptr, prm.P, nby, packed,
                       counts1, order_alt, use_alt);
    hipLaunchKernelGGL(rbw_scan1_kernel, dim3(1), dim3(1024), 0, s, counts1, n_vis_ptr, prm.P, ngy, tab, capacity);
    hipLaunchKernelGGL(rbw_scatter1_kernel, dim3(nb1), dim3(RB_THREADS), 0, s, packed, n_vis_ptr, prm.P, ngy, counts1, tab,
                       ent, capacity);
    hipLaunchKernelGGL(rbw_count2_kernel, dim3(nb2), dim3(RB_THREADS), 0, s, ent, capacity, tab, nbx, counts2);
    hipLaunchKernelGGL(rbw_scan2_kernel, dim3(gy), dim3(1024), 0, s, counts2, tab, gx, gy, ngx, ranges);
    hipLaunchKernelGGL(rbw_scatter2_kernel, dim3(nb2 + nb_apply), dim3(RB_THREADS), 0, s, ent, capacity, tab, ngx, counts2, list,
                       capacity, nb2, pg);
    GGD_HIP(hipGetLastError());
    return GGD_OK;
  }
  const bool fused2 = fold_rowtot && fold_status1 && fold_rowinst && nb2 <= RB_SCAN_IN_SCATTER_MAX_BLOCKS;
  if (fold_rowtot && fold_status1) {
    hipLaunchKernelGGL(rb_level1_kernel, dim3(nb1), dim3(RB_THREADS), 0, s, rect, order, n_vis_ptr, prm.P, fold_rowtot,
                       fold_status1, nb1, ggd_group_shift(nb1), tab, ent, capacity, order_alt, use_alt,
                       fused2 ? fold_rowinst : nullptr);
  } else {
    hipLaunchKernelGGL(rb_count1_kernel, dim3(nb1), dim3(RB_THREADS), 0, s, prm.width, prm.height, rect, order,
                       n_vis_ptr, prm.P, packed, counts1, order_alt, use_alt);
    hipLaunchKernelGGL(rb_scan1_kernel, dim3(1), dim3(1024), 0, s, counts1, n_vis_ptr, prm.P, tab, capacity);
    hipLaunchKernelGGL(rb_scatter1_kernel, dim3(nb1), dim3(RB_THREADS), 0, s, packed, n_vis_ptr, prm.P, counts1, tab,
                       ent, capacity);
  }
  hipLaunchKernelGGL(rb_count2_kernel, dim3(nb2), dim3(RB_THREADS), 0, s, ent, capacity, tab, counts2);
  if (fused2) {
    hipLaunchKernelGGL(rb_scatter2_kernel<true>, dim3(nb2 + nb_apply), dim3(RB_THREADS), 0, s, ent, capacity, tab, counts2, list,
                       capacity, nb2, pg, gx, gy, ranges);
    if (scan_in_scatter) *scan_in_scatter = true;
  } else {
    hipLaunchKernelGGL(rb_scan2_kernel, dim3(gy), dim3(1024), 0, s, counts2, tab, gx, gy, ranges);
    hipLaunchKernelGGL(rb_scatter2_kernel<false>, dim3(nb2 + nb_apply), dim3(RB_THREADS), 0, s, ent, capacity, tab, counts2, list,
                       capacity, nb2, pg, gx, gy, ranges);
  }
  GGD_HIP(hipGetLastError());
  return GGD_OK;
}
```

include/ggd_raster.h:

```cpp
#ifndef GGD_RASTER_H
#define GGD_RASTER_H

#include <stddef.h>
#include <stdint.h>

#ifdef __cplusplus
extern "C" {
#endif

#define GGD_TILE 16

enum {
  GGD_OK = 0,
  GGD_E_INVALID = -1,
  GGD_E_HIP = -2,
  GGD_E_NOMEM = -3,
  GGD_E_PREFILTER = -4,
  GGD_E_NODEVICE = -5,
  GGD_E_CAPACITY = -6
};

typedef struct ggd_ctx ggd_ctx;

typedef struct ggd_params {
  int32_t P;
  int32_t M;
  int32_t sh_degree;
  int32_t width, height;
  float tanfovx, tanfovy;
  float scale_modifier;
  int32_t prefiltered;
  int32_t debug;
  const float* viewmatrix;
  const float* projmatrix;
  const float* campos;
  const float* bg;
  int32_t raw_attributes;
  int32_t antialiasing;
} ggd_params;

typedef struct ggd_splat {
  float x, y;
  float hA, nB, hC;
  float thr;
  float opacity;
  float r, g, b;
  float ex, ey;
} ggd_splat;

typedef struct ggd_geom_view {
  size_t splat;
  size_t tiles_touched;
  size_t point_offsets;
  size_t clamped;
  size_t depth_keys;
  size_t rect;
  size_t header;
  size_t total;
} ggd_geom_view;

typedef struct ggd_binning_view {
  size_t keys;
  size_t list;
  size_t keys_alt;
  size_t list_alt;
  size_t total;
} ggd_binning_view;

typedef struct ggd_img_view {
  size_t ranges;
  size_t final_T;
  size_t n_contrib;
  size_t total;
} ggd_img_view;

size_t ggd_geom_bytes(int32_t P);
size_t ggd_binning_bytes(int64_t R);
size_t ggd_img_bytes(int32_t width, int32_t height);
int ggd_geom_layout(int32_t P, ggd_geom_view* out);
int ggd_binning_layout(int64_t R, ggd_binning_view* out);
int ggd_img_layout(int32_t width, int32_t height, ggd_img_view* out);

int ggd_sort_bits(int32_t width, int32_t height);

ggd_ctx* ggd_create(int device);
void ggd_destroy(ggd_ctx* ctx);
const char* ggd_last_error(ggd_ctx* ctx);
const char* ggd_version(void);

int ggd_forward_geometry(ggd_ctx* ctx, void* stream, const ggd_params* prm,
                         const float* means3D, const float* shs, const float* colors_precomp,
                         const float* opacities, const float* scales, const float* rotations,
                         const float* cov3D_precomp,
                         void* geom_buf, int32_t* radii, int64_t* num_rendered);

int ggd_forward_render(ggd_ctx* ctx, void* stream, const ggd_params* prm,
                       const void* geom_buf, int64_t num_rendered,
                       void* binning_buf, void* img_buf, float* out_color);

int ggd_forward(ggd_ctx* ctx, void* stream, const ggd_params* prm,
                const float* means3D, const float* shs, const float* colors_precomp, const float* opacities,
                const float* scales, const float* rotations, const float* cov3D_precomp,
                void* geom_buf, int32_t* radii, void* binning_buf, int64_t capacity, void* img_buf,
                float* out_color, int64_t* num_rendered);

int ggd_forward_enqueue(ggd_ctx* ctx, void* stream, const ggd_params* prm,
                        const float* means3D, const float* shs, const float* colors_precomp, const float* opacities,
                        const float* scales, const float* rotations, const float* cov3D_precomp,
                        void* geom_buf, int32_t* radii, void* binning_buf, int64_t capacity, void* img_buf, float* out_color);
int ggd_forward_collect(ggd_ctx* ctx, void* stream, int64_t* num_rendered);
int ggd_forward_can_speculate(ggd_ctx* ctx, const ggd_params* prm, int64_t capacity);

int ggd_backward(ggd_ctx* ctx, void* stream, const ggd_params* prm,
                 const float* means3D, const float* shs, const float* colors_precomp,
                 const float* opacities ,
                 const float* scales, const float* rotations, const float* cov3D_precomp,
                 const int32_t* radii,
                 const void* geom_buf, const void* binning_buf, const void* img_buf, int64_t num_rendered,
                 const float* dL_dpix,
                 float* dL_dmeans2D, float* dL_dcolors, float* dL_dopacity,
                 float* dL_dmeans3D, float* dL_dcov3D, float* dL_dsh, float* dL_dscales, float* dL_drots);

int ggd_forward_aux(ggd_ctx* ctx, void* stream, const ggd_params* prm,
                    const float* means3D, const float* shs, const float* colors_precomp, const float* opacities,
                    const float* scales, const float* rotations, const float* cov3D_precomp,
                    void* geom_buf, int32_t* radii, void* binning_buf, int64_t capacity, void* img_buf,
                    float* out_color, float* out_depth, float* out_alpha, int64_t* num_rendered);
int ggd_forward_render_aux(ggd_ctx* ctx, void* stream, const ggd_params* prm,
                           const void* geom_buf, int64_t num_rendered,
                           void* binning_buf, void* img_buf, float* out_color, float* out_depth, float* out_alpha);
int ggd_backward_aux(ggd_ctx* ctx, void* stream, const ggd_params* prm,
                     const float* means3D, const float* shs, const float* colors_precomp,
                     const float* opacities ,
                     const float* scales, const float* rotations, const float* cov3D_precomp,
                     const int32_t* radii,
                     const void* geom_buf, const void* binning_buf, const void* img_buf, int64_t num_rendered,
                     const float* dL_dpix, const float* dL_ddepth, const float* dL_dalpha,
                     float* dL_dmeans2D, float* dL_dcolors, float* dL_dopacity,
                     float* dL_dmeans3D, float* dL_dcov3D, float* dL_dsh, float* dL_dscales, float* dL_drots);

int ggd_backward_abs(ggd_ctx* ctx, void* stream, const ggd_params* prm,
                     const float* means3D, const float* shs, const float* colors_precomp,
                     const float* opacities ,
                     const float* scales, const float* rotations, const float* cov3D_precomp,
                     const int32_t* radii,
                     const void* geom_buf, const void* binning_buf, const void* img_buf, int64_t num_rendered,
                     const float* dL_dpix, const float* dL_ddepth, const float* dL_dalpha,
                     float* dL_dmeans2D, float* dL_dcolors, float* dL_dopacity,
                     float* dL_dmeans3D, float* dL_dcov3D, float* dL_dsh, float* dL_dscales, float* dL_drots,
                     float* dL_dmeans2D_abs);

int ggd_mark_visible(ggd_ctx* ctx, void* stream, int32_t P, const float* means3D,
                     const float* viewmatrix, const float* projmatrix, uint8_t* present);

int ggd_debug_unsorted(ggd_ctx* ctx, void* stream, uint64_t* keys, uint32_t* values, int64_t num_rendered);

enum {
  GGD_OPT_EXP_MODE = 0,
  GGD_OPT_BLEND_CULL = 1,
  GGD_OPT_BINNING = 2,
  GGD_OPT_BLEND_SPLIT = 3,
  GGD_OPT_FOLD = 4,
  GGD_OPT_MSD_SORT = 5,
  GGD_OPT_PREPROCESS_WGS = 6,
  GGD_OPT_COUNT
};
#define GGD_PREPROCESS_WGS_MAX (1 << 20)
int ggd_set_option(ggd_ctx* ctx, int option, int value);
int ggd_blend_stats(ggd_ctx* ctx, int enable, unsigned long long* out);
int ggd_blend_backward_stats(ggd_ctx* ctx, unsigned long long* out);
int ggd_blend_timeline(ggd_ctx* ctx, unsigned long long* out, int waves);
int ggd_get_option(ggd_ctx* ctx, int option);
enum {
  GGD_STAT_FLAT_STREAK = 100,
  GGD_STAT_SORT_RERUNS = 101,
  GGD_STAT_MSD_FRAMES = 102,
  GGD_STAT_SCAN_IN_SCATTER_FRAMES = 103
};

int ggd_triplane_forward(ggd_ctx* ctx, void* stream, const float* planes_cl, int32_t C, int32_t H, int32_t W,
                         const float* pos, int32_t N, float box_warp, float* out);
int ggd_triplane_backward(ggd_ctx* ctx, void* stream, int32_t C, int32_t H, int32_t W, const float* pos, int32_t N,
                          float box_warp, const float* dout, float* dplanes_cl);

int ggd_trigrid_forward(ggd_ctx* ctx, void* stream, const float* grids_cl, int32_t C, int32_t D, int32_t H, int32_t W,
                        int32_t axes, const float* pos, int32_t N, float box_warp, float* out);
int ggd_trigrid_backward(ggd_ctx* ctx, void* stream, int32_t C, int32_t D, int32_t H, int32_t W, int32_t axes,
                         const float* pos, int32_t N, float box_warp, const float* dout, float* dgrids_cl);

int ggd_planes_gather(ggd_ctx* ctx, void* stream, const float* grids_cl, int32_t C, int32_t D, int32_t H, int32_t W,
                      int32_t axes, const float* mod, const float* pos, int32_t N, float box_warp, float* out);
int ggd_planes_scatter(ggd_ctx* ctx, void* stream, int32_t C, int32_t D, int32_t H, int32_t W, int32_t axes,
                       const float* mod, const float* pos, int32_t N, float box_warp, const float* dout,
                       float* dgrids_cl, int32_t accumulate);

size_t ggd_surface_tmp_bytes(int32_t n);
int ggd_surface_sample(ggd_ctx* ctx, void* stream, const float* sigma, int32_t n, float level, int32_t num_points,
                       float thickness, uint64_t seed, float* positions, uint32_t* num_faces, void* tmp,
                       size_t tmp_bytes);

size_t ggd_decoder_packed_bytes(void);
int ggd_decoder_pack(ggd_ctx* ctx, void* stream, const float* const* params40, void* packed, void* packed_t);
int ggd_attrs_split(ggd_ctx* ctx, void* stream, const float* attrs, int64_t N, float* xyz, float* scale, float* rotation,
                    float* opacity, float* color);
int ggd_attrs_merge(ggd_ctx* ctx, void* stream, int64_t N, const float* dxyz, const float* dscale, const float* drotation,
                    const float* dopacity, const float* dcolor, float* dattrs);
int ggd_decoder_forward(ggd_ctx* ctx, void* stream, const float* feat, const float* pos, int32_t N,
                        const void* packed_weights, float* attrs);

typedef enum ggd_decoder_chain {
  GGD_CHAIN_SEQUENTIAL_REVERSED = 0,
  GGD_CHAIN_SEQUENTIAL = 1,
  GGD_CHAIN_PARALLEL = 2
} ggd_decoder_chain;
int ggd_decoder_pack_chain(ggd_ctx* ctx, void* stream, int32_t chain, const float* const* params40, void* packed,
                           void* packed_t);
int ggd_decoder_forward_chain(ggd_ctx* ctx, void* stream, int32_t chain, const float* feat, const float* pos, int32_t N,
                              const void* packed_weights, float* attrs);

size_t ggd_decoder_zbuf_bytes(int32_t N);
size_t ggd_decoder_packed_t_bytes(void);
int ggd_decoder_forward_train(ggd_ctx* ctx, void* stream, const float* feat, const float* pos, int32_t N,
                              const void* packed_weights, float* attrs, void* zbuf);
int ggd_decoder_backward(ggd_ctx* ctx, void* stream, int32_t N, const void* packed_t, const float* attrs,
                         const float* dattrs, const void* zbuf, void* dzbuf, float* dout, float* dfeat, float* dinfo);
int ggd_decoder_forward_train_chain(ggd_ctx* ctx, void* stream, int32_t chain, const float* feat, const float* pos, int32_t N,
                                    const void* packed_weights, float* attrs, void* zbuf);
int ggd_decoder_backward_chain(ggd_ctx* ctx, void* stream, int32_t chain, int32_t N, const void* packed_t, const float* attrs,
                               const float* dattrs, const void* zbuf, void* dzbuf, float* dout, float* dfeat, float* dinfo);

size_t ggd_decoder_wgrad_floats(void);
int ggd_decoder_wgrad(ggd_ctx* ctx, void* stream, int32_t N, const void* zbuf, const void* dzbuf, const float* dout,
                      const float* feat, const float* pos, const float* attrs, float* wgrad);
int ggd_decoder_wgrad_chain(ggd_ctx* ctx, void* stream, int32_t chain, int32_t N, const void* zbuf, const void* dzbuf,
                            const float* dout, const float* feat, const float* pos, const float* attrs, float* wgrad);

size_t ggd_image_loss_tmp_bytes(int32_t W, int32_t H);
int ggd_image_loss(ggd_ctx* ctx, void* stream, int32_t W, int32_t H, const float* image, const float* target,
                   const float* weights4, float* terms5, float* grad_image, void* tmp, size_t tmp_bytes);

int ggd_image_loss_masked(ggd_ctx* ctx, void* stream, int32_t W, int32_t H, const float* image, const float* target,
                          const float* mask, int32_t mask_w, int32_t mask_h, const float* weights4, float* terms5,
                          float* grad_image, void* tmp, size_t tmp_bytes);
int ggd_mask_composite(ggd_ctx* ctx, void* stream, int32_t W, int32_t H, int32_t channels, const float* src,
                       const float* mask, int32_t mask_w, int32_t mask_h, int32_t backward, float* dst);

size_t ggd_geometry_loss_tmp_bytes(int32_t W, int32_t H);
int ggd_geometry_loss(ggd_ctx* ctx, void* stream, int32_t W, int32_t H, const float* depth, const float* alpha,
                      const float* teacher_depth, const float* teacher_weights, int32_t tw, int32_t th, float tanfovx,
                      float tanfovy, int32_t ray_depth, const float* weights2, float* terms3, float* grad_depth,
                      float* grad_alpha, void* tmp, size_t tmp_bytes);

size_t ggd_knn_tmp_bytes(int32_t P);
int32_t ggd_knn_leaf_size(void);
int32_t ggd_knn_max_points(void);
int ggd_knn3(ggd_ctx* ctx, void* stream, const float* points, int32_t P, float* mean_dist2 ,
             float* dist2 , int32_t* idx ,
             unsigned long long* examined , void* tmp, size_t tmp_bytes);
int ggd_knn3_stage(ggd_ctx* ctx, void* stream, const float* points, int32_t P, float* mean_dist2, float* dist2, int32_t* idx,
                   unsigned long long* examined, void* tmp, size_t tmp_bytes, int32_t stage);

size_t ggd_densify_tmp_bytes(int32_t P);
int ggd_densify_stats(ggd_ctx* ctx, void* stream, int32_t P, const float* grad_means2D, const int32_t* radii ,
                      const uint8_t* filter , float* accum, float* denom, float* max_radii2D );
int ggd_densify_plan(ggd_ctx* ctx, void* stream, int32_t P, const float* accum, const float* denom, const float* scaling,
                     const float* opacity, float max_grad, float split_threshold, float min_opacity, int32_t use_world_size,
                     float world_size, void* tmp, size_t tmp_bytes, int64_t* counts4 );
int ggd_prune_plan(ggd_ctx* ctx, void* stream, int32_t P, const uint8_t* mask, void* tmp, size_t tmp_bytes,
                   int64_t* counts4 );
int ggd_densify_emit(ggd_ctx* ctx, void* stream, int32_t P, int32_t new_P, int32_t M, const float* const* in18,
                     float* const* out18, const float* noise , const void* tmp, size_t tmp_bytes);

int ggd_densify_gather(ggd_ctx* ctx, void* stream, int32_t P, int32_t new_P, int32_t width, const float* in, float* out,
                       const void* tmp, size_t tmp_bytes);

int ggd_decoder_backward_wgrad(ggd_ctx* ctx, void* stream, int32_t N, int32_t chunk, const void* packed_t,
                               const float* attrs, const float* dattrs, const void* zbuf, void* dzbuf, float* dout,
                               float* dfeat, float* dinfo, const float* feat, const float* pos, float* wgrad);
int ggd_decoder_backward_wgrad_chain(ggd_ctx* ctx, void* stream, int32_t chain, int32_t N, int32_t chunk, const void* packed_t,
                                     const float* attrs, const float* dattrs, const void* zbuf, void* dzbuf, float* dout,
                                     float* dfeat, float* dinfo, const float* feat, const float* pos, float* wgrad);

size_t ggd_decoder_packed_hl_bytes(void);
size_t ggd_decoder_dzbuf_hl_bytes(int32_t N);
size_t ggd_decoder_packed_t_hl_bytes(void);
int ggd_decoder_pack_hl(ggd_ctx* ctx, void* stream, const float* const* params40, void* packed_hl, void* packed_t_hl);
int ggd_decoder_forward_hl(ggd_ctx* ctx, void* stream, const float* feat, const float* pos, int32_t N,
                           const void* packed_hl, float* attrs, void* zbuf);
int ggd_decoder_backward_wgrad_hl(ggd_ctx* ctx, void* stream, int32_t N, int32_t chunk, const void* packed_t_hl,
                                  const float* attrs, const float* dattrs, const void* zbuf, void* dzbuf, float* dout,
                                  float* dfeat, float* dinfo, const float* feat, const float* pos, float* wgrad);
int ggd_decoder_pack_hl_chain(ggd_ctx* ctx, void* stream, int32_t chain, const float* const* params40, void* packed_hl,
                              void* packed_t_hl);
int ggd_decoder_forward_hl_chain(ggd_ctx* ctx, void* stream, int32_t chain, const float* feat, const float* pos, int32_t N,
                                 const void* packed_hl, float* attrs, void* zbuf);
int ggd_decoder_backward_wgrad_hl_chain(ggd_ctx* ctx, void* stream, int32_t chain, int32_t N, int32_t chunk,
                                        const void* packed_t_hl, const float* attrs, const float* dattrs, const void* zbuf,
                                        void* dzbuf, float* dout, float* dfeat, float* dinfo, const float* feat,
                                        const float* pos, float* wgrad);

int ggd_density_points(ggd_ctx* ctx, void* stream, const float* grids_cl, int32_t C, int32_t D, int32_t H, int32_t W,
                       int32_t axes, float box_warp, const float* w1, const float* b1, const float* w2, const float* b2,
                       int32_t rgb_act, const float* pos, int32_t N, float* sigma, float* rgb );
int ggd_density_grid(ggd_ctx* ctx, void* stream, const float* grids_cl, int32_t C, int32_t D, int32_t H, int32_t W,
                     int32_t axes, float box_warp, const float* w1, const float* b1, const float* w2, const float* b2,
                     int32_t rgb_act, int32_t n, double cube_length, int32_t lattice, float* sigma,
                     float* rgb );
int ggd_density_lattice(ggd_ctx* ctx, void* stream, int32_t n, double cube_length, int32_t lattice, float* pos);

int ggd_teacher_render(ggd_ctx* ctx, void* stream, const float* grids_cl, int32_t C, int32_t D, int32_t H, int32_t W,
                       int32_t axes, float box_warp, const float* w1, const float* b1, const float* w2, const float* b2,
                       int32_t rgb_act, const float* origins, const float* dirs, int32_t M, double ray_start, double ray_end,
                       const float* coarse_table , int32_t Nc, int32_t Ni, const float* u_coarse, const float* u_fine,
                       int32_t use_crop, double crop_limit, int32_t white_back, float* features, float* depth, float* weights,
                       float* samples );

int ggd_set_profiling(ggd_ctx* ctx, int enabled);
int ggd_stage_count(void);
const char* ggd_stage_name(int stage);
int ggd_stage_times(ggd_ctx* ctx, float* ms_out );

#ifdef __cplusplus
}
#endif
#endif
```

Measured before the change: 5351 frames/s.

## Count per-row tile instances inside MSD sort finish and use them in level-1 rowbin

The MSD sort finish kernel now also loads each sorted Gaussian's tile rect, packs the id with its compressed rect, and builds per-bucket and per-chunk row difference counts. These counts are scanned and published as bucket_rows and boundary_rows tables. A new counted level-1 rowbin kernel reads the packed entries and these prefix tables to get each block's global row offsets directly, with no decoupled lookback or per-item rect gather. This trades extra LDS atomics and global writes in the sort for a cheaper binning pass, and adds temp memory. It is enabled by default for tile grids of at most 64x64.

```diff
diff --git a/gaussian_gan_decoder_amd/_capi.py b/gaussian_gan_decoder_amd/_capi.py
--- a/gaussian_gan_decoder_amd/_capi.py
+++ b/gaussian_gan_decoder_amd/_capi.py
@@ -44,7 +44,9 @@
 
 
 OPT_EXP_MODE, OPT_BLEND_CULL, OPT_BINNING, OPT_BLEND_SPLIT, OPT_FOLD, OPT_MSD_SORT, OPT_PREPROCESS_WGS = 0, 1, 2, 3, 4, 5, 6
+OPT_L1_COUNTED = 7
 STAT_FLAT_STREAK, STAT_SORT_RERUNS, STAT_MSD_FRAMES, STAT_SCAN_IN_SCATTER_FRAMES = 100, 101, 102, 103
+STAT_L1_COUNTED_FRAMES = 104
 SPLAT_BYTES = 48
 SPLAT_FIELDS = ("x", "y", "hA", "nB", "hC", "thr", "opacity", "r", "g", "b", "ex", "ey")
 
diff --git a/gaussian_gan_decoder_amd/csrc/ggd_binning.hip b/gaussian_gan_decoder_amd/csrc/ggd_binning.hip
--- a/gaussian_gan_decoder_amd/csrc/ggd_binning.hip
+++ b/gaussian_gan_decoder_amd/csrc/ggd_binning.hip
@@ -458,7 +458,8 @@
                                                                        uint32_t* __restrict__ keys_out,
                                                                        uint32_t* __restrict__ vals_out,
                                                                        const uint32_t* __restrict__ hist ,
-                                                                       const uint32_t* __restrict__ table, int ntiles, int kshift) {
+                                                                       const uint32_t* __restrict__ table, int ntiles, int kshift,
+                                                                       msd_rows rows ) {
   __shared__ msd_lds L;
   const int tid = threadIdx.x;
   const uint32_t b = blockIdx.x;
@@ -478,14 +479,25 @@
       const size_t src = msd_piece_src_big(L, table, b, ntiles, p);
       vals_out[(size_t)base + p] = vals_in[src];
     }
+  } else if (nb > (uint32_t)MSD_XCAP) {
+    msd_bucket_sort<true, MSDF_ITEMS>(L, keys_in, vals_in, ntiles, nb, kshift, keys_out + base, vals_out + base, rows, base);
+  }
+  uint32_t run = 0;
+  if (nb > (uint32_t)MSD_XCAP) {
+    if (!rows.rect) return;
+    for (uint32_t p0 = 0; p0 < nb; p0 += (uint32_t)GGD_MSD_CAP) {
+      __syncthreads();
+      msd_bucket_rows(L, rows, b, base, nb, p0, run, vals_out + base);
+    }
     return;
   }
-  if (nb > (uint32_t)MSD_XCAP) {
-    msd_bucket_sort<true, MSDF_ITEMS>(L, keys_in, vals_in, ntiles, nb, kshift, keys_out + base, vals_out + base);
-    return;
-  }
-  msd_bucket_sort<false, MSDX_ITEMS>(L, keys_in, vals_in, ntiles, nb, kshift, nullptr, nullptr);
-  for (uint32_t p = tid; p < nb; p += MSDF_THREADS) vals_out[(size_t)base + p] = L.kv[MSD_XCAP + p];
+  msd_bucket_sort<false, MSDX_ITEMS>(L, keys_in, vals_in, ntiles, nb, kshift, nullptr, nullptr, rows, base);
+  if (rows.rect && tid < 64) msd_publish_rows(reinterpret_cast<const int*>(&L.pp[0]), rows, b, base, base + nb, true, run);
+  for (uint32_t p = tid; p < nb; p += MSDF_THREADS) {
+    const uint32_t id = L.kv[MSD_XCAP + p];
+    vals_out[(size_t)base + p] = id;
+    if (rows.rect && base + p < rows.n) rows.packed[base + p] = make_uint2(id, L.kv[p]);
+  }
 }
 
 __global__ __launch_bounds__(256) void ranges_kernel(const uint64_t* __restrict__ keys, int64_t n,
@@ -617,7 +629,7 @@
 
 int ggd_launch_sort32_msd(ggd_ctx* ctx, hipStream_t s, const uint32_t* keys_src, uint32_t* keys_a, uint32_t* vals_a,
                           uint32_t* keys_b, uint32_t* vals_b, int64_t n, uint32_t* table, const ggd_scan_piggy* piggy,
-                          const ggd_fold* fold) {
+                          const ggd_fold* fold, const ggd_l1_counted* counted) {
   if (n <= 0) return GGD_OK;
   if (!fold || !fold->msd || !piggy || !piggy->wg_info || !ggd_sort32_msd_supported(n))
     return ggd_fail(ctx, GGD_E_INVALID, "sort32 (two launches): needs the folded front end in its msd form");
@@ -628,8 +640,14 @@
   pg.n_valid = ctl.n_valid; pg.fold_hist = ctl.ghist;
   hipLaunchKernelGGL(sort_msd_partition_kernel, dim3(ntiles + 1), dim3(RS_THREADS), 0, s, keys_src, keys_b, vals_b, n, table,
                      ntiles, fold->msd_lo, fold->msd_shift, pg);
+  msd_rows rows = {};
+  if (counted) {
+    if (!counted->rect || !counted->packed || !counted->bucket_rows || !counted->boundary_rows || counted->chunks != rb_blocks1((int)n))
+      return ggd_fail(ctx, GGD_E_INVALID, "sort32 (two launches): incomplete arrays for the counted level 1");
+    rows = msd_rows{counted->rect, counted->packed, counted->bucket_rows, counted->boundary_rows, (uint32_t)counted->chunks, (uint32_t)n};
+  }
   hipLaunchKernelGGL(sort_msd_finish_kernel, dim3(GGD_MSD_BINS), dim3(MSDF_THREADS), 0, s, keys_b, vals_b, keys_a, vals_a,
-                     ctl.ghist, table, ntiles, fold->msd_shift);
+                     ctl.ghist, table, ntiles, fold->msd_shift, rows);
   GGD_HIP(hipGetLastError());
   return GGD_OK;
 }
diff --git a/gaussian_gan_decoder_amd/csrc/ggd_binning_layout.h b/gaussian_gan_decoder_amd/csrc/ggd_binning_layout.h
--- a/gaussian_gan_decoder_amd/csrc/ggd_binning_layout.h
+++ b/gaussian_gan_decoder_amd/csrc/ggd_binning_layout.h
@@ -120,6 +120,7 @@
 
 struct ggd_rowbin_tmp {
   size_t packed, counts1, tab, ent, counts2, total;
+  size_t bucket_rows, boundary_rows, total_counted;
 };
 static inline ggd_rowbin_tmp ggd_rowbin_layout(int P, uint32_t capacity, int W, int H) {
   const bool wide = rb_is_wide(W, H);
@@ -131,5 +132,8 @@
   t.ent = t.tab + ggd_align((size_t)(wide ? RBW_TAB_WORDS : RB_TAB_WORDS) * 4);
   t.counts2 = t.ent + ggd_align((size_t)capacity * 8);
   t.total = t.counts2 + ggd_align((size_t)rb_blocks2(capacity, wide) * (wide ? nbx : 64) * 4);
+  t.bucket_rows = t.total;
+  t.boundary_rows = t.bucket_rows + ggd_align((size_t)GGD_MSD_BINS * 64 * 4);
+  t.total_counted = t.boundary_rows + ggd_align((size_t)rb_blocks1(P) * 64 * 4);
   return t;
 }
diff --git a/gaussian_gan_decoder_amd/csrc/ggd_capi.hip b/gaussian_gan_decoder_amd/csrc/ggd_capi.hip
--- a/gaussian_gan_decoder_amd/csrc/ggd_capi.hip
+++ b/gaussian_gan_decoder_amd/csrc/ggd_capi.hip
@@ -138,6 +138,7 @@
   if (const char* e = getenv("GGD_FOLD")) ctx->opt[GGD_OPT_FOLD] = atoi(e) != 0;
   if (const char* e = getenv("GGD_MSD_SORT")) ctx->opt[GGD_OPT_MSD_SORT] = atoi(e) != 0;
   if (const char* e = getenv("GGD_PREPROCESS_WGS")) { const int v = atoi(e); if (v >= 0 && v <= GGD_PREPROCESS_WGS_MAX) ctx->opt[GGD_OPT_PREPROCESS_WGS] = v; }
+  if (const char* e = getenv("GGD_L1_COUNTED")) ctx->opt[GGD_OPT_L1_COUNTED] = atoi(e) != 0;
   if (const char* e = getenv("GGD_MSD_BUCKETS")) { const int v = atoi(e); if (v >= 16 && v <= GGD_MSD_BINS) ctx->spec.msd_buckets = v; }
   int prev = 0;
   (void)hipGetDevice(&prev);
@@ -181,7 +182,7 @@
 
 extern "C" int ggd_set_option(ggd_ctx* ctx, int option, int value) {
   if (!ctx) return GGD_E_INVALID;
-  static const int kMax[GGD_OPT_COUNT] = {3, 1, 3, 4, 1, 1, GGD_PREPROCESS_WGS_MAX};
+  static const int kMax[GGD_OPT_COUNT] = {3, 1, 3, 4, 1, 1, GGD_PREPROCESS_WGS_MAX, 1};
   if (option < 0 || option >= GGD_OPT_COUNT || value < 0 || value > kMax[option])
     return ggd_fail(ctx, GGD_E_INVALID, "ggd_set_option: unknown option or value");
   ctx->opt[option] = value;
@@ -228,6 +229,7 @@
   if (ctx && option == GGD_STAT_SORT_RERUNS) return (int)(ctx->spec.reruns & 0x7fffffffull);
   if (ctx && option == GGD_STAT_MSD_FRAMES) return (int)(ctx->spec.msd_frames & 0x7fffffffull);
   if (ctx && option == GGD_STAT_SCAN_IN_SCATTER_FRAMES) return (int)(ctx->scan_in_scatter_frames & 0x7fffffffull);
+  if (ctx && option == GGD_STAT_L1_COUNTED_FRAMES) return (int)(ctx->l1_counted_frames & 0x7fffffffull);
   if (!ctx || option < 0 || option >= GGD_OPT_COUNT) return GGD_E_INVALID;
   return ctx->opt[option];
 }
@@ -468,6 +470,8 @@
   ggd_scan_piggy pg;
   ggd_fold fold;
   const uint32_t *n_vis_ptr = nullptr, *flat_ptr = nullptr;
+  const bool narrow = !rb_is_wide(prm->width, prm->height);
+  bool counted = false;
   {
     StageTimer t(ctx, ST_SORT, s);
     if (riding) {
@@ -489,10 +493,13 @@
     fr.report.folded = folded;
     fold.msd = msd ? 1 : 0;
     fold.msd_lo = fr.plan.lo; fold.msd_shift = fr.plan.shift;
-    if (msd)
+    if (msd) {
+      counted = ctx->opt[GGD_OPT_L1_COUNTED] != 0 && narrow;
+      const ggd_l1_counted l1c = ggd_rowbin_counted(bin_tmp_ptr, g.rect, prm->P, capacity, prm->width, prm->height);
       rc = ggd_launch_sort32_msd(ctx, s, g.depth_keys, ka, va, kb, vb, prm->P,
-                                 reinterpret_cast<uint32_t*>(sc + 4 * pairs + sort_tmp + bin_tmp), &pg, &fold);
-    else {
+                                 reinterpret_cast<uint32_t*>(sc + 4 * pairs + sort_tmp + bin_tmp), &pg, &fold,
+                                 counted ? &l1c : nullptr);
+    } else {
       ggd_sort32_opts so;
       so.clean_ctl = folded ? nullptr : clean_ctl;
       so.piggy = riding ? &pg : nullptr;
@@ -508,13 +515,14 @@
     n_vis_ptr = sc.n_valid; flat_ptr = sc.flat;
   }
   StageTimer t(ctx, ST_DUPLICATE, s);
-  const bool l1 = folded && (prm->width + 15) / 16 <= 64 && (prm->height + 15) / 16 <= 64;
+  const bool l1 = folded && narrow;
   bool scan_in_scatter = false;
   rc = ggd_launch_rowbin(ctx, s, *prm, g.rect, va, n_vis_ptr, list, ranges, capacity, bin_tmp_ptr, bin_tmp, vb,
                          flat_ptr, riding ? &pg : nullptr, l1 ? ggd_fold_rowtot(fold.ctl) : nullptr,
                          l1 ? ggd_fold_l1_status(fold.ctl, prm->P) : nullptr, l1 ? ggd_fold_rowinst(fold.ctl, prm->P) : nullptr,
-                         &scan_in_scatter);
+                         &scan_in_scatter, counted ? ggd_sort_ctl::in_fold(fold.ctl).ghist : nullptr);
   if (scan_in_scatter) ++ctx->scan_in_scatter_frames;
+  if (counted && rc == GGD_OK) ++ctx->l1_counted_frames;
   return rc;
 }
 
diff --git a/gaussian_gan_decoder_amd/csrc/ggd_common.h b/gaussian_gan_decoder_amd/csrc/ggd_common.h
--- a/gaussian_gan_decoder_amd/csrc/ggd_common.h
+++ b/gaussian_gan_decoder_amd/csrc/ggd_common.h
@@ -55,6 +55,7 @@
   int fold_cur = 0;
   bool fold_poisoned = false;
   unsigned long long scan_in_scatter_frames = 0;
+  unsigned long long l1_counted_frames = 0;
   ggd_spec spec;
   ggd_frame frame;
   struct { bool valid = false; ggd_params prm; const void* geom = nullptr; void* binning = nullptr; int64_t capacity = 0;
@@ -62,7 +63,7 @@
   void* gelu_tables = nullptr;
   void *dbg_keys = nullptr, *dbg_vals = nullptr;
   size_t dbg_cap = 0;
-  int opt[GGD_OPT_COUNT] = {3, 1, 1, 1, 1, 1, 0};
+  int opt[GGD_OPT_COUNT] = {3, 1, 1, 1, 1, 1, 0, 1};
   unsigned long long* blend_stats = nullptr;
   unsigned long long* stats_buf = nullptr;
   bool profiling = false;
@@ -169,16 +170,34 @@
                            uint32_t* keys_b, uint32_t* vals_b, int64_t n, int nbits, void* tmp, size_t tmp_bytes,
                            const ggd_sort32_opts& opts = ggd_sort32_opts());
 bool ggd_sort32_msd_supported(int64_t n);
+struct ggd_l1_counted {
+  const uint2* rect = nullptr;
+  uint2* packed = nullptr;
+  uint32_t* bucket_rows = nullptr;
+  uint32_t* boundary_rows = nullptr;
+  int chunks = 0;
+};
 int ggd_launch_sort32_msd(ggd_ctx* ctx, hipStream_t s, const uint32_t* keys_src, uint32_t* keys_a, uint32_t* vals_a,
                           uint32_t* keys_b, uint32_t* vals_b, int64_t n, uint32_t* table, const ggd_scan_piggy* piggy,
-                          const ggd_fold* fold);
+                          const ggd_fold* fold, const ggd_l1_counted* counted = nullptr);
 bool ggd_rowbin_supported(int W, int H);
-static inline size_t ggd_rowbin_tmp_bytes(int P, uint32_t capacity, int W, int H) { return ggd_rowbin_layout(P, capacity, W, H).total; }
+static inline size_t ggd_rowbin_tmp_bytes(int P, uint32_t capacity, int W, int H) { return ggd_rowbin_layout(P, capacity, W, H).total_counted; }
+static inline ggd_l1_counted ggd_rowbin_counted(void* tmp, const uint2* rect, int P, uint32_t capacity, int W, int H) {
+  const ggd_rowbin_tmp lay = ggd_rowbin_layout(P, capacity, W, H);
+  char* p = static_cast<char*>(tmp);
+  ggd_l1_counted c;
+  c.rect = rect; c.packed = reinterpret_cast<uint2*>(p + lay.packed);
+  c.bucket_rows = reinterpret_cast<uint32_t*>(p + lay.bucket_rows);
+  c.boundary_rows = reinterpret_cast<uint32_t*>(p + lay.boundary_rows);
+  c.chunks = rb_blocks1(P);
+  return c;
+}
 int ggd_launch_rowbin(ggd_ctx* ctx, hipStream_t s, const ggd_params& prm, const uint2* rect, const uint32_t* order,
                       const uint32_t* n_vis_ptr, uint32_t* list, uint32_t* ranges, uint32_t capacity, void* tmp,
                       size_t tmp_bytes, const uint32_t* order_alt = nullptr, const uint32_t* use_alt = nullptr,
                       const ggd_scan_piggy* apply = nullptr, const uint32_t* fold_rowtot = nullptr, uint32_t* fold_status1 = nullptr,
-                      const uint32_t* fold_rowinst = nullptr, bool* scan_in_scatter = nullptr);
+                      const uint32_t* fold_rowinst = nullptr, bool* scan_in_scatter = nullptr,
+                      const uint32_t* counted_hist = nullptr);
 int ggd_launch_ranges(ggd_ctx* ctx, hipStream_t s, const uint64_t* keys, int64_t n, uint32_t* ranges, int T);
 int ggd_launch_blend(ggd_ctx* ctx, hipStream_t s, const ggd_params& prm, const ggd_splat* splat,
                      const uint32_t* list, const uint32_t* ranges, uint32_t capacity, float* out_color, float* final_T,
diff --git a/gaussian_gan_decoder_amd/csrc/ggd_msd_finish.inc b/gaussian_gan_decoder_amd/csrc/ggd_msd_finish.inc
--- a/gaussian_gan_decoder_amd/csrc/ggd_msd_finish.inc
+++ b/gaussian_gan_decoder_amd/csrc/ggd_msd_finish.inc
@@ -65,11 +65,79 @@
   __syncthreads();
 }
 
+constexpr int MSD_ROW_SEGS = GGD_MSD_CAP / 1024 + 1;
+static_assert(MSD_ROW_SEGS * 65 * sizeof(int) <= sizeof(msd_lds::cnt) && MSD_ROW_SEGS * 65 * sizeof(int) <= sizeof(msd_lds::pp),
+              "the row difference arrays reuse the digit counts / the piece table");
+struct msd_rows {
+  const uint2* rect; uint2* packed; uint32_t* bucket_rows; uint32_t* boundary_rows;
+  uint32_t chunks, n;
+};
+
+__device__ __forceinline__ uint32_t msd_count_rows(int* diff, uint32_t k0, uint32_t rank, uint2 rc) {
+  uint32_t x0 = rc.x & 0xffffu, x1 = rc.x >> 16, y0 = min(rc.y & 0xffffu, 64u), y1 = min(rc.y >> 16, 64u);
+  const bool any = (int)(x1 - x0) * (int)(y1 - y0) > 0 && y1 > y0;
+  if (!any) return 0u;
+  const uint32_t s = min((rank >> 10) - k0, (uint32_t)(MSD_ROW_SEGS - 1));
+  atomicAdd(&diff[s * 65u + y0], 1);
+  atomicAdd(&diff[s * 65u + y1], -1);
+  return (x0 & 0xffu) | ((x1 & 0xffu) << 8) | (y0 << 16) | (y1 << 24);
+}
+
+__device__ __forceinline__ void msd_publish_rows(const int* diff, const msd_rows& R, uint32_t b, uint32_t first, uint32_t end, bool last,
+                                                 uint32_t& run) {
+  const int tid = threadIdx.x;
+  const uint32_t k0 = first >> 10;
+  const uint32_t nseg = min(((end - 1u) >> 10) - k0 + 1u, (uint32_t)MSD_ROW_SEGS);
+  for (uint32_t s = 0; s < nseg; ++s) {
+    const uint32_t k = k0 + s;
+    if ((s > 0u || (first & 1023u) == 0u) && k < R.chunks) R.boundary_rows[(size_t)k * 64 + tid] = run;
+    run += (uint32_t)wave_inclusive_scan(diff[s * 65u + tid]);
+  }
+  if (last) R.bucket_rows[(size_t)b * 64 + tid] = run;
+}
+
+__device__ __forceinline__ void msd_bucket_rows(msd_lds& L, const msd_rows& R, uint32_t b, uint32_t base, uint32_t nb, uint32_t p0,
+                                                uint32_t& run, const uint32_t* vals_g) {
+  const int tid = threadIdx.x;
+  int* diff = reinterpret_cast<int*>(&L.cnt[0][0]);
+  const uint32_t p1 = min(nb, p0 + (uint32_t)GGD_MSD_CAP);
+  const uint32_t k0 = (base + p0) >> 10;
+  for (uint32_t z = tid; z < (uint32_t)(MSD_ROW_SEGS * 65); z += MSDF_THREADS) diff[z] = 0;
+  __syncthreads();
+  constexpr int RB = 4;
+#pragma unroll 1
+  for (uint32_t q0 = p0; q0 < p1; q0 += (uint32_t)(RB * MSDF_THREADS)) {
+    uint32_t id[RB];
+    uint2 rc[RB];
+#pragma unroll
+    for (int r = 0; r < RB; ++r) {
+      const uint32_t p = q0 + (uint32_t)(r * MSDF_THREADS + tid);
+      id[r] = 0u; rc[r] = make_uint2(0u, 0u);
+      if (p < p1) {
+        id[r] = vals_g[p];
+        rc[r] = R.rect[min(id[r], R.n - 1u)];
+      }
+    }
+#pragma unroll
+    for (int r = 0; r < RB; ++r) {
+      const uint32_t p = q0 + (uint32_t)(r * MSDF_THREADS + tid);
+      if (p < p1 && base + p < R.n) R.packed[base + p] = make_uint2(id[r], msd_count_rows(diff, k0, base + p, rc[r]));
+    }
+  }
+  __syncthreads();
+  if (tid < 64) msd_publish_rows(diff, R, b, base + p0, base + p1, p1 == nb, run);
+}
+
 template <bool GLOBAL_X, int ITEMS>
 __device__ __forceinline__ void msd_bucket_sort(msd_lds& L, const uint32_t* __restrict__ keys_in, const uint32_t* __restrict__ vals_in,
-                                                int ntiles, uint32_t nb, int kshift, uint32_t* xk_g, uint32_t* xv_g) {
+                                                int ntiles, uint32_t nb, int kshift, uint32_t* xk_g, uint32_t* xv_g,
+                                                const msd_rows& R, uint32_t base) {
   const int tid = threadIdx.x, lane = tid & 63, wv = tid >> 6;
   uint32_t key[ITEMS], val[ITEMS], rank[ITEMS];
+  const bool rows_here = !GLOBAL_X && R.rect != nullptr;
+  int* diff = reinterpret_cast<int*>(&L.pp[0]);
+  constexpr int EARLY = GLOBAL_X ? 1 : 4;
+  uint2 rc[EARLY];
   const int rounds = (int)((nb + MSDF_THREADS - 1) / MSDF_THREADS);
   const uint32_t pbase = (uint32_t)wv * (64u * (uint32_t)rounds) + (uint32_t)lane;
 #pragma unroll
@@ -100,8 +168,22 @@
         }
       }
     }
+    const bool count_rows = rows_here && (pass == 1 || kshift <= 8);
+    if constexpr (!GLOBAL_X) {
+      if (count_rows) {
+#pragma unroll
+        for (int r = 0; r < EARLY; ++r) {
+          if (r >= rounds) break;
+          rc[r] = make_uint2(0u, 0u);
+          if (pbase + r * 64 < nb) rc[r] = R.rect[min(val[r], R.n - 1u)];
+        }
+      }
+    }
     for (int z = tid; z < MSDF_WAVES * 128; z += MSDF_THREADS) reinterpret_cast<uint32_t*>(&L.cnt[0][0])[z] = 0u;
     __syncthreads();
+    if (count_rows) {
+      for (int z = tid; z < MSD_ROW_SEGS * 65; z += MSDF_THREADS) diff[z] = 0;
+    }
 #pragma unroll
     for (int r = 0; r < ITEMS; ++r) {
       if (r >= rounds) break;
@@ -142,10 +224,14 @@
       if (pbase + r * 64 < nb) {
         const uint32_t d = (key[r] >> shift) & ((1u << nbits) - 1u);
         const uint32_t p = (uint32_t)L.cnt[wv][d] + rank[r];
-        if (GLOBAL_X) { xk_g[p] = key[r]; xv_g[p] = val[r]; }
-        else { L.kv[p] = key[r]; L.kv[MSD_XCAP + p] = val[r]; }
-      }
-    }
-    __syncthreads();
-  }
-}
+        if constexpr (GLOBAL_X) { xk_g[p] = key[r]; xv_g[p] = val[r]; }
+        else {
+          L.kv[p] = !count_rows ? key[r]
+                               : msd_count_rows(diff, base >> 10, base + p, r < EARLY ? rc[r < EARLY ? r : 0] : R.rect[min(val[r], R.n - 1u)]);
+          L.kv[MSD_XCAP + p] = val[r];
+        }
+      }
+    }
+    __syncthreads();
+  }
+}
diff --git a/gaussian_gan_decoder_amd/csrc/ggd_rowbin.hip b/gaussian_gan_decoder_amd/csrc/ggd_rowbin.hip
--- a/gaussian_gan_decoder_amd/csrc/ggd_rowbin.hip
+++ b/gaussian_gan_decoder_amd/csrc/ggd_rowbin.hip
@@ -286,6 +286,139 @@
   });
 }
 
+__global__ __launch_bounds__(RB_THREADS) void rb_level1_counted_kernel(const uint2* __restrict__ packed,
+                                                                       const uint32_t* __restrict__ hist ,
+                                                                       const uint32_t* __restrict__ n_vis_ptr, int P,
+                                                                       const uint32_t* __restrict__ rowtot,
+                                                                       const uint32_t* __restrict__ bucket_rows,
+                                                                       const uint32_t* __restrict__ boundary_rows,
+                                                                       uint32_t* __restrict__ tab, uint2* __restrict__ ent,
+                                                                       uint32_t ent_cap, const uint32_t* __restrict__ rowinst) {
+  __shared__ uint4 slab[RB_WAVES][64];
+  __shared__ uint32_t wcnt[RB_WAVES][64];
+  __shared__ uint2 stage[RB_STAGE1];
+  __shared__ uint32_t s_scan[RB_WAVES][2];
+  __shared__ __attribute__((aligned(16))) uint32_t s_rows[RB_WAVES][64];
+  uint16_t* s_used = reinterpret_cast<uint16_t*>(stage);
+  static_assert(GGD_MSD_BINS * sizeof(uint16_t) <= sizeof(stage), "the bucket list fits the staging buffer");
+  static_assert(GGD_MSD_BINS == 4 * RB_THREADS, "a thread takes four buckets of the histogram");
+  const int tid = threadIdx.x, lane = tid & 63, wv = tid >> 6;
+  const uint32_t base = (uint32_t)blockIdx.x * RB_CHUNK;
+  const uint32_t wbeg = base + (uint32_t)wv * RB_WCHUNK;
+  const uint32_t n_vis = min((uint32_t)P, *n_vis_ptr);
+  const uint4 h4 = reinterpret_cast<const uint4*>(hist)[tid];
+  uint32_t tot = 0;
+#pragma unroll
+  for (int r = 0; r < GGD_FOLD_REPS; ++r) tot += rowtot[r * 64 + lane];
+  const uint32_t bound = boundary_rows[(size_t)blockIdx.x * 64 + lane];
+  uint2 raw[RB_IPL];
+#pragma unroll
+  for (int q = 0; q < RB_IPL; ++q) raw[q] = packed[min(wbeg + (uint32_t)(q * 64 + lane), (uint32_t)P - 1u)];
+  const uint32_t inc = wave_inclusive_scan(tot);
+  const uint32_t rowstart = inc - tot;
+  if (blockIdx.x == 0 && wv == 0) {
+    rb_write_row_tables(tab, lane, tot, inc, ent_cap);
+    if (rowinst) {
+      uint32_t inst = 0;
+#pragma unroll
+      for (int r = 0; r < GGD_FOLD_REPS; ++r) inst += rowinst[r * 64 + lane];
+      tab[RB_TAB_ROWINST + lane] = inst;
+    }
+  }
+  if (base >= n_vis) return;
+  const int n_items = (int)min((uint32_t)RB_WCHUNK, n_vis > wbeg ? n_vis - wbeg : 0u);
+  uint32_t n_used;
+  {
+    const uint32_t h[4] = {h4.x, h4.y, h4.z, h4.w};
+    const uint32_t hsum = h4.x + h4.y + h4.z + h4.w;
+    const uint32_t hinc = wave_inclusive_scan(hsum);
+    if (lane == 63) s_scan[wv][0] = hinc;
+    __syncthreads();
+    uint32_t end = hinc - hsum;
+#pragma unroll
+    for (int w = 0; w < RB_WAVES; ++w) if (w < wv) end += s_scan[w][0];
+    uint32_t use = 0;
+#pragma unroll
+    for (int j = 0; j < 4; ++j) {
+      end += h[j];
+      if (h[j] != 0u && end <= base) use |= 1u << j;
+    }
+    const uint32_t ucnt = (uint32_t)__popc(use);
+    const uint32_t uinc = wave_inclusive_scan(ucnt);
+    if (lane == 63) s_scan[wv][1] = uinc;
+    __syncthreads();
+    uint32_t pos = uinc - ucnt;
+    n_used = 0;
+#pragma unroll
+    for (int w = 0; w < RB_WAVES; ++w) { const uint32_t c = s_scan[w][1]; if (w < wv) pos += c; n_used += c; }
+#pragma unroll
+    for (int j = 0; j < 4; ++j) if (use & (1u << j)) s_used[pos++] = (uint16_t)(4 * tid + j);
+  }
+  uint32_t iv[RB_IPL], pa[RB_IPL], pb[RB_IPL];
+#pragma unroll
+  for (int q = 0; q < RB_IPL; ++q) {
+    const bool have = q * 64 + lane < n_items;
+    const uint32_t y0 = min((raw[q].y >> 16) & 0xffu, 64u), y1 = min(raw[q].y >> 24, 64u);
+    pa[q] = have ? raw[q].x : 0u;
+    pb[q] = have ? raw[q].y & 0xffffu : 0u;
+    iv[q] = have ? y0 | (y1 << 8) : 0u;
+  }
+  uint64_t cols[RB_IPL];
+  const uint32_t mine = wave_cols(iv, n_items, cols);
+  wcnt[wv][lane] = mine;
+  __syncthreads();
+  {
+    constexpr int BATCH = 8;
+    const uint32_t sub = (uint32_t)lane >> 4, c4 = ((uint32_t)lane & 15u) * 4u;
+    uint4 acc = make_uint4(0, 0, 0, 0);
+    for (uint32_t i0 = (uint32_t)wv * 4u; i0 < n_used; i0 += 4u * RB_WAVES * BATCH) {
+      uint4 v[BATCH];
+#pragma unroll
+      for (int j = 0; j < BATCH; ++j) {
+        const uint32_t i = i0 + sub + (uint32_t)(4 * RB_WAVES * j);
+        v[j] = make_uint4(0, 0, 0, 0);
+        if (i < n_used) v[j] = *reinterpret_cast<const uint4*>(bucket_rows + (size_t)s_used[i] * 64 + c4);
+      }
+#pragma unroll
+      for (int j = 0; j < BATCH; ++j) { acc.x += v[j].x; acc.y += v[j].y; acc.z += v[j].z; acc.w += v[j].w; }
+    }
+#pragma unroll
+    for (int d = 16; d <= 32; d <<= 1) {
+      acc.x += (uint32_t)__shfl_xor((int)acc.x, d, 64); acc.y += (uint32_t)__shfl_xor((int)acc.y, d, 64);
+      acc.z += (uint32_t)__shfl_xor((int)acc.z, d, 64); acc.w += (uint32_t)__shfl_xor((int)acc.w, d, 64);
+    }
+    if (lane < 16) *reinterpret_cast<uint4*>(&s_rows[wv][c4]) = acc;
+  }
+  __syncthreads();
+  uint32_t before = 0, rowtot_c = 0;
+#pragma unroll
+  for (int w = 0; w < RB_WAVES; ++w) { const uint32_t c = wcnt[w][lane]; if (w < wv) before += c; rowtot_c += c; }
+  const uint32_t gbase = rowstart + bound + s_rows[0][lane] + s_rows[1][lane] + s_rows[2][lane] + s_rows[3][lane];
+  const uint32_t rowend = wave_inclusive_scan(rowtot_c);
+  const uint32_t total = (uint32_t)__shfl((int)rowend, 63, 64);
+  const uint32_t rowbeg = rowend - rowtot_c;
+  if (total <= (uint32_t)RB_STAGE1) {
+    uint32_t ldst = rowbeg + before;
+    wave_emit<true>(iv, pa, pb, cols, n_items, ldst, slab[wv], [&](uint32_t d, uint32_t id, uint32_t xx) { stage[d] = make_uint2(id, xx); });
+    __syncthreads();
+#pragma unroll 4
+    for (int c = wv; c < 64; c += RB_WAVES) {
+      const uint32_t n = (uint32_t)__shfl((int)rowtot_c, c, 64);
+      if (n == 0) continue;
+      const uint32_t b0 = (uint32_t)__shfl((int)rowbeg, c, 64), g = (uint32_t)__shfl((int)gbase, c, 64);
+      for (uint32_t k = lane; k < n; k += 64) {
+        const uint32_t d = g + k;
+        if (d < ent_cap) ent[d] = stage[b0 + k];
+      }
+    }
+    return;
+  }
+  uint32_t dst = gbase + before;
+  wave_emit<true>(iv, pa, pb, cols, n_items, dst, slab[wv], [&](uint32_t d, uint32_t id, uint32_t xx) {
+    if (d < ent_cap) ent[d] = make_uint2(id, xx);
+  });
+}
+
 __device__ __forceinline__ bool rb_block_row_range(const uint32_t* __restrict__ tab, uint32_t blk, uint32_t ent_cap, int& row,
                                                    uint32_t& chunk, uint32_t& rbeg, uint32_t& rend) {
   const int lane = threadIdx.x & 63;
@@ -513,7 +646,8 @@
 int ggd_launch_rowbin(ggd_ctx* ctx, hipStream_t s, const ggd_params& prm, const uint2* rect, const uint32_t* order,
                       const uint32_t* n_vis_ptr, uint32_t* list, uint32_t* ranges, uint32_t capacity, void* tmp,
                       size_t tmp_bytes, const uint32_t* order_alt, const uint32_t* use_alt, const ggd_scan_piggy* apply,
-                      const uint32_t* fold_rowtot, uint32_t* fold_status1, const uint32_t* fold_rowinst, bool* scan_in_scatter) {
+                      const uint32_t* fold_rowtot, uint32_t* fold_status1, const uint32_t* fold_rowinst, bool* scan_in_scatter,
+                      const uint32_t* counted_hist) {
   if (scan_in_scatter) *scan_in_scatter = false;
   if (!ggd_rowbin_supported(prm.width, prm.height)) return ggd_fail(ctx, GGD_E_INVALID, "tile grid too large for row binning");
   const ggd_rowbin_tmp lay = ggd_rowbin_layout(prm.P, capacity, prm.width, prm.height);
@@ -546,7 +680,12 @@
     return GGD_OK;
   }
   const bool fused2 = fold_rowtot && fold_status1 && fold_rowinst && nb2 <= RB_SCAN_IN_SCATTER_MAX_BLOCKS;
-  if (fold_rowtot && fold_status1) {
+  if (counted_hist) {
+    if (!fold_rowtot || tmp_bytes < lay.total_counted) return ggd_fail(ctx, GGD_E_INVALID, "rowbin: counted level 1 needs the folded front end and its row tables");
+    hipLaunchKernelGGL(rb_level1_counted_kernel, dim3(nb1), dim3(RB_THREADS), 0, s, packed, counted_hist, n_vis_ptr, prm.P,
+                       fold_rowtot, reinterpret_cast<const uint32_t*>(p + lay.bucket_rows),
+                       reinterpret_cast<const uint32_t*>(p + lay.boundary_rows), tab, ent, capacity, fused2 ? fold_rowinst : nullptr);
+  } else if (fold_rowtot && fold_status1) {
     hipLaunchKernelGGL(rb_level1_kernel, dim3(nb1), dim3(RB_THREADS), 0, s, rect, order, n_vis_ptr, prm.P, fold_rowtot,
                        fold_status1, nb1, ggd_group_shift(nb1), tab, ent, capacity, order_alt, use_alt,
                        fused2 ? fold_rowinst : nullptr);
diff --git a/include/ggd_raster.h b/include/ggd_raster.h
--- a/include/ggd_raster.h
+++ b/include/ggd_raster.h
@@ -163,6 +163,7 @@
   GGD_OPT_FOLD = 4,
   GGD_OPT_MSD_SORT = 5,
   GGD_OPT_PREPROCESS_WGS = 6,
+  GGD_OPT_L1_COUNTED = 7,
   GGD_OPT_COUNT
 };
 #define GGD_PREPROCESS_WGS_MAX (1 << 20)
@@ -175,7 +176,8 @@
   GGD_STAT_FLAT_STREAK = 100,
   GGD_STAT_SORT_RERUNS = 101,
   GGD_STAT_MSD_FRAMES = 102,
-  GGD_STAT_SCAN_IN_SCATTER_FRAMES = 103
+  GGD_STAT_SCAN_IN_SCATTER_FRAMES = 103,
+  GGD_STAT_L1_COUNTED_FRAMES = 104
 };
 
 int ggd_triplane_forward(ggd_ctx* ctx, void* stream, const float* planes_cl, int32_t C, int32_t H, int32_t W,
```

Measured after the change: 5462 frames/s, median of 6. 1.02x the previous value.
